# irenemizus/ArtStyleTransfer

Hardware: AMD Instinct MI355X
Metric: style-transfer iters/sec at L=2 (1024-px) (higher is better)
Workload: dtype f32 via f16x2 split (3 f16 MFMAs per product, f32 accumulate; the 14 large-channel conv launches of a closure as Winograd F(2,3) in that arithmetic); 1 GPU; pyramid style transfer, levels_num=3 (1536x1024+768x512+384x256), lbfgs as the reference constructs it (max_eval 1 under torch 2.10), content+noise init, seeded synthetic VGG19 weights, per-step image yield on; parallelism=1 GPU

## Files before the change

### artstyletransfer_amd/_lib.py

```python
from __future__ import annotations

import ctypes as C
import os
import subprocess
import threading

_HERE = os.path.dirname(os.path.abspath(__file__))
LIB_PATH = os.environ.get("NST_LIB") or os.path.join(_HERE, "libnst_hip.so")
CSRC = os.path.join(_HERE, "csrc")

NST_OK = 0
NST_E_ARG = -1
NST_E_STATE = -2
NST_E_UNAVAILABLE = -5
NST_VGG19_CONVS = 13
NST_MAX_LEVELS = 8
NST_LOSS_ROW = 4
NST_MAX_STYLES = 8
NST_OPT_ADAM = 0
NST_OPT_LBFGS = 1
NST_COLOR_RGB = 0
NST_COLOR_LUMINANCE = 1
NST_POOL_MAX = 0
NST_POOL_AVG = 1

c_float_p = C.POINTER(C.c_float)
REDUCE_HOOK = C.CFUNCTYPE(None, C.c_void_p)
c_void = C.c_void_p


NST_CONV_F32, NST_CONV_BF16X3, NST_CONV_F16X2 = 0, 1, 2
CONV_MODES = {"f32": NST_CONV_F32, "bf16x3": NST_CONV_BF16X3, "f16x2": NST_CONV_F16X2}
NST_COMM_ID_BYTES = 128


class StepInfo(C.Structure):
    _fields_ = [("closures", C.c_int), ("total_closures", C.c_int), ("accepted", C.c_int),
                ("loss", C.c_float), ("lr", C.c_float), ("t", C.c_float), ("history", C.c_int)]


class Options(C.Structure):
    _fields_ = [("struct_size", C.c_int), ("conv_mode", C.c_int), ("batched", C.c_int), ("single_stream", C.c_int),
                ("use_graph", C.c_int), ("h2_band_rows", C.c_int), ("lbfgs_gram", C.c_int), ("h2_mfma16", C.c_int),
                ("h2_wg256", C.c_int), ("h2_tile_rows", C.c_int), ("gram_overlap", C.c_int), ("h2_persist", C.c_int), ("level_split", C.c_int), ("h2_winograd", C.c_int)]


class LaunchInfo(C.Structure):
    _fields_ = [(n, C.c_int) for n in ("cls", "h", "w", "cin", "cout", "layer", "h2_rows", "h2_bn", "h2_ntw", "h2_chunk",
                                       "h2_mfma16", "h2_persist", "h2_second", "h2_unpool", "h2_bands")]


SYMBOLS = {
    "nst_version": (C.c_int, []),
    "nst_last_error": (C.c_char_p, [c_void]),
    "nst_device_count": (C.c_int, [C.POINTER(C.c_int)]),
    "nst_ctx_create": (C.c_int, [C.c_int, C.POINTER(c_void), C.POINTER(c_void), C.POINTER(c_void)]),
    "nst_options_default": (None, [C.POINTER(Options)]),
    "nst_ctx_create_ex": (C.c_int, [C.c_int, C.POINTER(c_void), C.POINTER(c_void), C.POINTER(Options), C.POINTER(c_void)]),
    "nst_ctx_destroy": (None, [c_void]),
    "nst_job_configure": (C.c_int, [c_void, C.c_int, C.c_int, C.c_int]),
    "nst_job_set_taps": (C.c_int, [c_void, C.c_int, C.c_uint, C.c_int]),
    "nst_job_set_color": (C.c_int, [c_void, C.c_int]),
    "nst_job_color": (C.c_int, [c_void]),
    "nst_job_set_pooling": (C.c_int, [c_void, C.c_int]),
    "nst_job_pooling": (C.c_int, [c_void]),
    "nst_job_set_style_weights": (C.c_int, [c_void, c_float_p]),
    "nst_job_style_weights": (C.c_int, [c_void, c_float_p]),
    "nst_color_stats": (C.c_int, [c_void, c_void, C.c_int, C.c_int, C.POINTER(C.c_double), C.POINTER(C.c_double), c_void]),
    "nst_color_transfer_matrix": (C.c_int, [C.POINTER(C.c_double)] * 6),
    "nst_color_affine": (C.c_int, [c_void, c_void, C.c_int, C.c_int, C.POINTER(C.c_double), C.POINTER(C.c_double), c_void, c_void]),
    "nst_luminance": (C.c_int, [c_void, c_void, C.c_int, C.c_int, C.c_double, C.c_double, c_void, c_void]),
    "nst_luminance_recombine": (C.c_int, [c_void, c_void, c_void, C.c_int, C.c_int, c_void, c_void]),
    "nst_level_set_targets": (C.c_int, [c_void, C.c_int, c_void, c_void, C.c_int, C.c_int, c_void]),
    "nst_level_set_targets_blend": (C.c_int, [c_void, C.c_int, c_void, C.c_int, C.POINTER(c_void), C.POINTER(C.c_int),
                                              C.POINTER(C.c_int), c_float_p, c_void]),
    "nst_level_set_guidance": (C.c_int, [c_void, C.c_int, C.c_int, c_void, c_float_p, c_void]),
    "nst_level_set_targets_guided": (C.c_int, [c_void, C.c_int, c_void, c_void, C.c_int, C.c_int, c_void, c_void]),
    "nst_level_guidance": (C.c_int, [c_void, C.c_int, C.POINTER(C.c_int), c_float_p, C.POINTER(C.c_double)]),
    "nst_level_guidance_planes": (C.c_int, [c_void, C.c_int, C.c_int, c_void, c_void]),
    "nst_closure": (C.c_int, [c_void, c_void, C.c_float, C.c_float, C.c_float, c_void, c_void, c_void]),
    "nst_closure_levels": (C.c_int, [c_void, c_void, C.c_float, C.c_float, C.c_float, C.c_uint, c_void, c_void, c_void]),
    "nst_closure_forward": (C.c_int, [c_void, c_void, C.c_float, C.c_float, C.c_float, C.c_uint, c_void, c_void]),
    "nst_closure_backward": (C.c_int, [c_void, c_void, C.c_float, C.c_float, C.c_float, C.c_uint, c_void, c_void]),
    "nst_opt_shard_levels": (C.c_int, [c_void, C.c_uint, c_void, c_void, c_void, c_void]),
    "nst_opt_shard_levels_comm": (C.c_int, [c_void, C.c_uint, c_void]),
    "nst_opt_history": (C.c_int, [c_void, C.POINTER(C.c_int), C.POINTER(C.c_int)]),
    "nst_opt_set_closure_reuse": (C.c_int, [c_void, C.c_int]),
    "nst_opt_closure_stats": (C.c_int, [c_void, C.POINTER(C.c_long), C.POINTER(C.c_long)]),
    "nst_opt_set_lazy_backward": (C.c_int, [c_void, C.c_int]),
    "nst_opt_backward_stats": (C.c_int, [c_void, C.POINTER(C.c_long), C.POINTER(C.c_long)]),
    "nst_comm_unique_id": (C.c_int, [c_void]),
    "nst_comm_create": (C.c_int, [C.c_int, C.c_int, C.c_int, c_void, C.POINTER(c_void)]),
    "nst_comm_destroy": (None, [c_void]),
    "nst_comm_info": (C.c_int, [c_void, C.POINTER(C.c_int), C.POINTER(C.c_int), C.POINTER(C.c_long), C.POINTER(C.c_double)]),
    "nst_comm_allreduce_sum": (C.c_int, [c_void, c_void, C.c_size_t, c_void]),
    "nst_adam_step": (C.c_int, [c_void, c_void, c_void, c_void, c_void, C.c_size_t, C.c_int, C.c_double, c_void]),
    "nst_lbfgs_direction": (C.c_int, [c_void, c_void, C.POINTER(c_void), C.POINTER(c_void), C.POINTER(C.c_float), C.c_int,
                                      C.c_float, C.c_size_t, C.c_int, c_void, c_void]),
    "nst_opt_create": (C.c_int, [c_void, C.c_int, C.c_float, C.c_int, C.POINTER(c_void)]),
    "nst_opt_destroy": (None, [c_void]),
    "nst_opt_step": (C.c_int, [c_void, c_void, C.c_float, C.c_float, C.c_float, c_void, C.c_int,
                               C.POINTER(StepInfo), c_void]),
    "nst_vgg_features": (C.c_int, [c_void, c_void, C.c_int, C.c_int, C.POINTER(c_void), c_void]),
    "nst_vgg_features_backward": (C.c_int, [c_void, c_void, C.c_int, C.c_int, C.POINTER(c_void), c_void, c_void]),
    "nst_vgg_activations": (C.c_int, [c_void, c_void, C.c_int, C.c_int, C.POINTER(c_void), c_void]),
    "nst_level_activation": (C.c_int, [c_void, C.c_int, C.c_int, c_void, c_void]),
    "nst_level_image": (C.c_int, [c_void, C.c_int, c_void, c_void]),
    "nst_gram": (C.c_int, [c_void, c_void, C.c_int, C.c_int, C.c_int, C.c_int, c_void, c_void]),
    "nst_guided_gram_backward": (C.c_int, [c_void, c_void, C.c_size_t, C.c_int, C.c_int, c_void, c_void, c_void, c_void, c_void,
                                            c_void, c_void]),
    "nst_total_variation": (C.c_int, [c_void, c_void, C.c_int, C.c_int, C.c_int, c_void, c_void, c_void]),
    "nst_bicubic_half": (C.c_int, [c_void, c_void, C.c_int, C.c_int, C.c_int, c_void, c_void]),
    "nst_bicubic_half_backward": (C.c_int, [c_void, c_void, C.c_int, C.c_int, C.c_int, c_void, c_void]),
    "nst_prepare_img": (C.c_int, [c_void, c_void, C.c_int, C.c_int, c_void, c_void]),
    "nst_unprepare_img": (C.c_int, [c_void, c_void, C.c_int, C.c_int, c_void, c_void]),
    "nst_resize_bicubic": (C.c_int, [c_void, c_void, C.c_int, C.c_int, C.c_int, c_void, C.c_int, C.c_int, c_void]),
    "nst_gather_rows": (C.c_int, [c_void, c_void, c_void, C.c_size_t, C.c_int, c_void, c_void]),
    "nst_gaussian_mask_accumulate": (C.c_int, [c_void, c_void, c_void, C.c_int, C.c_int, C.c_int, C.c_double, C.c_double,
                                               C.c_double, c_void]),
    "nst_noise_blend": (C.c_int, [c_void, c_void, c_void, C.c_int, C.c_int, C.c_int, C.c_double, c_void, c_void]),
    "nst_scale": (C.c_int, [c_void, c_void, C.c_float, C.c_size_t, c_void, c_void]),
    "nst_window_sums_count": (C.c_int, [C.POINTER(C.c_size_t)]),
    "nst_window_begin": (C.c_int, [c_void, c_void, C.c_int, C.c_int, C.c_int, c_void, c_void]),
    "nst_window_end": (C.c_int, [c_void, c_void, C.c_int, C.c_int, C.c_int, C.c_float, C.c_float, C.c_float, c_void, c_void,
                                 c_void, c_void]),
    "nst_conv_mode": (C.c_int, [c_void]),
    "nst_ctx_bytes": (C.c_int, [c_void, C.POINTER(C.c_size_t)]),
    "nst_set_timing": (C.c_int, [c_void, C.c_int]),
    "nst_last_closure_ms": (C.c_int, [c_void, C.POINTER(C.c_float)]),
    "nst_last_closure_class": (C.c_int, [c_void, C.c_int, C.POINTER(C.c_float), C.POINTER(C.c_int),
                                         C.POINTER(C.c_double)]),
    "nst_last_closure_launches": (C.c_int, [c_void, C.POINTER(LaunchInfo), C.c_int, C.POINTER(C.c_int)]),
    "nst_dump_last_closure": (C.c_int, [c_void]),
    "nst_timing_totals": (C.c_int, [c_void, C.c_int, C.POINTER(C.c_double), C.POINTER(C.c_long),
                                    C.POINTER(C.c_double), C.c_int]),
    "nst_timing_mfma_flops": (C.c_int, [c_void, C.c_int, C.POINTER(C.c_double)]),
}

_lib = None
_lock = threading.Lock()


class NstError(RuntimeError):
    pass


def build(force: bool = False) -> str:
    if force:
        subprocess.run(["make", "-C", CSRC, "clean"], check=True, stdout=subprocess.DEVNULL)
    subprocess.run(["make", "-C", CSRC, "-j8"], check=True)
    return LIB_PATH


def load():
    global _lib
    with _lock:
        if _lib is not None:
            return _lib
        if not os.path.exists(LIB_PATH):
            raise NstError(
                f"{LIB_PATH} is missing: the HIP extension is the only implementation of the style-transfer "
                f"hot path (no CPU fallback). Build it with `python -c 'import __graft_entry__ as g; g.build()'` "
                f"or `make -C {CSRC}`.")
        try:
            lib = C.CDLL(LIB_PATH)
        except OSError as e:
            raise NstError(f"cannot load {LIB_PATH}: {e}") from e
        for name, (res, args) in SYMBOLS.items():
            try:
                fn = getattr(lib, name)
            except AttributeError as e:
                raise NstError(f"{LIB_PATH} does not export {name}; rebuild it") from e
            fn.restype = res
            fn.argtypes = args
        _lib = lib
        return lib


def check(ctx, code: int, what: str) -> None:
    if code != NST_OK:
        msg = load().nst_last_error(ctx)
        raise NstError(f"{what} failed ({code}): {msg.decode() if msg else '?'}")
```

### artstyletransfer_amd/csrc/conv_h2.hip

```cpp
#include <hip/hip_runtime.h>

#include <cstdlib>
#include <type_traits>

#include "nst_kernels.h"

namespace nst {

typedef float f32x4 __attribute__((ext_vector_type(4)));
typedef float f32x2 __attribute__((ext_vector_type(2)));
typedef float f32x16 __attribute__((ext_vector_type(16)));
typedef unsigned int u32x2 __attribute__((ext_vector_type(2)));
typedef unsigned int u32x4 __attribute__((ext_vector_type(4)));
typedef _Float16 f16x2 __attribute__((ext_vector_type(2)));
typedef _Float16 f16x8 __attribute__((ext_vector_type(8)));

namespace {

#ifndef NST_H2_DEEP_WEIGHT_PREFETCH
#define NST_H2_DEEP_WEIGHT_PREFETCH 1
#endif
#ifndef NST_H2_WEIGHT_SETS4
#define NST_H2_WEIGHT_SETS4 1
#endif
// ... 574 lines not shown
    ConvParams p;
    {
        int sp_again, ct_again;
        if (Tiles::REFETCH) (void)tiles.get(opaque_s(tile_k), p, sp_again, ct_again);
        else p = p_loop;
    }
    const int words = p.Cout >> 5;
    const bool avg = p.pool_avg != 0;
    float amax = 0.f;
    auto record_amax = [&]() {
        if (p.amax_out) {
#pragma unroll
            for (int off = 32; off > 0; off >>= 1) amax = fmaxf(amax, __shfl_xor(amax, off));
            if (lane == 0) atomicMax(p.amax_out + ((slot_seed * (C::NT / 64) + wave) & (NST_AMAX_SLOTS - 1)), __float_as_uint(amax));
        }
    };

    if constexpr (M16) {
        const int cg0 = n0 + wn * 32 * NTW;
        const float lo_clamp = p.relu ? 0.f : -__builtin_inff();
        auto word_of = [&](const unsigned long long b_even, const unsigned long long b_odd) -> unsigned {
            return (unsigned)((b_even >> (16 * kg)) & 0xFFFFull) | ((unsigned)((b_odd >> (16 * kg)) & 0xFFFFull) << 16);
        };
        const bool interior = (y0 + TH <= p.H) && (x0 + C::TW <= p.W);
        const bool fwd_like = !p.bits_in && !p.addend;
        const bool bwd_like = p.bits_in && !p.bits_out && !p.pool_out && !p.pcode_out;
        if (interior && !p.mask && (fwd_like || bwd_like) && (size_t)p.H * p.W * p.Cout * 4 < 0xFFFFFF00ull) {
            const unsigned out_bytes = (unsigned)((size_t)p.H * p.W * p.Cout * 4);
            const unsigned bit_bytes = (unsigned)((size_t)p.H * p.W * words * 4);
            const int colB = p.Cout * 4, rowB = p.W * colB;
            const int wcolB = words * 4, wrowB = p.W * wcolB;
            const int pix0 = (y0 + wm * 4) * p.W + x0 + 4 * kg;
            const unsigned vbase = (unsigned)pix0 * (unsigned)colB + (unsigned)(cg0 + l15) * 4u;
            const unsigned wbase = (unsigned)pix0 * (unsigned)wcolB + (unsigned)(cg0 >> 5) * 4u;
            const __amdgpu_buffer_rsrc_t rs_out = __builtin_amdgcn_make_buffer_rsrc(p.out, 0, out_bytes * ABL_ST, 0x00020000);
            if (bwd_like) {
                const __amdgpu_buffer_rsrc_t rs_bits = __builtin_amdgcn_make_buffer_rsrc(const_cast<unsigned*>(p.bits_in), 0, bit_bytes * ABL_EL, 0x00020000);
                const __amdgpu_buffer_rsrc_t rs_add = __builtin_amdgcn_make_buffer_rsrc(const_cast<float*>(p.addend), 0, p.addend ? out_bytes * ABL_EL : 0u, 0x00020000);
                unsigned wv[4][4][NTW];
#pragma unroll
                for (int mt = 0; mt < 4; ++mt)
#pragma unroll
                    for (int i = 0; i < 4; ++i) {
                        if (NTW == 2) {
                            const u32x2 w2 = __builtin_bit_cast(u32x2, __builtin_amdgcn_raw_buffer_load_b64(rs_bits, wbase, mt * wrowB + i * wcolB, 0));
                            wv[mt][i][0] = w2[0];
                            wv[mt][i][NTW - 1] = w2[1];
                        } else {
                            wv[mt][i][0] = __builtin_amdgcn_raw_buffer_load_b32(rs_bits, wbase, mt * wrowB + i * wcolB, 0);
                        }
                    }
#pragma unroll
                for (int nt = 0; nt < NT16; ++nt) {
                    const float bv = p.bias ? p.bias[cg0 + nt * 16 + l15] : 0.f;
#pragma unroll
                    for (int mt = 0; mt < 4; ++mt) {
                        float ad[4] = {0.f, 0.f, 0.f, 0.f};
                        if (p.addend) {
#pragma unroll
                            for (int i = 0; i < 4; ++i)
                                ad[i] = __builtin_bit_cast(float, __builtin_amdgcn_raw_buffer_load_b32(rs_add, vbase, mt * rowB + i * colB + nt * 64, 0));
                        }
#pragma unroll
                        for (int i = 0; i < 4; ++i) {
                            float v = fmaf(ax16[mt][nt][i], LO_DOWN, am16[mt][nt][i]) * inv + bv;
                            v = fmaxf(v + ad[i], lo_clamp);
                            v = ((wv[mt][i][nt >> 1] >> ((nt & 1) * 16 + l15)) & 1u) ? v : 0.f;
                            __builtin_amdgcn_raw_buffer_store_b32(__builtin_bit_cast(unsigned, v), rs_out, vbase, mt * rowB + i * colB + nt * 64, 0);
                            amax = fmaxf(amax, fabsf(v));
                        }
                    }
                }
            } else {
                const int PW2 = p.W >> 1;
                const unsigned pool_bytes = (unsigned)((size_t)(p.H >> 1) * PW2 * p.Cout * 4);
                const __amdgpu_buffer_rsrc_t rs_bits = __builtin_amdgcn_make_buffer_rsrc(p.bits_out, 0, p.bits_out ? bit_bytes * ABL_ST : 0u, 0x00020000);
                const __amdgpu_buffer_rsrc_t rs_pool = __builtin_amdgcn_make_buffer_rsrc(p.pool_out, 0, p.pool_out ? pool_bytes * ABL_ST : 0u, 0x00020000);
                const __amdgpu_buffer_rsrc_t rs_code = __builtin_amdgcn_make_buffer_rsrc(
                    p.pcode_out, 0, p.pcode_out ? (unsigned)((size_t)(p.H >> 1) * PW2 * words * 16) * ABL_ST : 0u, 0x00020000);
                const unsigned wlane = (l15 == 0) ? wbase : 0xFFFFFF00u;
                const int ppix0 = ((y0 + wm * 4) >> 1) * PW2 + ((x0 + 4 * kg) >> 1);
                const unsigned pbase = (unsigned)ppix0 * (unsigned)colB + (unsigned)(cg0 + l15) * 4u;
                const unsigned cbase = (l15 == 0) ? ((unsigned)ppix0 * (unsigned)words + (unsigned)(cg0 >> 5)) * 16u : 0xFFFFFF00u;
#pragma unroll
                for (int nt = 0; nt < NT16; ++nt) {
                    const float bv = p.bias ? p.bias[cg0 + nt * 16 + l15] : 0.f;
#pragma unroll
                    for (int mt = 0; mt < 4; ++mt)
#pragma unroll
                        for (int i = 0; i < 4; ++i) {
                            float v = fmaf(ax16[mt][nt][i], LO_DOWN, am16[mt][nt][i]) * inv + bv;
                            v = fmaxf(v, lo_clamp);
                            am16[mt][nt][i] = v;
                            __builtin_amdgcn_raw_buffer_store_b32(__builtin_bit_cast(unsigned, v), rs_out, vbase, mt * rowB + i * colB + nt * 64, 0);
                            amax = fmaxf(amax, fabsf(v));
                        }
                }
                if (p.bits_out) {
#pragma unroll
                    for (int mt = 0; mt < 4; ++mt)
#pragma unroll
                        for (int i = 0; i < 4; ++i)
#pragma unroll
                            for (int w = 0; w < NTW; ++w) {
                                const unsigned long long b0 = __ballot(am16[mt][2 * w][i] > 0.f), b1 = __ballot(am16[mt][2 * w + 1][i] > 0.f);
                                __builtin_amdgcn_raw_buffer_store_b32(word_of(b0, b1), rs_bits, wlane, mt * wrowB + i * wcolB + w * 4, 0);
                            }
                }
                if (p.pool_out) {
#pragma unroll
                    for (int mt = 0; mt < 4; mt += 2)
#pragma unroll
                        for (int i = 0; i < 4; i += 2) {
                            const int poff = (mt >> 1) * PW2 + (i >> 1);
                            unsigned long long code[NTW][4][2];
#pragma unroll
                            for (int nt = 0; nt < NT16; ++nt) {
                                const float e0 = am16[mt][nt][i], e1 = am16[mt][nt][i + 1], e2 = am16[mt + 1][nt][i], e3 = am16[mt + 1][nt][i + 1];
                                const float mx = avg ? (((e0 + e1) + e2) + e3) * 0.25f : fmaxf(fmaxf(e0, e1), fmaxf(e2, e3));
                                __builtin_amdgcn_raw_buffer_store_b32(__builtin_bit_cast(unsigned, mx), rs_pool, pbase, poff * colB + nt * 64, 0);
                                if (p.pcode_out) {
                                    if (avg) {
                                        code[nt >> 1][0][nt & 1] = __ballot(e0 > 0.f);
                                        code[nt >> 1][1][nt & 1] = __ballot(e1 > 0.f);
                                        code[nt >> 1][2][nt & 1] = __ballot(e2 > 0.f);
                                        code[nt >> 1][3][nt & 1] = __ballot(e3 > 0.f);
                                    } else {
                                        int pos = 0;
                                        float best = e0;
                                        if (e1 > best) { best = e1; pos = 1; }
                                        if (e2 > best) { best = e2; pos = 2; }
                                        if (e3 > best) { best = e3; pos = 3; }
                                        const bool live = best > 0.f;
#pragma unroll
                                        for (int q = 0; q < 4; ++q) code[nt >> 1][q][nt & 1] = __ballot(live && pos == q);
                                    }
                                }
                            }
                            if (p.pcode_out) {
#pragma unroll
                                for (int w = 0; w < NTW; ++w)
#pragma unroll
                                    for (int q = 0; q < 4; ++q)
                                        __builtin_amdgcn_raw_buffer_store_b32(word_of(code[w][q][0], code[w][q][1]), rs_code, cbase,
                                                                              (poff * words + w) * 16 + q * 4, 0);
                            }
                        }
                }
            }
            record_amax();
            return;
        }
#pragma unroll
        for (int mt = 0; mt < 4; ++mt) {
            const int y = y0 + wm * 4 + mt;
#pragma unroll
            for (int i = 0; i < 4; ++i) {
                const int x = x0 + 4 * kg + i;
                const bool inb = (y < p.H && x < p.W);
                const size_t pix = (size_t)y * p.W + x;
#pragma unroll
                for (int nt = 0; nt < NT16; ++nt) {
                    const int co = cg0 + nt * 16 + l15;
                    const size_t idx = pix * p.Cout + co;
                    float v = fmaf(ax16[mt][nt][i], LO_DOWN, am16[mt][nt][i]) * inv + (p.bias ? p.bias[co] : 0.f);
                    if (p.addend && inb) v += p.addend[idx];
                    if (p.relu) v = fmaxf(v, 0.f);
                    if (p.bits_in) {
                        const unsigned wv = inb ? p.bits_in[pix * words + (co >> 5)] : 0u;
                        v = ((wv >> (co & 31)) & 1u) ? v : 0.f;
                    } else if (p.mask) {
                        v = (inb && p.mask[idx] > 0.f) ? v : 0.f;
                    }
                    am16[mt][nt][i] = v;
                    if (inb) {
                        p.out[idx] = v;
                        amax = fmaxf(amax, fabsf(v));
                    }
                }
                if (p.bits_out) {
#pragma unroll
                    for (int w = 0; w < NTW; ++w) {
                        const unsigned long long b0 = __ballot(am16[mt][2 * w][i] > 0.f), b1 = __ballot(am16[mt][2 * w + 1][i] > 0.f);
                        if (l15 == 0 && inb) p.bits_out[pix * words + (cg0 >> 5) + w] = word_of(b0, b1);
                    }
                }
            }
        }
        if (p.pool_out) {
            const int PH2 = p.H >> 1, PW2 = p.W >> 1;
#pragma unroll
            for (int mt = 0; mt < 4; mt += 2)
#pragma unroll
                for (int i = 0; i < 4; i += 2) {
                    const int py = (y0 + wm * 4 + mt) >> 1, px = (x0 + 4 * kg + i) >> 1;
                    const bool inw = (py < PH2 && px < PW2);
                    unsigned long long code[NTW][4][2];
#pragma unroll
                    for (int nt = 0; nt < NT16; ++nt) {
                        const float e0 = am16[mt][nt][i], e1 = am16[mt][nt][i + 1], e2 = am16[mt + 1][nt][i], e3 = am16[mt + 1][nt][i + 1];
                        const float mx = avg ? (((e0 + e1) + e2) + e3) * 0.25f : fmaxf(fmaxf(e0, e1), fmaxf(e2, e3));
                        if (inw) p.pool_out[((size_t)py * PW2 + px) * p.Cout + cg0 + nt * 16 + l15] = mx;
                        if (avg) {
                            code[nt >> 1][0][nt & 1] = __ballot(e0 > 0.f);
                            code[nt >> 1][1][nt & 1] = __ballot(e1 > 0.f);
                            code[nt >> 1][2][nt & 1] = __ballot(e2 > 0.f);
                            code[nt >> 1][3][nt & 1] = __ballot(e3 > 0.f);
                        } else {
                            int pos = 0;
                            float best = e0;
                            if (e1 > best) { best = e1; pos = 1; }
                            if (e2 > best) { best = e2; pos = 2; }
                            if (e3 > best) { best = e3; pos = 3; }
                            const bool live = best > 0.f;
#pragma unroll
                            for (int q = 0; q < 4; ++q) code[nt >> 1][q][nt & 1] = __ballot(live && pos == q);
                        }
                    }
                    if (p.pcode_out) {
#pragma unroll
                        for (int w = 0; w < NTW; ++w)
#pragma unroll
                            for (int q = 0; q < 4; ++q)
                                if (l15 == 0 && inw)
                                    p.pcode_out[(((size_t)py * PW2 + px) * words + (cg0 >> 5) + w) * 4 + q] = word_of(code[w][q][0], code[w][q][1]);
                    }
                }
        }
        record_amax();
        return;
    }

    const bool interior = (y0 + TH <= p.H) && (x0 + C::TW <= p.W);
    const bool fwd_like = !p.bits_in && !p.addend;
    const bool bwd_like = p.bits_in && !p.bits_out && !p.pool_out && !p.pcode_out;
    if (interior && !p.mask && (fwd_like || bwd_like) && (size_t)p.H * p.W * p.Cout * 4 < 0xFFFFFF00ull) {
        const unsigned out_bytes = (unsigned)((size_t)p.H * p.W * p.Cout * 4);
        const unsigned bit_bytes = (unsigned)((size_t)p.H * p.W * words * 4);
        const int colB = p.Cout * 4, rowB = p.W * colB;
        const int wcolB = words * 4, wrowB = p.W * wcolB;
        const int pix0 = (y0 + wm * 4) * p.W + x0 + 4 * half;
        const int cg0 = n0 + wn * 32 * NTW;
        const unsigned vbase = (unsigned)pix0 * (unsigned)colB + (unsigned)(cg0 + l31) * 4u;
        const unsigned wbase = (unsigned)pix0 * (unsigned)wcolB + (unsigned)(cg0 >> 5) * 4u;
        const __amdgpu_buffer_rsrc_t rs_out = __builtin_amdgcn_make_buffer_rsrc(p.out, 0, out_bytes * ABL_ST, 0x00020000);
        auto soff = [&](int mt, int r, int rb, int cb) { return ((r >> 3) + 2 * mt) * rb + ((r & 3) + 8 * ((r >> 2) & 1)) * cb; };
        if (bwd_like) {
            const __amdgpu_buffer_rsrc_t rs_bits = __builtin_amdgcn_make_buffer_rsrc(const_cast<unsigned*>(p.bits_in), 0, bit_bytes * ABL_EL, 0x00020000);
            const __amdgpu_buffer_rsrc_t rs_add = __builtin_amdgcn_make_buffer_rsrc(const_cast<float*>(p.addend), 0, p.addend ? out_bytes * ABL_EL : 0u, 0x00020000);
            const float lo_clamp = p.relu ? 0.f : -__builtin_inff();
            if (!p.addend) {
                unsigned wv[2][16][NTW];
#pragma unroll
                for (int mt = 0; mt < 2; ++mt)
#pragma unroll
                    for (int r = 0; r < 16; ++r) {
                        if (NTW == 4) {
                            const u32x4 w4 = __builtin_amdgcn_raw_buffer_load_b128(rs_bits, wbase, soff(mt, r, wrowB, wcolB), 0);
#pragma unroll
                            for (int k = 0; k < NTW; ++k) wv[mt][r][k] = w4[k & 3];
                        } else if (NTW == 2) {
                            const u32x2 w2 = __builtin_bit_cast(u32x2, __builtin_amdgcn_raw_buffer_load_b64(rs_bits, wbase, soff(mt, r, wrowB, wcolB), 0));
                            wv[mt][r][0] = w2[0];
                            wv[mt][r][NTW - 1] = w2[1];
                        } else {
                            wv[mt][r][0] = __builtin_amdgcn_raw_buffer_load_b32(rs_bits, wbase, soff(mt, r, wrowB, wcolB), 0);
                        }
                    }
#pragma unroll
                for (int nt = 0; nt < NTW; ++nt) {
                    const float bv = p.bias ? p.bias[cg0 + nt * 32 + l31] : 0.f;
#pragma unroll
                    for (int mt = 0; mt < 2; ++mt)
#pragma unroll
                        for (int r = 0; r < 16; ++r) {
                            float v = fmaf(accx[mt][nt][r], LO_DOWN, accm[mt][nt][r]) * inv + bv;
                            v = fmaxf(v + 0.f, lo_clamp);
                            v = ((wv[mt][r][nt] >> l31) & 1u) ? v : 0.f;
                            __builtin_amdgcn_raw_buffer_store_b32(__builtin_bit_cast(unsigned, v), rs_out, vbase, soff(mt, r, rowB, colB) + nt * 128, 0);
                            amax = fmaxf(amax, fabsf(v));
                        }
                }
                record_amax();
                return;
            }
#pragma unroll
            for (int nt = 0; nt < NTW; ++nt) {
                const float bv = p.bias ? p.bias[cg0 + nt * 32 + l31] : 0.f;
#pragma unroll
                for (int mt = 0; mt < 2; ++mt) {
#pragma unroll
                    for (int r0 = 0; r0 < 16; r0 += 8) {
                        unsigned wv[8];
                        float ad[8];
#pragma unroll
                        for (int k = 0; k < 8; ++k) {
                            const int r = r0 + k;
                            wv[k] = __builtin_amdgcn_raw_buffer_load_b32(rs_bits, wbase, soff(mt, r, wrowB, wcolB) + nt * 4, 0);
                            ad[k] = __builtin_bit_cast(float, __builtin_amdgcn_raw_buffer_load_b32(rs_add, vbase, soff(mt, r, rowB, colB) + nt * 128, 0));
                        }
#pragma unroll
                        for (int k = 0; k < 8; ++k) {
                            const int r = r0 + k;
                            float v = fmaf(accx[mt][nt][r], LO_DOWN, accm[mt][nt][r]) * inv + bv;
                            v = fmaxf(v + ad[k], lo_clamp);
                            v = ((wv[k] >> l31) & 1u) ? v : 0.f;
                            __builtin_amdgcn_raw_buffer_store_b32(__builtin_bit_cast(unsigned, v), rs_out, vbase, soff(mt, r, rowB, colB) + nt * 128, 0);
                            amax = fmaxf(amax, fabsf(v));
                        }
                    }
                }
            }
        } else {
            const int PW2 = p.W >> 1;
            const unsigned pool_bytes = (unsigned)((size_t)(p.H >> 1) * PW2 * p.Cout * 4);
            const __amdgpu_buffer_rsrc_t rs_bits = __builtin_amdgcn_make_buffer_rsrc(p.bits_out, 0, p.bits_out ? bit_bytes * ABL_ST : 0u, 0x00020000);
            const __amdgpu_buffer_rsrc_t rs_pool = __builtin_amdgcn_make_buffer_rsrc(p.pool_out, 0, p.pool_out ? pool_bytes * ABL_ST : 0u, 0x00020000);
            const __amdgpu_buffer_rsrc_t rs_code = __builtin_amdgcn_make_buffer_rsrc(
                p.pcode_out, 0, p.pcode_out ? (unsigned)((size_t)(p.H >> 1) * PW2 * words * 16) * ABL_ST : 0u, 0x00020000);
            const unsigned wlane = (l31 == 0) ? wbase : 0xFFFFFF00u;
            const int ppix0 = ((y0 + wm * 4) >> 1) * PW2 + ((x0 + 4 * half) >> 1);
            const unsigned pbase = (unsigned)ppix0 * (unsigned)colB + (unsigned)(cg0 + l31) * 4u;
            const unsigned cbase = (l31 == 0) ? ((unsigned)ppix0 * (unsigned)words + (unsigned)(cg0 >> 5)) * 16u : 0xFFFFFF00u;
            const float lo_clamp = p.relu ? 0.f : -__builtin_inff();
#pragma unroll
            for (int nt = 0; nt < NTW; ++nt) {
                const float bv = p.bias ? p.bias[cg0 + nt * 32 + l31] : 0.f;
#pragma unroll
                for (int mt = 0; mt < 2; ++mt) {
#pragma unroll
                    for (int r = 0; r < 16; ++r) {
                        float v = fmaf(accx[mt][nt][r], LO_DOWN, accm[mt][nt][r]) * inv + bv;
                        v = fmaxf(v, lo_clamp);
                        accm[mt][nt][r] = v;
                        __builtin_amdgcn_raw_buffer_store_b32(__builtin_bit_cast(unsigned, v), rs_out, vbase, soff(mt, r, rowB, colB) + nt * 128, 0);
                        amax = fmaxf(amax, fabsf(v));
                        if (p.bits_out) {
                            const unsigned long long bal = __ballot(v > 0.f);
                            __builtin_amdgcn_raw_buffer_store_b32(half ? (unsigned)(bal >> 32) : (unsigned)bal, rs_bits, wlane,
                                                                  soff(mt, r, wrowB, wcolB) + nt * 4, 0);
                        }
                    }
                    if (p.pool_out) {
#pragma unroll
                        for (int j = 0; j < 4; ++j) {
                            const int r = 2 * j;
                            const int pcol = (j & 1) + 4 * (j >> 1);
                            const float mx = avg ? (((accm[mt][nt][r] + accm[mt][nt][r + 1]) + accm[mt][nt][r + 8]) + accm[mt][nt][r + 9]) * 0.25f
                                                 : fmaxf(fmaxf(accm[mt][nt][r], accm[mt][nt][r + 1]),
                                                         fmaxf(accm[mt][nt][r + 8], accm[mt][nt][r + 9]));
                            __builtin_amdgcn_raw_buffer_store_b32(__builtin_bit_cast(unsigned, mx), rs_pool, pbase,
                                                                  (mt * PW2 + pcol) * colB + nt * 128, 0);
                            if (p.pcode_out) {
                                int pos = 0;
                                float best = accm[mt][nt][r];
                                if (accm[mt][nt][r + 1] > best) { best = accm[mt][nt][r + 1]; pos = 1; }
                                if (accm[mt][nt][r + 8] > best) { best = accm[mt][nt][r + 8]; pos = 2; }
                                if (accm[mt][nt][r + 9] > best) { best = accm[mt][nt][r + 9]; pos = 3; }
                                const bool live = best > 0.f;
                                constexpr int roff[4] = {0, 1, 8, 9};
#pragma unroll
                                for (int q = 0; q < 4; ++q) {
                                    const unsigned long long bal = __ballot(avg ? accm[mt][nt][r + roff[q]] > 0.f : (live && pos == q));
                                    __builtin_amdgcn_raw_buffer_store_b32(half ? (unsigned)(bal >> 32) : (unsigned)bal, rs_code, cbase,
                                                                          ((mt * PW2 + pcol) * words + nt) * 16 + q * 4, 0);
                                }
                            }
                        }
                    }
                }
            }
        }
        record_amax();
        return;
    }

#pragma unroll
    for (int nt = 0; nt < NTW; ++nt) {
        const int co = n0 + wn * 32 * NTW + nt * 32 + l31;
        const int cw = (n0 + wn * 32 * NTW + nt * 32) >> 5;
        const float bv = p.bias ? p.bias[co] : 0.f;
#pragma unroll
        for (int mt = 0; mt < 2; ++mt) {
#pragma unroll
            for (int r = 0; r < 16; ++r) {
                const int m = (r & 3) + 8 * (r >> 2) + 4 * half;
                const int y = y0 + wm * 4 + mt * 2 + (m >> 4);
                const int x = x0 + (m & 15);
                const bool inb = (y < p.H && x < p.W);
                const size_t pix = (size_t)y * p.W + x;
                const size_t idx = pix * p.Cout + co;
                float v = fmaf(accx[mt][nt][r], LO_DOWN, accm[mt][nt][r]) * inv + bv;
                if (p.addend && inb) v += p.addend[idx];
                if (p.relu) v = fmaxf(v, 0.f);
                if (p.bits_in) {
                    const unsigned wv = inb ? p.bits_in[pix * words + cw] : 0u;
                    v = ((wv >> l31) & 1u) ? v : 0.f;
                } else if (p.mask) {
                    v = (inb && p.mask[idx] > 0.f) ? v : 0.f;
                }
                if (p.bits_out) {
                    const unsigned long long bal = __ballot(v > 0.f);
                    if (l31 == 0 && inb) p.bits_out[pix * words + cw] = half ? (unsigned)(bal >> 32) : (unsigned)bal;
                }
                accm[mt][nt][r] = v;
                if (inb) {
                    p.out[idx] = v;
                    amax = fmaxf(amax, fabsf(v));
                }
            }
            if (p.pool_out) {
                const int py = (y0 + wm * 4 + mt * 2) >> 1;
                const int PH2 = p.H >> 1, PW2 = p.W >> 1;
#pragma unroll
                for (int j = 0; j < 4; ++j) {
                    const int r = 2 * j;
                    const float mx = avg ? (((accm[mt][nt][r] + accm[mt][nt][r + 1]) + accm[mt][nt][r + 8]) + accm[mt][nt][r + 9]) * 0.25f
                                         : fmaxf(fmaxf(accm[mt][nt][r], accm[mt][nt][r + 1]),
                                                 fmaxf(accm[mt][nt][r + 8], accm[mt][nt][r + 9]));
                    const int mcol = (r & 3) + 8 * (r >> 2) + 4 * half;
                    const int px = (x0 + mcol) >> 1;
                    const bool inw = (py < PH2 && px < PW2);
                    if (inw) p.pool_out[((size_t)py * PW2 + px) * p.Cout + co] = mx;
                    if (p.pcode_out) {
                        int pos = 0;
                        float best = accm[mt][nt][r];
                        if (accm[mt][nt][r + 1] > best) { best = accm[mt][nt][r + 1]; pos = 1; }
                        if (accm[mt][nt][r + 8] > best) { best = accm[mt][nt][r + 8]; pos = 2; }
                        if (accm[mt][nt][r + 9] > best) { best = accm[mt][nt][r + 9]; pos = 3; }
                        const bool live = best > 0.f;
                        constexpr int roff[4] = {0, 1, 8, 9};
#pragma unroll
                        for (int q = 0; q < 4; ++q) {
                            const unsigned long long bal = __ballot(avg ? accm[mt][nt][r + roff[q]] > 0.f : (live && pos == q));
                            if (l31 == 0 && inw)
                                p.pcode_out[(((size_t)py * PW2 + px) * words + cw) * 4 + q] = half ? (unsigned)(bal >> 32) : (unsigned)bal;
                        }
                    }
                }
            }
        }
    }
    record_amax();
    };
    epilogue();
    if (!tiles.get(tile_k + 1, p, sp, ct)) break;
    primed = chain;
  }
}

__device__ __forceinline__ int xcd_contiguous(const int b, const int grid) {
#ifdef NST_NO_XCD_MAP
    return b;
#else
    const int x = b & 7, k = b >> 3;
    const int q = grid >> 3, r = grid & 7;
    return x * q + (x < r ? x : r) + k;
#endif
}

struct H2OneTile {
    static constexpr bool REFETCH = false;
    const ConvParams& p;
    int n_ct;
    __device__ __forceinline__ bool get(const int k, ConvParams& q, int& sp, int& ct) const {
        if (k > 0) return false;
        const int t = xcd_contiguous((int)blockIdx.x, (int)gridDim.x);
        q = p;
        sp = t / n_ct;
        ct = t % n_ct;
        return true;
    }
};
template <bool PERSIST>
struct H2BatchTiles {
    static constexpr bool REFETCH = PERSIST;
    const ConvBatch& b;
    int n_ct;
    __device__ __forceinline__ bool get(const int k, ConvParams& p, int& sp, int& ct) const {
        int t;
        if (!PERSIST) {
            if (k > 0) return false;
            t = xcd_contiguous((int)blockIdx.x, (int)gridDim.x);
        } else {
            const int x = (int)blockIdx.x & 7, j = ((int)blockIdx.x >> 3) + k * ((int)gridDim.x >> 3);
            const int q = b.total_tiles >> 3, r = b.total_tiles & 7;
            if (j >= q + (x < r ? 1 : 0)) return false;
            t = x * q + (x < r ? x : r) + j;
        }
        const int sp_all = t / n_ct;
// ... 93 lines not shown
    sh.rows = shortk ? 8 : h2_tile_rows(Cout, blocks16, tile_rows);
    sh.bn = wide ? 128 : 64;
    sh.chunk = (!wide || shortk) ? 16 : 32;
    sh.ntw = (sh.chunk == 16) ? 2 : (sh.rows < 16 ? 1 : (wg256 ? 4 : 2));
    sh.m16 = (sh.chunk == 32 && sh.ntw <= 2 && h2_use_m16(mfma16, sh.rows, sh.ntw, unpool)) ? 1 : 0;
    sh.second = second ? 1 : 0;
    sh.unpool = unpool ? 1 : 0;
    sh.bands = 1;
    int tiles = 0;
    for (int i = 0; i < n; ++i) tiles += ((W[i] + 15) / 16) * ((H[i] + sh.rows - 1) / sh.rows);
    *blocks = tiles * (Cout / sh.bn);
    const bool pshape = sh.chunk == 16 || (sh.rows == 16 && sh.ntw == 2);
    sh.persist = (persist_opt && !second && Cin > 0 && *blocks > h2_resident(sh) && pshape && !sh.m16) ? 1 : 0;
    return sh;
}

template <int TH, int BN, int NTW, int KC>
static void launch_batch_cfg(const ConvBatch& b, const H2Shape& sh, int blocks, hipStream_t stream) {
    constexpr int lds = H2Cfg<TH, BN, NTW, KC>::LDS_BYTES;
    constexpr int nt = H2Cfg<TH, BN, NTW, KC>::NT;
    if constexpr (h2_m16_built<NTW, KC>) {
        if (sh.m16) {
            if (b.unpool) hipLaunchKernelGGL((conv_h2_batch_kernel<TH, BN, NTW, KC, true, true, false>), dim3(blocks), dim3(nt), lds, stream, b);
            else hipLaunchKernelGGL((conv_h2_batch_kernel<TH, BN, NTW, KC, false, true, false>), dim3(blocks), dim3(nt), lds, stream, b);
            return;
        }
    }
    if constexpr (h2_persist_shape<TH, BN, NTW, KC>) {
        if (sh.persist) {
            if (b.unpool) hipLaunchKernelGGL((conv_h2_batch_kernel<TH, BN, NTW, KC, true, false, true>), dim3(blocks), dim3(nt), lds, stream, b);
            else hipLaunchKernelGGL((conv_h2_batch_kernel<TH, BN, NTW, KC, false, false, true>), dim3(blocks), dim3(nt), lds, stream, b);
            return;
        }
    }
    if (b.unpool) hipLaunchKernelGGL((conv_h2_batch_kernel<TH, BN, NTW, KC, true, false, false>), dim3(blocks), dim3(nt), lds, stream, b);
    else hipLaunchKernelGGL((conv_h2_batch_kernel<TH, BN, NTW, KC, false, false, false>), dim3(blocks), dim3(nt), lds, stream, b);
}
template <int TH, int BN, int NTW, int KC>
static void launch_single_cfg(const ConvParams& p, const H2Shape& sh, int blocks, hipStream_t stream) {
    constexpr int lds = H2Cfg<TH, BN, NTW, KC>::LDS_BYTES;
    constexpr int nt = H2Cfg<TH, BN, NTW, KC>::NT;
    if constexpr (h2_m16_built<NTW, KC>) {
        if (sh.m16) {
            if (p.pcode_in) hipLaunchKernelGGL((conv_h2_kernel<TH, BN, NTW, KC, true, true>), dim3(blocks), dim3(nt), lds, stream, p);
            else hipLaunchKernelGGL((conv_h2_kernel<TH, BN, NTW, KC, false, true>), dim3(blocks), dim3(nt), lds, stream, p);
            return;
        }
    }
    if (p.pcode_in) hipLaunchKernelGGL((conv_h2_kernel<TH, BN, NTW, KC, true, false>), dim3(blocks), dim3(nt), lds, stream, p);
    else hipLaunchKernelGGL((conv_h2_kernel<TH, BN, NTW, KC, false, false>), dim3(blocks), dim3(nt), lds, stream, p);
}

static bool h2_operands_ok(const void* wt, const unsigned* amax_in, int Cin, int Cout, const float* in2, const float* wt2,
                           const unsigned* a2, const unsigned* w2, int Cin2) {
    if (Cin % 32 != 0 || Cout % 64 != 0) return false;
    if (Cin > 0 ? (!wt || !amax_in) : !in2) return false;
    if (in2 && (!wt2 || !a2 || !w2 || Cin2 % 32 != 0 || Cin2 != Cout)) return false;
    return true;
}

template <int TH, int BN, int NTW, int KC>
struct H2Tag { static constexpr int th = TH, bn = BN, ntw = NTW, kc = KC; };
template <typename Launch>
static void h2_dispatch(const H2Shape& sh, Launch&& go) {
    if (sh.bn == 64) go(H2Tag<16, 64, 2, 16>{});
    else if (sh.chunk == 16) go(H2Tag<8, 128, 2, 16>{});
    else if (sh.rows == 4) go(H2Tag<4, 128, 1, 32>{});
    else if (sh.rows == 8) go(H2Tag<8, 128, 1, 32>{});
    else if (sh.ntw == 4) go(H2Tag<16, 128, 4, 32>{});
    else go(H2Tag<16, 128, 2, 32>{});
}

hipError_t launch_conv_h2_batch(const ConvBatch& b0, hipStream_t stream, H2Shape* shape) {
    if (b0.n < 1 || b0.n > 8) return hipErrorInvalidValue;
    ConvBatch b = b0;
    int H[8], W[8];
    bool second = false;
    for (int i = 0; i < b.n; ++i) {
        const ConvImage& im = b.img[i];
        if (!h2_operands_ok(b.wt_h2, im.amax_in, b.Cin, b.Cout, im.in2, im.wt2_f32, im.amax_in2, im.amax_w2, b.Cin2))
            return hipErrorInvalidValue;
        if ((size_t)im.H * im.W * (b.Cin > b.Cin2 ? b.Cin : b.Cin2) * 4 >= 0xFFFFFF00ull) return hipErrorInvalidValue;
        if ((b.unpool != 0) != (im.pcode_in != nullptr)) return hipErrorInvalidValue;
        H[i] = im.H; W[i] = im.W;
        second = second || (im.in2 != nullptr);
    }
    int blocks = 0;
    const H2Shape sh = h2_launch_shape(H, W, b.n, b.Cin, b.Cout, b.unpool != 0, second, b.tile_rows, b.mfma16, b.wg256, b.persist, &blocks);
    int tiles = 0;
    for (int i = 0; i < b.n; ++i) {
        b.img[i].tiles_x = (b.img[i].W + 15) / 16;
        tiles += b.img[i].tiles_x * ((b.img[i].H + sh.rows - 1) / sh.rows);
        b.img[i].tile_end = tiles;
    }
    b.total_tiles = blocks;
    b.persist = sh.persist;
    if (sh.persist) blocks = h2_resident(sh);
    if (shape) *shape = sh;
    h2_dispatch(sh, [&](auto cfg) { launch_batch_cfg<decltype(cfg)::th, decltype(cfg)::bn, decltype(cfg)::ntw, decltype(cfg)::kc>(b, sh, blocks, stream); });
    return hipGetLastError();
}

hipError_t launch_conv_h2(const ConvParams& p0, hipStream_t stream, H2Shape* shape) {
    if (!h2_operands_ok(p0.wt_h2, p0.amax_in, p0.Cin, p0.Cout, p0.in2, p0.wt2_f32, p0.amax_in2, p0.amax_w2, p0.Cin2))
        return hipErrorInvalidValue;
    ConvParams p = p0;
    p.ksplit = 1;
    int all_blocks = 0;
    H2Shape sh = h2_launch_shape(&p.H, &p.W, 1, p.Cin, p.Cout, p.pcode_in != nullptr, p.in2 != nullptr, p.tile_rows, p.mfma16, p.wg256, 0, &all_blocks);
    const int th = sh.rows;
    p.tiles_x = (p.W + 15) / 16;
    const int cmax = p.Cin > p.Cout ? (p.Cin > p.Cin2 ? p.Cin : p.Cin2) : (p.Cout > p.Cin2 ? p.Cout : p.Cin2);
    const size_t row_bytes = (size_t)p.W * cmax * 4;
    int band_rows = p.H;
    if ((size_t)p.H * row_bytes >= 0xFFFFFF00ull) {
        const long fit = (long)(0xFFFFFF00ull / row_bytes) - 32;
        band_rows = (int)(fit / 16) * 16;
        if (band_rows < 16) return hipErrorInvalidValue;
    }
    const int forced_band = p.band_rows;
    if (forced_band >= 16 && forced_band / 16 * 16 < band_rows) band_rows = forced_band / 16 * 16;
    const int PW2 = p.W >> 1, wi = p.Cin >> 5, wo = p.Cout >> 5;
    int bands = 0;
    for (int r0 = 0; r0 < p.H; r0 += band_rows) {
        const int r1 = (r0 + band_rows < p.H) ? r0 + band_rows : p.H;
        const int b0 = (r0 >= 16) ? r0 - 16 : 0, b1 = (r1 + 16 < p.H) ? r1 + 16 : p.H;
        ConvParams q = p;
        const size_t px0 = (size_t)b0 * p.W, pp0 = (size_t)(b0 >> 1) * PW2;
        if (q.pcode_in) { q.in += pp0 * p.Cin; q.pcode_in += pp0 * wi * 4; }
        else if (q.in) q.in += px0 * p.Cin;
        if (q.in2) { q.in2 += px0 * p.Cin2; if (q.in2_rows > 0) q.in2_row0 -= b0; }
        q.out += px0 * p.Cout;
        if (q.addend) q.addend += px0 * p.Cout;
        if (q.mask) q.mask += px0 * p.Cout;
        if (q.bits_in) q.bits_in += px0 * wo;
        if (q.bits_out) q.bits_out += px0 * wo;
        if (q.pool_out) q.pool_out += pp0 * p.Cout;
        if (q.pcode_out) q.pcode_out += pp0 * wo * 4;
        q.H = b1 - b0;
        q.ty0 = (r0 - b0) / th;
        q.tiles_y = (r1 - r0 + th - 1) / th;
        const int blocks = q.tiles_x * q.tiles_y * (p.Cout / sh.bn);
        h2_dispatch(sh, [&](auto cfg) { launch_single_cfg<decltype(cfg)::th, decltype(cfg)::bn, decltype(cfg)::ntw, decltype(cfg)::kc>(q, sh, blocks, stream); });
        const hipError_t e = hipGetLastError();
        if (e != hipSuccess) return e;
        ++bands;
    }
    sh.bands = bands;
    if (shape) *shape = sh;
    return hipSuccess;
}

__global__ __launch_bounds__(256) void absmax_slots_kernel(const float* __restrict__ x, size_t n, unsigned* __restrict__ slots) {
    float m = 0.f;
    const size_t n4 = n / 4;
    for (size_t i = (size_t)blockIdx.x * blockDim.x + threadIdx.x; i < n4; i += (size_t)gridDim.x * blockDim.x) {
        const f32x4 v = reinterpret_cast<const f32x4*>(x)[i];
        m = fmaxf(fmaxf(m, fmaxf(fabsf(v[0]), fabsf(v[1]))), fmaxf(fabsf(v[2]), fabsf(v[3])));
    }
    if (blockIdx.x == 0 && threadIdx.x < (n & 3)) m = fmaxf(m, fabsf(x[n4 * 4 + threadIdx.x]));
#pragma unroll
    for (int off = 32; off > 0; off >>= 1) m = fmaxf(m, __shfl_xor(m, off));
    if ((threadIdx.x & 63) == 0)
        atomicMax(slots + ((blockIdx.x * 4 + (threadIdx.x >> 6)) & (NST_AMAX_SLOTS - 1)), __float_as_uint(m));
}
hipError_t launch_absmax_slots(const float* x, size_t n, unsigned* slots, hipStream_t stream) {
    size_t blocks = (n / 4 + 255) / 256;
    if (blocks > 1024) blocks = 1024;
    if (blocks < 1) blocks = 1;
    hipLaunchKernelGGL(absmax_slots_kernel, dim3((unsigned)blocks), dim3(256), 0, stream, x, n, slots);
    return hipGetLastError();
}

}
```

### artstyletransfer_amd/csrc/conv_wino.hip

```cpp
#include <hip/hip_runtime.h>

#include "nst_kernels.h"

namespace nst {

typedef float f32x4 __attribute__((ext_vector_type(4)));
typedef float f32x2 __attribute__((ext_vector_type(2)));
typedef float f32x16 __attribute__((ext_vector_type(16)));
typedef unsigned int u32x2 __attribute__((ext_vector_type(2)));
typedef unsigned int u32x4 __attribute__((ext_vector_type(4)));
typedef _Float16 f16x2 __attribute__((ext_vector_type(2)));
typedef _Float16 f16x8 __attribute__((ext_vector_type(8)));

#ifdef NST_WINO_STAMPS
__device__ unsigned long long g_wino_stamps[(1 << 14) * 8];
#define WSTAMP(k)                                                                                      \
    do {                                                                                               \
        if (tid == 0 && blockIdx.x < (1 << 14)) g_wino_stamps[blockIdx.x * 8 + (k)] = __builtin_amdgcn_s_memtime(); \
    } while (0)
#define WSTAMP_REAL(k)                                                                                 \
    do {                                                                                               \
        if (tid == 0 && blockIdx.x < (1 << 14)) g_wino_stamps[blockIdx.x * 8 + (k)] = __builtin_amdgcn_s_memrealtime(); \
    } while (0)
#else
// ... 212 lines not shown
            *reinterpret_cast<_Float16*>(base + x * W_PAIRS * W_ROWB + 64) = lo;
        }
    };

    const int a_base = ((l31 >> 3)) * W_PROWB + (xi * W_PAIRS + (l31 & 7)) * W_ROWB + half * 16;
    struct AF { f16x8 v[2][2]; };
    auto read_a = [&](AF& f, const unsigned char* buf, int ky, int ks) {
#pragma unroll
        for (int mt = 0; mt < 2; ++mt)
#pragma unroll
            for (int s = 0; s < 2; ++s)
                f.v[mt][s] = *reinterpret_cast<const f16x8*>(buf + a_base + (mt * 4 + ky) * W_PROWB + s * 64 + ks * 32);
    };
    struct BF { f16x8 v[2][2]; };
    auto load_b = [&](BF& f, int chunk, int ky, int ks) {
        const int soff = (((((ct * nch + chunk) * 3 + ky) * 8 + wave) * 2 + ks) * 4 * 64) * 16;
#pragma unroll
        for (int nt = 0; nt < 2; ++nt)
#pragma unroll
            for (int s = 0; s < 2; ++s)
                f.v[nt][s] = __builtin_bit_cast(f16x8, __builtin_amdgcn_raw_buffer_load_b128(rs_w, lane * 16 + (nt * 2 + s) * 64 * 16, soff, 0));
    };
    auto multiply = [&](const AF& a, const BF& w) {
#pragma unroll
        for (int mt = 0; mt < 2; ++mt)
#pragma unroll
            for (int nt = 0; nt < 2; ++nt) {
                accx[mt][nt] = __builtin_amdgcn_mfma_f32_32x32x16_f16(a.v[mt][1], w.v[nt][0], accx[mt][nt], 0, 0, 0);
                accm[mt][nt] = __builtin_amdgcn_mfma_f32_32x32x16_f16(a.v[mt][0], w.v[nt][0], accm[mt][nt], 0, 0, 0);
                accx[mt][nt] = __builtin_amdgcn_mfma_f32_32x32x16_f16(a.v[mt][0], w.v[nt][1], accx[mt][nt], 0, 0, 0);
            }
    };

    Stage d;
    Stage1 d1;
    BF B[3];
    AF A[2];
    {
        task_load(d, tid, 0);
        load_b(B[0], 0, 0, 0);
        load_b(B[1], 0, 0, 1);
        task_store(d, tid, smem);
        row_load(d1, tid, 0);
        row_store(d1, tid, smem);
    }
    __syncthreads();
    WSTAMP(1);
    read_a(A[0], smem, 0, 0);
    if (wave >= 4) __builtin_amdgcn_s_setprio(1);

    for (int c = 0; c < nch; ++c) {
        const unsigned char* cur = smem + (c & 1) * W_A_BYTES;
        unsigned char* nxt = smem + ((c + 1) & 1) * W_A_BYTES;
        const int cn = (c + 1 < nch) ? c + 1 : c;
        int to = tid;
        asm volatile("" : "+v"(to));
#pragma unroll
        for (int q = 0; q < 6; ++q) {
            {
                const int q2 = q + 2;
                if (q2 < 6) load_b(B[q2 % 3], c, q2 >> 1, q2 & 1);
                else load_b(B[q2 % 3], cn, (q2 - 6) >> 1, (q2 - 6) & 1);
            }
            if (q == 0) task_load(d, to, cn);
            if (q == 1) row_load(d1, to, cn);
            if (q + 1 < 6) read_a(A[(q + 1) & 1], cur, (q + 1) >> 1, (q + 1) & 1);
            multiply(A[q & 1], B[q % 3]);
            if (q == 4) task_store(d, to, nxt);
            if (q == 5) row_store(d1, to, nxt);
        }
        __syncthreads();
        if (c + 1 < nch) read_a(A[0], nxt, 0, 0);
    }

    WSTAMP(2);
    constexpr bool M_FWD = MODE != 2, M_BWD = MODE != 1;
    const float* const e_bias = M_FWD ? b.bias : nullptr;
    const bool e_relu = MODE == 0 ? (b.relu != 0) : (MODE == 1);
    unsigned* const e_bits_out = M_FWD ? im.bits_out : nullptr;
    float* const e_pool_out = M_FWD ? im.pool_out : nullptr;
    unsigned* const e_pcode_out = M_FWD ? im.pcode_out : nullptr;
    const float* const e_addend = M_BWD ? im.addend : nullptr;
    const unsigned* const e_bits_in = M_BWD ? im.bits_in : nullptr;
    float* E = reinterpret_cast<float*>(smem);
    unsigned* WB = reinterpret_cast<unsigned*>(smem + W_BITS_OFF);
    unsigned* PC = reinterpret_cast<unsigned*>(smem + W_CODE_OFF);
    const int words = Cout >> 5;
    float amax = 0.f;
    const int yp = tid >> 7, p = (tid >> 4) & 7, cq = tid & 15;
    f32x4 bvp[2];
    unsigned mw[2][2][2];
#pragma unroll
    for (int pass = 0; pass < 2; ++pass) {
        const int co = n0 + pass * 64 + cq * 4;
        bvp[pass] = e_bias ? *reinterpret_cast<const f32x4*>(e_bias + co) : f32x4{0.f, 0.f, 0.f, 0.f};
#pragma unroll
        for (int k = 0; k < 2; ++k) {
            const int gy = y0 + 2 * yp + k, gx = x0 + 2 * p;
            const size_t pa = (size_t)gy * W + gx;
            mw[pass][k][0] = (e_bits_in && gy < H && gx < W) ? e_bits_in[pa * (Cout >> 5) + (co >> 5)] : 0u;
            mw[pass][k][1] = (e_bits_in && gy < H && gx + 1 < W) ? e_bits_in[(pa + 1) * (Cout >> 5) + (co >> 5)] : 0u;
        }
    }
#pragma unroll
    for (int mt = 0; mt < 2; ++mt)
#pragma unroll
        for (int nt = 0; nt < 2; ++nt)
#pragma unroll
            for (int r = 0; r < 16; ++r) {
                const int m = (r & 3) + 8 * (r >> 2) + 4 * half;
                E[(xi * 64 + mt * 32 + m) * 128 + wn * 64 + nt * 32 + l31] = fmaf(accx[mt][nt][r], LO_DOWN, accm[mt][nt][r]) * inv;
            }
    __syncthreads();
    WSTAMP(3);
    for (int pass = 0; pass < 2; ++pass) {
        const int co = n0 + pass * 64 + cq * 4;
        const f32x4 bv = bvp[pass];
        const int w = pass * 2 + (cq >> 3), sh = (cq & 7) * 4;
        f32x4 win[2][2];
#pragma unroll
        for (int k = 0; k < 2; ++k) {
            const int yy = 2 * yp + k, pr = yy * 8 + p;
            const f32x4 m0 = *reinterpret_cast<const f32x4*>(E + (0 * 64 + pr) * 128 + pass * 64 + cq * 4);
            const f32x4 m1 = *reinterpret_cast<const f32x4*>(E + (1 * 64 + pr) * 128 + pass * 64 + cq * 4);
            const f32x4 m2 = *reinterpret_cast<const f32x4*>(E + (2 * 64 + pr) * 128 + pass * 64 + cq * 4);
            const f32x4 m3 = *reinterpret_cast<const f32x4*>(E + (3 * 64 + pr) * 128 + pass * 64 + cq * 4);
            f32x4 ya = m0 + m1 + m2 + bv, yb = m1 - m2 - m3 + bv;
            const int gy = y0 + yy, gx = x0 + 2 * p;
            const bool ina = gy < H && gx < W, inb = gy < H && gx + 1 < W;
            const size_t pa = (size_t)gy * W + gx;
            if (e_addend) {
                if (ina) ya += *reinterpret_cast<const f32x4*>(e_addend + pa * Cout + co);
                if (inb) yb += *reinterpret_cast<const f32x4*>(e_addend + (pa + 1) * Cout + co);
            }
            unsigned ka = 0xFu, kb = 0xFu;
            if (e_bits_in) {
                ka = (mw[pass][k][0] >> (co & 31)) & 0xFu;
                kb = (mw[pass][k][1] >> (co & 31)) & 0xFu;
            }
            unsigned na = 0u, nb = 0u;
#pragma unroll
            for (int e = 0; e < 4; ++e) {
                if (e_relu) { ya[e] = fmaxf(ya[e], 0.f); yb[e] = fmaxf(yb[e], 0.f); }
                ya[e] = ((ka >> e) & 1u) ? ya[e] : 0.f;
                yb[e] = ((kb >> e) & 1u) ? yb[e] : 0.f;
                na |= (ya[e] > 0.f ? 1u : 0u) << e;
                nb |= (yb[e] > 0.f ? 1u : 0u) << e;
                if (ina) amax = fmaxf(amax, fabsf(ya[e]));
                if (inb) amax = fmaxf(amax, fabsf(yb[e]));
            }
            if (ina) *reinterpret_cast<f32x4*>(im.out + pa * Cout + co) = ya;
            if (inb) *reinterpret_cast<f32x4*>(im.out + (pa + 1) * Cout + co) = yb;
            if (e_bits_out) {
                const int pix = yy * 16 + 2 * p;
                const unsigned wa = or8(na << sh), wb = or8(nb << sh);
                if ((cq & 7) == 0) { WB[pix * 4 + w] = wa; WB[(pix + 1) * 4 + w] = wb; }
            }
            win[k][0] = ya; win[k][1] = yb;
        }
        const int py = (y0 + 2 * yp) >> 1, px = (x0 + 2 * p) >> 1;
        const bool inw = py < PH2 && px < PW2;
        if (e_pool_out) {
            f32x4 mx;
            unsigned cn[4] = {0u, 0u, 0u, 0u};
#pragma unroll
            for (int e = 0; e < 4; ++e) {
                const float e0 = win[0][0][e], e1 = win[0][1][e], e2 = win[1][0][e], e3 = win[1][1][e];
                if (b.pool_avg) {
                    mx[e] = (((e0 + e1) + e2) + e3) * 0.25f;
                    cn[0] |= (e0 > 0.f ? 1u : 0u) << e;
                    cn[1] |= (e1 > 0.f ? 1u : 0u) << e;
                    cn[2] |= (e2 > 0.f ? 1u : 0u) << e;
                    cn[3] |= (e3 > 0.f ? 1u : 0u) << e;
                    continue;
                }
                mx[e] = fmaxf(fmaxf(e0, e1), fmaxf(e2, e3));
                int pos = 0;
                float best = e0;
                if (e1 > best) { best = e1; pos = 1; }
                if (e2 > best) { best = e2; pos = 2; }
                if (e3 > best) { best = e3; pos = 3; }
                const bool live = best > 0.f;
#pragma unroll
                for (int q = 0; q < 4; ++q) cn[q] |= ((live && pos == q) ? 1u : 0u) << e;
            }
            if (inw) *reinterpret_cast<f32x4*>(e_pool_out + ((size_t)py * PW2 + px) * Cout + co) = mx;
            if (e_pcode_out) {
#pragma unroll
                for (int q = 0; q < 4; ++q) {
                    const unsigned wq = or8(cn[q] << sh);
                    if ((cq & 7) == 0) PC[((yp * 8 + p) * 4 + w) * 4 + q] = wq;
                }
            }
        }
    }
    if (e_bits_out || e_pcode_out) {
        __syncthreads();
        if (e_bits_out) {
            const int pix = tid >> 2, w2 = tid & 3;
            const int gy = y0 + (pix >> 4), gx = x0 + (pix & 15);
            if (gy < H && gx < W) e_bits_out[((size_t)gy * W + gx) * words + (n0 >> 5) + w2] = WB[tid];
        }
        if (e_pcode_out) {
            const int pp = tid >> 4, w2 = (tid >> 2) & 3, q = tid & 3;
            const int qy = (y0 >> 1) + (pp >> 3), qx = (x0 >> 1) + (pp & 7);
            if (qy < PH2 && qx < PW2) e_pcode_out[(((size_t)qy * PW2 + qx) * words + (n0 >> 5) + w2) * 4 + q] = PC[tid];
        }
    }
    if (im.amax_out) {
#pragma unroll
        for (int off = 32; off > 0; off >>= 1) amax = fmaxf(amax, __shfl_xor(amax, off));
        if (lane == 0) atomicMax(im.amax_out + ((blockIdx.x * 8 + wave) & (NST_AMAX_SLOTS - 1)), __float_as_uint(amax));
    }
    WSTAMP(4);
#ifdef NST_WINO_STAMPS
    asm volatile("s_waitcnt vmcnt(0)" ::: "memory");
#endif
    WSTAMP(5);
    WSTAMP_REAL(7);
}

namespace {
template <bool UNPOOL, int MODE>
hipError_t wino_attr() {
    return hipFuncSetAttribute(reinterpret_cast<const void*>(&conv_wino_batch_kernel<UNPOOL, MODE>), hipFuncAttributeMaxDynamicSharedMemorySize, W_LDS);
}
}

hipError_t conv_wino_init_device() {
    hipError_t e = wino_attr<false, 0>();
    if (e == hipSuccess) e = wino_attr<false, 1>();
    if (e == hipSuccess) e = wino_attr<false, 2>();
    if (e == hipSuccess) e = wino_attr<true, 0>();
    if (e == hipSuccess) e = wino_attr<true, 2>();
    return e;
}

bool conv_wino_eligible(const ConvBatch& b) {
    if (!b.wt_wino || b.Cin < 128 || b.Cin % 64 != 0 || b.Cout % 128 != 0 || b.Cin2 != 0) return false;
    for (int i = 0; i < b.n; ++i) {
        const ConvImage& im = b.img[i];
        if (im.in2 || im.mask || !im.amax_in || (b.unpool != 0) != (im.pcode_in != nullptr)) return false;
        if (im.pcode_out && !im.pool_out) return false;
        if ((size_t)im.H * im.W * (b.Cin > b.Cout ? b.Cin : b.Cout) * 4 >= 0xFFFFFF00ull) return false;
    }
    return true;
}

hipError_t launch_conv_wino_batch(const ConvBatch& b0, hipStream_t stream) {
    if (b0.n < 1 || b0.n > 8 || !conv_wino_eligible(b0)) return hipErrorInvalidValue;
    ConvBatch b = b0;
    int tiles = 0;
    for (int i = 0; i < b.n; ++i) {
        b.img[i].tiles_x = (b.img[i].W + W_TW - 1) / W_TW;
        tiles += b.img[i].tiles_x * ((b.img[i].H + W_TH - 1) / W_TH);
        b.img[i].tile_end = tiles;
    }
    bool fwd = b.relu && b.bias, bwd = !b.relu && !b.bias;
    for (int i = 0; i < b.n; ++i) {
        const ConvImage& im = b.img[i];
        fwd = fwd && !im.addend && !im.bits_in;
        bwd = bwd && !im.bits_out && !im.pool_out && !im.pcode_out;
    }
    const dim3 grid(tiles * (b.Cout / 128)), block(512);
    if (b.unpool) {
        if (bwd) hipLaunchKernelGGL((conv_wino_batch_kernel<true, 2>), grid, block, W_LDS, stream, b);
        else hipLaunchKernelGGL((conv_wino_batch_kernel<true, 0>), grid, block, W_LDS, stream, b);
    } else {
        if (fwd) hipLaunchKernelGGL((conv_wino_batch_kernel<false, 1>), grid, block, W_LDS, stream, b);
        else if (bwd) hipLaunchKernelGGL((conv_wino_batch_kernel<false, 2>), grid, block, W_LDS, stream, b);
        else hipLaunchKernelGGL((conv_wino_batch_kernel<false, 0>), grid, block, W_LDS, stream, b);
    }
    return hipGetLastError();
}

}
```

### artstyletransfer_amd/csrc/nst_api.cpp

```cpp
#include <algorithm>
#include <cmath>
#include <cstring>

#include "nst_ctx.h"

using namespace nst;

static int vgg_outputs(nst_ctx* ctx, const float* x, int h, int w, float* const* outs, int n, const int* layer_of, void* stream) {
    NSTCHK(bind(ctx));
    if (!x || !outs) return fail(ctx, NST_E_ARG, "null argument");
    hipStream_t s = static_cast<hipStream_t>(stream);
    Scratch sc(ctx, s);
    ActSet& a = sc.acts;
    NSTCHK(alloc_acts(ctx, a, h, w));
    NSTCHK(forward(ctx, a, x, h, w, s));
    for (int i = 0; i < n; ++i) {
        if (!outs[i]) continue;
        const int l = layer_of ? layer_of[i] : i;
        if (launch_hwc_to_chw(a.act[l], kCout[l], a.h[l], a.w[l], outs[i], s) != hipSuccess) return fail(ctx, NST_E_HIP, "hwc_to_chw launch failed");
    }
    return sc.finish();
}

extern "C" {

int nst_vgg_features(nst_ctx* ctx, const float* x, int h, int w, float* const* outs, void* stream) {
    return vgg_outputs(ctx, x, h, w, outs, 6, kTapLayer, stream);
}
int nst_vgg_activations(nst_ctx* ctx, const float* x, int h, int w, float* const* outs, void* stream) {
    return vgg_outputs(ctx, x, h, w, outs, NL, nullptr, stream);
}

int nst_vgg_features_backward(nst_ctx* ctx, const float* x, int h, int w, const float* const* gouts, float* gx,
                              void* stream) {
    NSTCHK(bind(ctx));
    if (!x || !gouts || !gx) return fail(ctx, NST_E_ARG, "null argument");
    hipStream_t s = static_cast<hipStream_t>(stream);
    Scratch sc(ctx, s);
    ActSet& a = sc.acts;
    float* g0 = nullptr; float* g1 = nullptr;
    NSTCHK(alloc_acts(ctx, a, h, w));
    NSTCHK(sc.alloc(&g0, (size_t)h * w * 64));
    NSTCHK(sc.alloc(&g1, (size_t)h * w * 64));
    NSTCHK(forward(ctx, a, x, h, w, s));
    Inject inj[NL];
    for (int i = 0; i < 6; ++i) {
        if (!gouts[i]) continue;
        const int l = kTapLayer[i];
        float* g = nullptr;
        NSTCHK(sc.alloc(&g, (size_t)a.h[l] * a.w[l] * kCout[l]));
        if (launch_chw_to_hwc(gouts[i], kCout[l], a.h[l], a.w[l], g, s) != hipSuccess) return fail(ctx, NST_E_HIP, "chw_to_hwc launch failed");
        inj[l].direct = g;
    }
    NSTCHK(backward(ctx, a, inj, nullptr, g0, g1, gx, h, w, s, NL - 1, ctx->taps.use_relu != 0));
    return sc.finish();
}

int nst_gram(nst_ctx* ctx, const float* f, int C, int h, int w, int normalize, float* gram, void* stream) {
    NSTCHK(bind(ctx));
    if (!f || !gram || C < 1 || h < 1 || w < 1) return fail(ctx, NST_E_ARG, "bad argument");
    hipStream_t s = static_cast<hipStream_t>(stream);
    const size_t N = (size_t)h * w;
    Scratch sc(ctx, s);
    float* nhwc = nullptr; float* part = nullptr; unsigned* amax = nullptr;
    NSTCHK(sc.alloc(&nhwc, N * C));
    NSTCHK(sc.alloc(&part, (size_t)gram_nsplit(C, N) * C * C));
    if (ctx->conv_mode == 2) NSTCHK(sc.alloc(&amax, (size_t)NST_AMAX_SLOTS));
    if (launch_chw_to_hwc(f, C, h, w, nhwc, s) != hipSuccess) return fail(ctx, NST_E_HIP, "chw_to_hwc launch failed");
    if (amax && (launch_zero(amax, NST_AMAX_SLOTS, s) != hipSuccess || launch_absmax_slots(nhwc, N * C, amax, s) != hipSuccess))
        return fail(ctx, NST_E_HIP, "absmax launch failed");
    NSTCHK(gram_of(ctx, nhwc, N, C, amax, normalize ? (float)((double)C * h * w) : 1.f, part, nullptr, 0.f, gram, nullptr, nullptr, nullptr, nullptr, s));
    return sc.finish();
}

int nst_guided_gram_backward(nst_ctx* ctx, const float* f, size_t N, int C, int R, const float* planes, const float* S,
                             const float* addend, const unsigned* relu_bits, float* out, unsigned* amax_slots, void* stream) {
    NSTCHK(bind(ctx));
    if (!f || !planes || !S || !out || N < 1 || C < 64 || C % 64 != 0 || R < 1 || R > NST_MAX_REGIONS)
        return fail(ctx, NST_E_ARG, "bad argument");
    hipStream_t s = static_cast<hipStream_t>(stream);
    GuidedBwd gb{};
    gb.F = f; gb.N = N; gb.C = C; gb.R = R;
    for (int r = 0; r < R; ++r) { gb.t[r] = planes + (size_t)r * N; gb.S[r] = S + (size_t)r * C * C; }
    gb.addend = addend; gb.out = out; gb.bits = relu_bits; gb.amax_out = amax_slots;
    if (amax_slots) HIPCHK(ctx, launch_zero(amax_slots, NST_AMAX_SLOTS, s));
    HIPCHK(ctx, launch_guided_bwd(gb, s));
    return NST_OK;
}

int nst_level_activation(nst_ctx* ctx, int level, int layer, float* out, void* stream) {
    NSTCHK(bind(ctx));
    ++ctx->ws_seq;
    if (level < 0 || level >= ctx->levels) return fail(ctx, NST_E_STATE, "level not configured");
    if (layer < 0 || layer >= NL || !out) return fail(ctx, NST_E_ARG, "bad argument");
    const ActSet& a = ctx->lv[level].acts;
    hipStream_t s = enter(ctx, stream);
    HIPCHK(ctx, launch_hwc_to_chw(a.act[layer], kCout[layer], a.h[layer], a.w[layer], out, s));
    mark(ctx, s);
    return NST_OK;
}

int nst_level_image(nst_ctx* ctx, int level, float* out, void* stream) {
    NSTCHK(bind(ctx));
    if (level < 1 || level >= ctx->levels) return fail(ctx, NST_E_ARG, "level must be 1 .. levels_num - 1 (level 0 is the caller's x)");
    if (!out) return fail(ctx, NST_E_ARG, "null argument");
    const LevelWs& L = ctx->lv[level];
    hipStream_t s = enter(ctx, stream);
    HIPCHK(ctx, hipMemcpyAsync(out, L.xl, (size_t)ctx->channels * L.h * L.w * sizeof(float), hipMemcpyDeviceToDevice, s));
    mark(ctx, s);
    return NST_OK;
}

int nst_total_variation(nst_ctx* ctx, const float* y, int C, int h, int w, float* value, float* grad, void* stream) {
    NSTCHK(bind(ctx));
    if (!y || !value) return fail(ctx, NST_E_ARG, "null argument");
    hipStream_t s = static_cast<hipStream_t>(stream);
    double* partial = nullptr; float* means = nullptr;
    int r = dev_alloc_t(ctx, &partial, 2 * TV_BLOCKS);
    if (r == NST_OK) r = dev_alloc_t(ctx, &means, 2);
    hipError_t e = hipSuccess;
    if (r == NST_OK) {
        e = launch_tv_partial(y, C, h, w, partial, s);
        if (e == hipSuccess) e = launch_tv_finish(y, C, h, w, partial, 1.f, grad, 0, means, s);
        float m[2] = {0, 0};
        if (e == hipSuccess) e = hipMemcpyAsync(m, means, 8, hipMemcpyDeviceToHost, s);
        if (e == hipSuccess) e = hipStreamSynchronize(s);
        const float tv = m[0] * m[0] + m[1] * m[1];
        if (e == hipSuccess) e = hipMemcpy(value, &tv, 4, hipMemcpyHostToDevice);
    }
    dev_free(partial); dev_free(means);
    if (r != NST_OK) return r;
    HIPCHK(ctx, e);
    return NST_OK;
}

int nst_bicubic_half(nst_ctx* ctx, const float* x, int C, int h, int w, float* y, void* stream) {
    NSTCHK(bind(ctx));
    if (!x || !y || h < 2 || w < 2) return fail(ctx, NST_E_ARG, "bad argument");
    HIPCHK(ctx, launch_bicubic_down(x, C, h, w, h / 2, w / 2, y, static_cast<hipStream_t>(stream)));
    return NST_OK;
}
int nst_bicubic_half_backward(nst_ctx* ctx, const float* gy, int C, int h, int w, float* gx, void* stream) {
    NSTCHK(bind(ctx));
    if (!gy || !gx || h < 2 || w < 2) return fail(ctx, NST_E_ARG, "bad argument");
    HIPCHK(ctx, launch_bicubic_down_bwd(gy, C, h, w, h / 2, w / 2, gx, 0, static_cast<hipStream_t>(stream)));
    return NST_OK;
}
int nst_prepare_img(nst_ctx* ctx, const float* hwc, int h, int w, float* chw, void* stream) {
    NSTCHK(bind(ctx));
    if (!hwc || !chw) return fail(ctx, NST_E_ARG, "null argument");
    HIPCHK(ctx, launch_prepare_img(hwc, h, w, chw, static_cast<hipStream_t>(stream)));
    return NST_OK;
}
int nst_unprepare_img(nst_ctx* ctx, const float* chw, int h, int w, float* hwc, void* stream) {
    NSTCHK(bind(ctx));
    if (!hwc || !chw) return fail(ctx, NST_E_ARG, "null argument");
    HIPCHK(ctx, launch_unprepare_img(chw, h, w, hwc, static_cast<hipStream_t>(stream)));
    return NST_OK;
}

int nst_resize_bicubic(nst_ctx* ctx, const float* src, int h, int w, int channels, float* dst, int nh, int nw, void* stream) {
    NSTCHK(bind(ctx));
    if (!src || !dst || h < 1 || w < 1 || nh < 1 || nw < 1 || channels < 1) return fail(ctx, NST_E_ARG, "bad argument");
    HIPCHK(ctx, launch_resize_hwc(src, h, w, channels, dst, nh, nw, static_cast<hipStream_t>(stream)));
    return NST_OK;
}
int nst_gather_rows(nst_ctx* ctx, const float* src, const long long* perm, size_t rows, int channels, float* dst, void* stream) {
    NSTCHK(bind(ctx));
    if (!src || !perm || !dst || channels < 1) return fail(ctx, NST_E_ARG, "bad argument");
    HIPCHK(ctx, launch_gather_rows(src, perm, rows, channels, dst, static_cast<hipStream_t>(stream)));
    return NST_OK;
}
int nst_gaussian_mask_accumulate(nst_ctx* ctx, float* acc, const float* src, int h, int w, int channels, double central,
                                 double peripheral, double dispersion, void* stream) {
    NSTCHK(bind(ctx));
    if (!acc || h < 1 || w < 1 || channels < 1) return fail(ctx, NST_E_ARG, "bad argument");
    HIPCHK(ctx, launch_gauss_mask_acc(acc, src, h, w, channels, central, peripheral, dispersion, static_cast<hipStream_t>(stream)));
    return NST_OK;
}
int nst_noise_blend(nst_ctx* ctx, const float* content, const float* noise, int h, int w, int channels, double noise_factor,
                    float* out, void* stream) {
    NSTCHK(bind(ctx));
// ... 145 lines not shown
```

### artstyletransfer_amd/csrc/nst_closure.cpp

```cpp
#include <algorithm>
#include <cmath>
#include <cstring>

#include "nst_ctx.h"

using namespace nst;

namespace {

double conv_flops(int h, int w, int cin, int cout, int taps) { return 2.0 * h * w * (double)cin * cout * taps; }

bool uses_pieces(const nst_ctx* ctx, const ConvParams& p) {
    if (ctx->conv_mode == 2) return true;
    return ctx->conv_mode != 0 && (size_t)p.H * p.W * p.Cin * 4 < 0xFFFFFF00ull;
}
hipError_t launch_conv3(nst_ctx* ctx, const ConvParams& p, Timer& t) {
    hipStream_t s = t.s;
    if (uses_pieces(ctx, p)) {
        if (ctx->conv_mode != 2) return launch_conv_bf3(p, s);
        H2Shape sh{};
        const hipError_t e = launch_conv_h2(p, s, &sh);
        t.shape(sh);
        return e;
    }
    hipError_t e = launch_conv_mfma(p, 9, s);
    if (e == hipSuccess && ctx->conv_mode == 2 && p.amax_out)
        e = launch_absmax_slots(p.out, (size_t)p.H * p.W * p.Cout, p.amax_out, s);
    return e;
}
bool bf3_unsplit(const nst_ctx* ctx, const ConvParams& p) {
    if (!uses_pieces(ctx, p)) return false;
    if (ctx->conv_mode == 2) return true;
    const int S = conv_bf3_ksplit(p.H, p.W, p.Cin, p.Cout);
    return !(p.partial && S > 1 && (size_t)S * p.H * p.W * p.Cout <= p.partial_floats);
}

void conv_setup(const nst_ctx* ctx, ConvParams& p, const ActSet& a, int l, bool dgrad) {
    p.wt = dgrad ? ctx->wd[l] : ctx->wf[l]; p.wt_bf = dgrad ? ctx->wd_bf[l] : ctx->wf_bf[l];
    p.partial = a.splitk; p.partial_floats = a.splitk_floats;
    if (ctx->conv_mode != 2) return;
    p.wt_h2 = dgrad ? ctx->wd_h2[l] : ctx->wf_h2[l]; p.wt_h2_inv = dgrad ? ctx->wd_h2_inv[l] : ctx->wf_h2_inv[l];
    p.band_rows = ctx->band_rows; p.mfma16 = ctx->mfma16; p.wg256 = ctx->wg256; p.tile_rows = ctx->tile_rows;
}
void conv_setup(const nst_ctx* ctx, ConvBatch& b, int l, bool dgrad) {
    b.mfma16 = ctx->mfma16; b.wg256 = ctx->wg256; b.tile_rows = ctx->tile_rows; b.persist = ctx->persist;
    if (l < 1) { b.wt_h2_inv = 1.f; return; }
    b.wt_bf = dgrad ? ctx->wd_bf[l] : ctx->wf_bf[l];
    b.wt_h2 = dgrad ? ctx->wd_h2[l] : ctx->wf_h2[l]; b.wt_h2_inv = dgrad ? ctx->wd_h2_inv[l] : ctx->wf_h2_inv[l];
    b.wt_wino = dgrad ? ctx->wd_wino[l] : ctx->wf_wino[l]; b.wt_wino_inv = dgrad ? ctx->wd_wino_inv[l] : ctx->wf_wino_inv[l];
}
int launch_conv_batch(nst_ctx* ctx, const ConvBatch& b, Timer& t, bool allow_wino) {
    const bool h2 = ctx->conv_mode == 2;
    if (h2 && allow_wino && b.wt_wino && conv_wino_eligible(b)) { t.mfma_factor(2.0); HIPCHK(ctx, launch_conv_wino_batch(b, t.s)); }
    else if (h2) {
        H2Shape sh{};
        const hipError_t e = launch_conv_h2_batch(b, t.s, &sh);
        t.shape(sh);
        HIPCHK(ctx, e);
    } else HIPCHK(ctx, launch_conv_bf3_batch(b, t.s));
    return NST_OK;
}

hipError_t launch_pool_fwd(const nst_ctx* ctx, const float* in, int H, int W, int C, float* out, hipStream_t s) {
    return (ctx->pool_avg ? launch_avgpool_fwd : launch_maxpool_fwd)(in, H, W, C, out, s);
}
hipError_t launch_pool_bwd_relu(const nst_ctx* ctx, const float* a, const float* gpool, int H, int W, int C, float* gin, hipStream_t s) {
    return (ctx->pool_avg ? launch_avgpool_bwd_relu : launch_maxpool_bwd_relu)(a, gpool, H, W, C, gin, s);
}

struct StyleTerm { int C; size_t N; double divisor; float coef; };
StyleTerm style_term(const Taps& tp, int q, const ActSet& a, float sw, float w, int norm_rows = 0) {
    const int l = tp.style[q], C = kCout[l];
    const size_t N = (size_t)(norm_rows > 0 ? norm_rows >> kScale[l] : a.h[l]) * a.w[l];
    const double chw = (double)C * (double)N;
    return {C, N, chw, (float)((double)sw * (double)w * 4.0 / ((double)tp.nstyle * (double)C * C * chw))};
}
float content_coef(float cw, double n) { return (float)((double)cw * 2.0 / n); }

size_t gram_part_offset(const Taps& tp, int h, int w, int k) {
    size_t off = 0;
    for (int q = 0; q < k; ++q) {
        const int l = tp.style[q];
        const size_t N = (size_t)(h >> kScale[l]) * (w >> kScale[l]);
        off += (size_t)gram_nsplit(kCout[l], N) * kCout[l] * kCout[l];
    }
    return off;
}

StyleTerm guided_term(const Taps& tp, int q, const ActSet& a, float sw, float w, const Guidance& g, int r) {
    const int l = tp.style[q], C = kCout[l];
    const size_t N = (size_t)a.h[l] * a.w[l];
    const double cn = (double)C * g.mass[kScale[l]][r];
    return {C, N, cn, (float)((double)sw * (double)w * (double)g.lambda[r] * 4.0 / ((double)tp.nstyle * (double)C * C * cn))};
}
bool guided_levels(const nst_ctx* ctx, const int* lv, int n) { return n > 0 && ctx->lv[lv[0]].guide.R > 0; }
GuidedBwd guided_bwd_of(const nst_ctx* ctx, const LevelWs& L, int q) {
    const int l = ctx->taps.style[q], C = kCout[l];
    GuidedBwd gb{};
    gb.R = L.guide.R; gb.C = C; gb.N = (size_t)L.acts.h[l] * L.acts.w[l]; gb.F = L.acts.act[l];
    for (int r = 0; r < gb.R; ++r) {
        gb.t[r] = L.guide.plane(kScale[l], r, L.h, L.w);
        gb.S[r] = L.guide.S[q] + (size_t)r * C * C;
    }
    return gb;
}
int launch_guided_backward(nst_ctx* ctx, const GuidedBwd& gb, hipStream_t s) {
    Timer t(ctx, s, K_GRAM, 2.0 * (double)gb.N * gb.C * gb.C * gb.R);
    HIPCHK(ctx, launch_guided_bwd(gb, s));
    return NST_OK;
}
int guided_fold(nst_ctx* ctx, LevelWs& L, int q, hipStream_t s) {
    Timer t(ctx, s, K_OTHER, 0);
    HIPCHK(ctx, launch_guided_fold(L.guide.partial[q], L.guide.R, gram_finish_blocks(kCout[ctx->taps.style[q]]), L.guide.lambda,
                                   L.style_partial[q], s));
    return NST_OK;
}

}

namespace nst {

int forward(nst_ctx* ctx, ActSet& a, const float* x, int h, int w, hipStream_t s, int last_layer, int channels) {
    a.begin_pass();
    const bool h2 = ctx->conv_mode == 2;
    if (h2) HIPCHK(ctx, launch_zero(a.amax, (size_t)(NL + kMaxStyle) * NST_AMAX_SLOTS, s));
    {
        Timer t(ctx, s, K_CONV1, conv_flops(h, w, 3, 64, 9));
        unsigned* bits = ctx->conv_mode ? a.bits[0] : nullptr;
        HIPCHK(ctx, launch_conv1_1_fwd(x, h, w, ctx->w11k, ctx->bias[0], a.act[0], bits, h2 ? amax_act(a, 0) : nullptr, s, channels));
        a.bits_valid[0] = bits != nullptr;
    }
    for (int l = 1; l <= last_layer; ++l) {
        const int pk = pool_index_after(l - 1);
        const float* in = (pk >= 0) ? a.pool[pk] : a.act[l - 1];
        ConvParams p{};
        p.in = in; p.bias = ctx->bias[l]; p.addend = nullptr; p.mask = nullptr; p.out = a.act[l];
        p.H = a.h[l]; p.W = a.w[l]; p.Cin = kCin[l]; p.Cout = kCout[l];
        p.relu = ctx->taps.relu_of(l);
        p.pool_avg = ctx->pool_avg;
        conv_setup(ctx, p, a, l, false);
        if (h2) {
            p.amax_in = amax_act(a, l - 1);
            p.amax_out = amax_act(a, l);
        }
        const int pa = pool_index_after(l);
        const bool fuse = bf3_unsplit(ctx, p);
        if (fuse) {
            p.bits_out = a.bits[l];
            if (pa >= 0 && l < last_layer) p.pool_out = a.pool[pa];
        }
        {
            Timer t(ctx, s, K_CONV3, conv_flops(p.H, p.W, p.Cin, p.Cout, 9), p.H, p.W, p.Cin, p.Cout, 9, l);
            HIPCHK(ctx, launch_conv3(ctx, p, t));
        }
        a.bits_valid[l] = fuse && a.bits[l] != nullptr;
        if (pa >= 0 && l < last_layer) {
            if (p.pool_out) {
                a.pooled[pa] = true;
            } else {
                Timer t(ctx, s, K_OTHER, 0);
                HIPCHK(ctx, launch_pool_fwd(ctx, a.act[l], a.h[l], a.w[l], kCout[l], a.pool[pa], s));
            }
        }
    }
    return NST_OK;
}

int backward(nst_ctx* ctx, ActSet& a, const Inject* inj, const ContentJob* cj, float* gbuf0, float* gbuf1, float* gx,
             int h, int w, hipStream_t s, int top, bool top_mask, int channels) {
    float* cur = gbuf0;
    float* oth = gbuf1;
    const bool h2 = ctx->conv_mode == 2;
    if (h2) HIPCHK(ctx, launch_zero(amax_grad(a, 0), (size_t)NL * NST_AMAX_SLOTS, s));
    {
        const int l = top;
        const size_t n = (size_t)a.h[l] * a.w[l] * kCout[l];
        const bool content = inj[l].content && cj;
        if (content) {
            Timer t(ctx, s, K_OTHER, 0);
            HIPCHK(ctx, launch_mse_grad(a.act[l], cj->target, cj->n, cj->coef, oth, cj->partial, s));
        }
        if (inj[l].guided) {
            GuidedBwd gb = *inj[l].guided;
            gb.addend = content ? oth : nullptr; gb.out = cur; gb.mask = top_mask ? a.act[l] : nullptr;
            NSTCHK(launch_guided_backward(ctx, gb, s));
        } else if (inj[l].S) {
            ConvParams p{};
            p.in = a.act[l]; p.wt = inj[l].S; p.out = cur; p.mask = top_mask ? a.act[l] : nullptr;
            p.addend = content ? oth : nullptr;
            p.H = a.h[l]; p.W = a.w[l]; p.Cin = kCout[l]; p.Cout = kCout[l];
            Timer t(ctx, s, K_GRAM, conv_flops(p.H, p.W, p.Cin, p.Cout, 1));
            HIPCHK(ctx, launch_conv_mfma(p, 1, s));
        } else if (content || inj[l].direct) {
            const float* g = content ? oth : inj[l].direct;
            Timer t(ctx, s, K_OTHER, 0);
            if (top_mask) HIPCHK(ctx, launch_relu_mask(a.act[l], g, n, cur, s));
            else HIPCHK(ctx, launch_copy(g, cur, n, s));
        } else {
            HIPCHK(ctx, launch_zero(cur, n, s));
        }
        if (h2) HIPCHK(ctx, launch_absmax_slots(cur, n, amax_grad(a, l), s));
    }
    for (int l = top; l >= 1; --l) {
        const int pk = pool_index_after(l - 1);
        ConvParams p{};
        p.in = cur; p.out = oth;
        p.H = a.h[l]; p.W = a.w[l]; p.Cin = kCout[l]; p.Cout = kCin[l];
        conv_setup(ctx, p, a, l, true);
        if (h2) {
            p.amax_in = amax_grad(a, l);
            p.amax_out = amax_grad(a, l - 1);
        }
        if (pk >= 0) {
            const bool avg = ctx->pool_avg != 0;
// ... 2 lines not shown
                Timer t(ctx, s, K_CONV3, conv_flops(p.H, p.W, p.Cin, p.Cout, 9), p.H, p.W, p.Cin, p.Cout, 9, -l);
                HIPCHK(ctx, launch_conv3(ctx, p, t));
            }
            Timer t(ctx, s, K_OTHER, 0);
            HIPCHK(ctx, launch_pool_bwd_relu(ctx, a.act[l - 1], oth, a.h[l - 1], a.w[l - 1], kCout[l - 1], cur, s));
            if (avg && h2)
                HIPCHK(ctx, launch_absmax_slots(cur, (size_t)a.h[l - 1] * a.w[l - 1] * kCout[l - 1], amax_grad(a, l - 1), s));
        } else {
            const int m = l - 1;
            const Inject& in = inj[m];
            const bool fuse = bf3_unsplit(ctx, p);
            double extra_flops = 0;
            if (in.content && cj) {
                Timer t(ctx, s, K_OTHER, 0);
                HIPCHK(ctx, launch_mse_grad(a.act[m], cj->target, cj->n, cj->coef, oth, cj->partial, s));
                p.addend = oth;
            } else if (in.direct) {
                p.addend = in.direct;
            }
            if (in.guided) {
                GuidedBwd gb = *in.guided;
                gb.addend = p.addend; gb.out = oth;
                NSTCHK(launch_guided_backward(ctx, gb, s));
                p.addend = oth;
            } else if (in.S && fuse && (h2 ? in.S_amax != nullptr : in.S_bf != nullptr)) {
                p.in2 = a.act[m]; p.Cin2 = kCout[m]; p.wt2_bf = in.S_bf;
                p.wt2_f32 = in.S; p.amax_in2 = amax_act(a, m); p.amax_w2 = in.S_amax;
                extra_flops = conv_flops(a.h[m], a.w[m], kCout[m], kCout[m], 1);
            } else if (in.S) {
                ConvParams q{};
                q.in = a.act[m]; q.wt = in.S; q.out = oth; q.addend = p.addend;
                q.H = a.h[m]; q.W = a.w[m]; q.Cin = kCout[m]; q.Cout = kCout[m];
                Timer t(ctx, s, K_GRAM, conv_flops(q.H, q.W, q.Cin, q.Cout, 1));
                HIPCHK(ctx, launch_conv_mfma(q, 1, s));
                p.addend = oth;
            }
            if (fuse && a.bits_valid[m]) p.bits_in = a.bits[m];
            else p.mask = a.act[m];
            {
                Timer t(ctx, s, K_CONV3, conv_flops(p.H, p.W, p.Cin, p.Cout, 9) + extra_flops, p.H, p.W, p.Cin, p.Cout, 9, -l);
                HIPCHK(ctx, launch_conv3(ctx, p, t));
            }
            float* tmp = cur; cur = oth; oth = tmp;
        }
    }
    {
        Timer t(ctx, s, K_CONV1, conv_flops(h, w, 64, 3, 9));
        HIPCHK(ctx, launch_conv1_1_dgrad(cur, h, w, ctx->w11d, h2 ? amax_grad(a, 0) : nullptr, gx, s, channels));
    }
    return NST_OK;
}

int gram_of(nst_ctx* ctx, const float* f_nhwc, size_t N, int C, const unsigned* f_amax, float divisor, float* part, const float* target,
            float coef, float* gram_out, float* S, unsigned short* S_bf, unsigned* S_amax, double* mse_partial,
            hipStream_t s) {
    const int ns = gram_nsplit(C, N);
    {
        Timer t(ctx, s, K_GRAM, 2.0 * (double)N * C * C);
        HIPCHK(ctx, launch_gram_partial(f_nhwc, N, C, ns, f_amax, part, s));
    }
    Timer t(ctx, s, K_OTHER, 0);
    HIPCHK(ctx, launch_gram_finish(part, gram_nslabs(C, ns), C, divisor, target, coef, gram_out, S, S_bf, S_amax,
                                   mse_partial, s));
    return NST_OK;
}

size_t gram_part_floats_for(const Taps& tp, int h, int w) { return gram_part_offset(tp, h, w, tp.nstyle); }

}

namespace {

struct Window {
    int row0, rows, H0;
    float* sums;
};
inline int win_r0(const Window& w, int sc) { return w.row0 >> sc; }
inline int win_nr(const Window& w, int sc) { return ((w.row0 + w.rows) >> sc) - (w.row0 >> sc); }
constexpr size_t kWinGramOff[5] = {0, 64 * 64, 64 * 64 + 128 * 128, 64 * 64 + 128 * 128 + 256 * 256,
                                   64 * 64 + 128 * 128 + 256 * 256 + 512 * 512};
constexpr size_t kWinScalarOff = 64 * 64 + 128 * 128 + 256 * 256 + 2 * 512 * 512;
constexpr size_t kWinSums = kWinScalarOff + 4;

int batched_gram(nst_ctx* ctx, const int* lv, int n, float sw, hipStream_t s, unsigned qmask);
int batched_forward(nst_ctx* ctx, const float* const* xi, const int* lv, int n, hipStream_t s, const Window* win, float fork_sw = -1.f) {
    const bool h2 = ctx->conv_mode == 2;
    const int top = ctx->taps.top;
    for (int k = 0; k < n; ++k) {
        LevelWs& L = ctx->lv[lv[k]];
        ActSet& a = L.acts;
        a.begin_pass();
        if (h2) HIPCHK(ctx, launch_zero(a.amax, (size_t)AMAX_IDS * NST_AMAX_SLOTS, s));
        {
            Timer t(ctx, s, K_OTHER, 0);
            HIPCHK(ctx, launch_tv_partial(xi[lv[k]], ctx->channels, L.h, L.w, L.tv_partial, s, win ? win->row0 : 0, win ? win->rows : 0));
        }
        Timer t(ctx, s, K_CONV1, conv_flops(L.h, L.w, 3, 64, 9));
        HIPCHK(ctx, launch_conv1_1_fwd(xi[lv[k]], L.h, L.w, ctx->w11k, ctx->bias[0], a.act[0], a.bits[0],
                                       h2 ? amax_act(a, 0) : nullptr, s, ctx->channels));
        a.bits_valid[0] = true;
    }
    for (int l = 1; l <= top; ++l) {
        const int pk = pool_index_after(l - 1), pa = pool_index_after(l);
        ConvBatch b{};
        b.n = n; b.bias = ctx->bias[l]; b.Cin = kCin[l]; b.Cout = kCout[l];
        b.relu = ctx->taps.relu_of(l);
        conv_setup(ctx, b, l, false);
        b.pool_avg = ctx->pool_avg;
        double flops = 0;
        for (int k = 0; k < n; ++k) {
            ActSet& a = ctx->lv[lv[k]].acts;
            ConvImage& im = b.img[k];
            im.in = (pk >= 0) ? a.pool[pk] : a.act[l - 1];
            im.out = a.act[l]; im.H = a.h[l]; im.W = a.w[l];
            im.bits_out = a.bits[l];
            im.pool_out = (pa >= 0) ? a.pool[pa] : nullptr;
            im.pcode_out = (pa >= 0 && h2) ? a.pcode[pa] : nullptr;
            a.bits_valid[l] = a.bits[l] != nullptr;
            if (pa >= 0) a.pooled[pa] = true;
            im.amax_in = amax_act(a, l - 1); im.amax_out = amax_act(a, l);
            flops += conv_flops(im.H, im.W, b.Cin, b.Cout, 9);
        }
        {
            Timer t(ctx, s, K_CONV3, flops, b.img[0].H, b.img[0].W, b.Cin, b.Cout, 9, l);
            NSTCHK(launch_conv_batch(ctx, b, t, true));
        }
        if (l == 4 && fork_sw >= 0.f && ctx->side) {
            HIPCHK(ctx, hipEventRecord(ctx->side_fork, s));
            HIPCHK(ctx, hipStreamWaitEvent(ctx->side, ctx->side_fork, 0));
            NSTCHK(batched_gram(ctx, lv, n, fork_sw, ctx->side, 0x07u));
            HIPCHK(ctx, hipEventRecord(ctx->side_join, ctx->side));
        }
    }
    return NST_OK;
}

int batched_gram_guided(nst_ctx* ctx, const int* lv, int n, float sw, hipStream_t s) {
    GramBatch gb{};
    double flops = 0;
    auto flush = [&]() -> int {
        if (gb.n == 0) return NST_OK;
        Timer t(ctx, s, K_GRAM, flops);
        HIPCHK(ctx, launch_gram_batch(gb, s));
        gb = GramBatch{};
        flops = 0;
        return NST_OK;
    };
    for (int k = 0; k < n; ++k) {
        LevelWs& L = ctx->lv[lv[k]];
        const Guidance& g = L.guide;
        for (int q = 0; q < ctx->taps.nstyle; ++q) {
            const int l = ctx->taps.style[q];
            for (int r = 0; r < g.R; ++r) {
                if (gb.n == NST_GRAM_BATCH_MAX) NSTCHK(flush());
                const StyleTerm st = guided_term(ctx->taps, q, L.acts, sw, ctx->style_weight(q), g, r);
                GramItem& it = gb.it[gb.n++];
                it.f = L.acts.act[l]; it.N = st.N; it.C = st.C; it.amax = amax_act(L.acts, l);
                it.guide = g.plane(kScale[l], r, L.h, L.w);
                it.part = g.part + (size_t)r * g.part_floats_r + gram_part_offset(ctx->taps, L.h, L.w, q);
                it.divisor = (float)st.divisor; it.target = g.gram_t[q] + (size_t)r * st.C * st.C;
                it.coef = st.coef;
                it.gram_out = nullptr; it.S = g.S[q] + (size_t)r * st.C * st.C; it.S_bf = nullptr; it.S_amax = nullptr;
                it.mse_partial = g.partial[q] + (size_t)r * gram_finish_blocks(st.C);
                flops += 2.0 * (double)st.N * st.C * st.C;
            }
        }
    }
    NSTCHK(flush());
    for (int k = 0; k < n; ++k)
        for (int q = 0; q < ctx->taps.nstyle; ++q) NSTCHK(guided_fold(ctx, ctx->lv[lv[k]], q, s));
    return NST_OK;
}

int batched_gram(nst_ctx* ctx, const int* lv, int n, float sw, hipStream_t s, unsigned qmask) {
    const bool h2 = ctx->conv_mode == 2;
    if (guided_levels(ctx, lv, n)) return qmask ? batched_gram_guided(ctx, lv, n, sw, s) : NST_OK;
    if (h2) {
        const int per = std::max(1, NST_GRAM_BATCH_MAX / ctx->taps.nstyle);
        for (int k0 = 0; k0 < n; k0 += per) {
            GramBatch gb{};
            double flops = 0;
            for (int k = k0; k < n && k < k0 + per; ++k) {
                LevelWs& L = ctx->lv[lv[k]];
                for (int q = 0; q < ctx->taps.nstyle; ++q) {
                    if (!((qmask >> q) & 1u)) continue;
                    const int l = ctx->taps.style[q];
                    const StyleTerm st = style_term(ctx->taps, q, L.acts, sw, ctx->style_weight(q));
                    GramItem& it = gb.it[gb.n++];
                    it.f = L.acts.act[l]; it.N = st.N; it.C = st.C; it.amax = amax_act(L.acts, l);
                    it.part = L.gram_part + gram_part_offset(ctx->taps, L.h, L.w, q);
                    it.divisor = (float)st.divisor; it.target = L.gram_t[q];
                    it.coef = st.coef;
                    it.gram_out = nullptr; it.S = L.S[q]; it.S_bf = L.S_bf[q]; it.S_amax = amax_S(L.acts, q);
                    it.mse_partial = L.style_partial[q];
                    flops += 2.0 * (double)st.N * st.C * st.C;
                }
            }
            if (gb.n == 0) continue;
            Timer t(ctx, s, K_GRAM, flops);
            HIPCHK(ctx, launch_gram_batch(gb, s));
        }
    }
    for (int k = 0; k < n && !h2; ++k) {
        LevelWs& L = ctx->lv[lv[k]];
        for (int q = 0; q < ctx->taps.nstyle; ++q) {
// ... 329 lines not shown
        const LevelWs& L = ctx->lv[i];
        if (L.guide.R > 0) {
            ++guided;
            if (!L.guide.targets || L.guide.targets_R != L.guide.R)
                return fail(ctx, NST_E_STATE, "guided targets of level " + std::to_string(i) + " not set (nst_level_set_targets_guided)");
        } else {
            ++plain;
            if (!L.targets) return fail(ctx, NST_E_STATE, "targets of level " + std::to_string(i) + " not set");
        }
    }
    if (guided && plain) return fail(ctx, NST_E_STATE, "the levels of one closure are all guided or all unguided (nst_level_set_guidance)");
    return NST_OK;
}

int set_content_target(nst_ctx* ctx, int level, const float* content, hipStream_t s) {
    LevelWs& L = ctx->lv[level];
    const Taps& tp = ctx->taps;
    if (batch_eligible(ctx)) {
        const float* xi[NST_MAX_LEVELS] = {};
        xi[level] = content;
        const int lv1 = level;
        NSTCHK(batched_forward(ctx, xi, &lv1, 1, s, nullptr));
    } else {
        NSTCHK(forward(ctx, L.acts, content, L.h, L.w, s, tp.content, ctx->channels));
    }
    HIPCHK(ctx, hipMemcpyAsync(L.content_t, L.acts.act[tp.content], L.content_n * 4, hipMemcpyDeviceToDevice, s));
    return NST_OK;
}

void guidance_offsets(int R, int h, int w, size_t off[6]) {
    off[0] = 0;
    for (int sc = 0; sc < 5; ++sc) off[sc + 1] = off[sc] + (size_t)R * (h >> sc) * (w >> sc);
}
int build_guidance(nst_ctx* ctx, float* dst, const size_t* off, int R, int h, int w, double* dscratch, double mass[5][NST_MAX_REGIONS],
                   double* bad, hipStream_t s) {
    double* out = dscratch + (size_t)R * GUIDE_MASS_BLOCKS * 2;
    for (int sc = 0; sc < 5; ++sc) {
        if (sc > 0) HIPCHK(ctx, launch_guide_pool(dst + off[sc - 1], R, h >> (sc - 1), w >> (sc - 1), dst + off[sc], s));
        HIPCHK(ctx, launch_guide_mass(dst + off[sc], R, (size_t)(h >> sc) * (w >> sc), dscratch, out + (size_t)sc * R * 2, s));
    }
    double host[5 * NST_MAX_REGIONS * 2];
    HIPCHK(ctx, hipMemcpyAsync(host, out, (size_t)5 * R * 2 * sizeof(double), hipMemcpyDeviceToHost, s));
    HIPCHK(ctx, hipStreamSynchronize(s));
    *bad = 0.0;
    for (int sc = 0; sc < 5; ++sc)
        for (int r = 0; r < R; ++r) {
            mass[sc][r] = host[((size_t)sc * R + r) * 2];
            if (sc == 0) *bad += host[((size_t)sc * R + r) * 2 + 1];
        }
    return NST_OK;
}
bool guidance_mass_ok(const Taps& tp, const double mass[5][NST_MAX_REGIONS], int R) {
    for (int q = 0; q < tp.nstyle; ++q)
        for (int r = 0; r < R; ++r)
            if (!(mass[kScale[tp.style[q]]][r] >= 1.0)) return false;
    return true;
}

int window_check(nst_ctx* ctx, const float* xs, int row0, int rows, int H0) {
    if (ctx->levels != 1) return fail(ctx, NST_E_STATE, "a stripe context is configured with levels_num = 1");
    if (ctx->conv_mode != 2) return fail(ctx, NST_E_STATE, "the stripe closure runs on the f16x2 convolutions (NST_CONV unset)");
    if (!ctx->taps.is_default)
        return fail(ctx, NST_E_STATE, "the stripe closure implements the default feature maps only (nst_job_set_taps(ctx, 4, 0x2F, 1))");
    if (ctx->channels != 3)
        return fail(ctx, NST_E_STATE, "the stripe closure implements RGB only (nst_job_set_color(ctx, NST_COLOR_RGB))");
    if (ctx->pool_avg)
        return fail(ctx, NST_E_STATE, "the stripe closure implements max pooling only (nst_job_set_pooling(ctx, NST_POOL_MAX))");
    if (!ctx->unit_style_weights())
        return fail(ctx, NST_E_STATE, "the stripe closure implements unit style layer weights only (nst_job_set_style_weights)");
    LevelWs& L = ctx->lv[0];
    if (L.guide.R > 0)
        return fail(ctx, NST_E_STATE, "the stripe closure implements no spatial control (nst_level_set_guidance(ctx, 0, 0, ...) clears it)");
    if (!L.targets) return fail(ctx, NST_E_STATE, "targets of the stripe not set");
    if (!xs) return fail(ctx, NST_E_ARG, "null buffer");
    const bool to_bottom = (row0 + rows == L.h);
    if (row0 < 0 || rows < 16 || row0 % 16 || (!to_bottom && rows % 16) || row0 + rows > L.h || H0 < L.h)
        return fail(ctx, NST_E_ARG, "stripe rows: start and interior boundaries on multiples of 16 rows, inside the stripe image");
    if ((size_t)L.h * L.w * 64 * 4 >= 0xFFFFFF00ull) return fail(ctx, NST_E_ARG, "stripe image too large for the f16x2 kernels");
    return NST_OK;
}

}

extern "C" {

int nst_level_set_targets_blend(nst_ctx* ctx, int level, const float* content, int K, const float* const* styles, const int* hs,
                                const int* ws, const float* blend, void* stream) {
    if (ctx) { ++ctx->closure_epoch; ++ctx->ws_seq; }
    NSTCHK(bind(ctx));
    if (level < 0 || level >= ctx->levels) return fail(ctx, NST_E_STATE, "level not configured");
    if (K < 1 || K > NST_MAX_STYLES) return fail(ctx, NST_E_ARG, "the number of style images must be 1 .. NST_MAX_STYLES");
    if (!content || !styles || !hs || !ws || !blend) return fail(ctx, NST_E_ARG, "null argument");
    for (int k = 0; k < K; ++k) {
        if (!styles[k]) return fail(ctx, NST_E_ARG, "null image");
        if (hs[k] < 16 || ws[k] < 16) return fail(ctx, NST_E_ARG, "style image must be at least 16x16");
    }
    for (int i = 0; i < K * 6; ++i)
        if (!(blend[i] >= 0.f) || std::isinf(blend[i])) return fail(ctx, NST_E_ARG, "blend weights must be finite and >= 0");
    const Taps& tp = ctx->taps;
    float bhat[NST_MAX_STYLES][kMaxStyle] = {};
    for (int q = 0; q < tp.nstyle; ++q) {
        const int i = tap_index_of(tp.style[q]);
        double sum = 0.0;
        for (int k = 0; k < K; ++k) sum += (double)blend[k * 6 + i];
        if (!(sum > 0.0)) return fail(ctx, NST_E_ARG, "every map of the style set needs a positive blend weight of some style image");
        for (int k = 0; k < K; ++k) bhat[k][q] = (float)((double)blend[k * 6 + i] / sum);
    }
    if (K > 1 && ctx->lv[level].guide.R > 0)
        return fail(ctx, NST_E_STATE, "a guided level takes one style image (nst_level_set_targets_guided): no blend of several");
    hipStream_t s = enter(ctx, stream);
    LevelWs& L = ctx->lv[level];
    NSTCHK(set_content_target(ctx, level, content, s));
    bool written[kMaxStyle] = {};
    for (int k = 0; k < K; ++k) {
        int deepest = -1;
        for (int q = 0; q < tp.nstyle; ++q) if (bhat[k][q] > 0.f) deepest = q;
        if (deepest < 0) continue;
        Scratch sc(ctx, s);
        float* part = nullptr;
        NSTCHK(alloc_acts(ctx, sc.acts, hs[k], ws[k]));
        NSTCHK(sc.alloc(&part, gram_part_floats_for(tp, hs[k], ws[k])));
        NSTCHK(forward(ctx, sc.acts, styles[k], hs[k], ws[k], s, tp.style[deepest], ctx->channels));
        for (int q = 0; q <= deepest; ++q) {
            if (!(bhat[k][q] > 0.f)) continue;
            const int l = tp.style[q];
            const StyleTerm st = style_term(tp, q, sc.acts, 0.f, 1.f);
            const int ns = gram_nsplit(st.C, st.N);
            {
                Timer t(ctx, s, K_GRAM, 2.0 * (double)st.N * st.C * st.C);
                HIPCHK(ctx, launch_gram_partial(sc.acts.act[l], st.N, st.C, ns, ctx->conv_mode == 2 ? amax_act(sc.acts, l) : nullptr, part, s));
            }
            Timer t(ctx, s, K_OTHER, 0);
            HIPCHK(ctx, launch_gram_finish_blend(part, gram_nslabs(st.C, ns), st.C, (float)st.divisor, bhat[k][q], written[q] ? 1 : 0,
                                                 L.gram_t[q], s));
            written[q] = true;
        }
        NSTCHK(sc.finish());
    }
    L.targets = true;
    return NST_OK;
}

int nst_level_set_targets(nst_ctx* ctx, int level, const float* content, const float* style, int hs, int ws,
                          void* stream) {
    const float ones[6] = {1.f, 1.f, 1.f, 1.f, 1.f, 1.f};
    return nst_level_set_targets_blend(ctx, level, content, 1, &style, &hs, &ws, ones, stream);
}

int nst_level_set_guidance(nst_ctx* ctx, int level, int R, const float* planes, const float* lambda, void* stream) {
    if (ctx) { ++ctx->closure_epoch; ++ctx->ws_seq; }
    NSTCHK(bind(ctx));
    drop_closure_state(ctx, false);
    if (level < 0 || level >= ctx->levels) return fail(ctx, NST_E_STATE, "level not configured");
    if (R < 0 || R > NST_MAX_REGIONS) return fail(ctx, NST_E_ARG, "the number of regions must be 0 .. NST_MAX_REGIONS");
    LevelWs& L = ctx->lv[level];
    if (R == 0) {
        quiesce(ctx);
        free_guidance(ctx, L);
        return NST_OK;
    }
    if (ctx->conv_mode != 2) return fail(ctx, NST_E_STATE, "spatial control runs in the f16x2 arithmetic only (NST_CONV unset)");
    if (!planes) return fail(ctx, NST_E_ARG, "null argument");
    float lam[NST_MAX_REGIONS] = {1.f, 1.f, 1.f, 1.f};
    bool positive = lambda == nullptr;
    for (int r = 0; r < R && lambda; ++r) {
        if (!(lambda[r] >= 0.f) || std::isinf(lambda[r])) return fail(ctx, NST_E_ARG, "region weights must be finite and >= 0");
        lam[r] = lambda[r];
        positive = positive || lambda[r] > 0.f;
    }
    if (!positive) return fail(ctx, NST_E_ARG, "at least one region weight must be positive");
    hipStream_t s = enter(ctx, stream);
    const Taps& tp = ctx->taps;
    LevelWs tmp;
    Guidance& g = tmp.guide;
    auto refuse = [&](int code, const char* msg) { const int rc = msg ? fail(ctx, code, msg) : code; free_guidance(ctx, tmp); return rc; };
    auto take = [&](auto** p, size_t count) -> int {
        const int rc = dev_alloc_t(ctx, p, count);
        if (rc == NST_OK) g.bytes += std::max<size_t>(count * sizeof(**p), 16);
        return rc;
    };
    size_t off[6];
    guidance_offsets(R, L.h, L.w, off);
    g.R = R; g.plane_floats = off[5];
    for (int sc = 0; sc < 5; ++sc) g.plane_off[sc] = off[sc];
    for (int r = 0; r < NST_MAX_REGIONS; ++r) g.lambda[r] = lam[r];
    int rc = take(&g.planes, g.plane_floats);
    if (rc != NST_OK) return refuse(rc, nullptr);
    double bad = 0.0;
    {
        Scratch sc(ctx, s);
        double* dscratch = nullptr;
        rc = sc.alloc(&dscratch, ((size_t)R * GUIDE_MASS_BLOCKS + 5 * R) * 2);
        if (rc == NST_OK && hipMemcpyAsync(g.planes, planes, (size_t)R * L.h * L.w * 4, hipMemcpyDeviceToDevice, s) != hipSuccess)
            rc = fail(ctx, NST_E_HIP, "hipMemcpyAsync of the guidance planes failed");
        if (rc == NST_OK) rc = build_guidance(ctx, g.planes, off, R, L.h, L.w, dscratch, g.mass, &bad, s);
        if (rc == NST_OK) rc = sc.finish();
        if (rc != NST_OK) return refuse(rc, nullptr);
    }
    if (bad > 0.0) return refuse(NST_E_ARG, "guidance values must be finite and in [0,1]");
    if (!guidance_mass_ok(tp, g.mass, R))
        return refuse(NST_E_ARG, "a region has a mass sum t^2 below 1 on a map in use: less than one pixel's worth of guidance");
    Guidance& old = L.guide;
    if (old.R == R) {
        quiesce(ctx);
        std::swap(old.planes, g.planes);
        for (int sc = 0; sc < 5; ++sc)
            for (int r = 0; r < NST_MAX_REGIONS; ++r) old.mass[sc][r] = g.mass[sc][r];
        for (int r = 0; r < NST_MAX_REGIONS; ++r) old.lambda[r] = g.lambda[r];
        free_guidance(ctx, tmp);
        mark(ctx, s);
        return NST_OK;
    }
    g.part_floats_r = gram_part_floats_for(tp, L.h, L.w);
    rc = take(&g.part, (size_t)R * g.part_floats_r);
    for (int q = 0; q < tp.nstyle && rc == NST_OK; ++q) {
        const size_t C = (size_t)kCout[tp.style[q]];
        rc = take(&g.gram_t[q], (size_t)R * C * C);
        if (rc == NST_OK) rc = take(&g.S[q], (size_t)R * C * C);
        if (rc == NST_OK) rc = take(&g.partial[q], (size_t)R * gram_finish_blocks((int)C));
    }
    if (rc != NST_OK) return refuse(rc, nullptr);
    quiesce(ctx);
    free_guidance(ctx, L);
    L.guide = g;
    tmp.guide = Guidance();
    mark(ctx, s);
    return NST_OK;
}

int nst_level_set_targets_guided(nst_ctx* ctx, int level, const float* content, const float* style, int hs, int ws,
                                 const float* style_planes, void* stream) {
    if (ctx) { ++ctx->closure_epoch; ++ctx->ws_seq; }
    NSTCHK(bind(ctx));
    drop_closure_state(ctx, false);
    if (level < 0 || level >= ctx->levels) return fail(ctx, NST_E_STATE, "level not configured");
    LevelWs& L = ctx->lv[level];
    Guidance& g = L.guide;
    if (g.R < 1) return fail(ctx, NST_E_STATE, "the level has no guidance (nst_level_set_guidance first)");
    if (!content || !style || !style_planes) return fail(ctx, NST_E_ARG, "null argument");
    if (hs < 16 || ws < 16) return fail(ctx, NST_E_ARG, "style image must be at least 16x16");
    const Taps& tp = ctx->taps;
    const int R = g.R;
    hipStream_t s = enter(ctx, stream);
    Scratch sc(ctx, s);
    size_t off[6];
    guidance_offsets(R, hs, ws, off);
    float* sp = nullptr;
    double* dscratch = nullptr;
    double smass[5][NST_MAX_REGIONS] = {};
    double bad = 0.0;
    NSTCHK(sc.alloc(&sp, off[5]));
    NSTCHK(sc.alloc(&dscratch, ((size_t)R * GUIDE_MASS_BLOCKS + 5 * R) * 2));
    HIPCHK(ctx, hipMemcpyAsync(sp, style_planes, (size_t)R * hs * ws * 4, hipMemcpyDeviceToDevice, s));
    NSTCHK(build_guidance(ctx, sp, off, R, hs, ws, dscratch, smass, &bad, s));
    if (bad > 0.0) return fail(ctx, NST_E_ARG, "guidance values must be finite and in [0,1]");
    if (!guidance_mass_ok(tp, smass, R))
        return fail(ctx, NST_E_ARG, "a style region has a mass sum t^2 below 1 on a map in use: less than one pixel's worth of guidance");
    g.targets = false;
    NSTCHK(set_content_target(ctx, level, content, s));
    float* part = nullptr;
    NSTCHK(alloc_acts(ctx, sc.acts, hs, ws));
    NSTCHK(sc.alloc(&part, gram_part_floats_for(tp, hs, ws)));
    NSTCHK(forward(ctx, sc.acts, style, hs, ws, s, tp.style[tp.nstyle - 1], ctx->channels));
    for (int q = 0; q < tp.nstyle; ++q) {
        const int l = tp.style[q], C = kCout[l], scl = kScale[l];
        const size_t N = (size_t)sc.acts.h[l] * sc.acts.w[l];
        const int ns = gram_nsplit(C, N);
        for (int r = 0; r < R; ++r) {
            {
                Timer t(ctx, s, K_GRAM, 2.0 * (double)N * C * C);
                HIPCHK(ctx, launch_gram_partial(sc.acts.act[l], N, C, ns, amax_act(sc.acts, l), part, s, sp + off[scl] + (size_t)r * N));
            }
            Timer t(ctx, s, K_OTHER, 0);
            HIPCHK(ctx, launch_gram_finish_blend(part, gram_nslabs(C, ns), C, (float)((double)C * smass[scl][r]), 1.f, 0,
                                                 g.gram_t[q] + (size_t)r * C * C, s));
        }
    }
    NSTCHK(sc.finish());
    g.targets = true; g.targets_R = R;
    mark(ctx, s);
    return NST_OK;
}

int nst_level_guidance(const nst_ctx* ctx, int level, int* R, float* lambda, double* mass) {
    if (!ctx) return fail(nullptr, NST_E_ARG, "null context");
    if (level < 0 || level >= ctx->levels) return NST_E_STATE;
    const Guidance& g = ctx->lv[level].guide;
    if (R) *R = g.R;
    for (int r = 0; r < NST_MAX_REGIONS && lambda; ++r) lambda[r] = g.lambda[r];
    for (int sc = 0; sc < 5 && mass; ++sc)
        for (int r = 0; r < NST_MAX_REGIONS; ++r) mass[sc * NST_MAX_REGIONS + r] = r < g.R ? g.mass[sc][r] : 0.0;
    return NST_OK;
}

int nst_level_guidance_planes(nst_ctx* ctx, int level, int scale, float* out, void* stream) {
    NSTCHK(bind(ctx));
    if (level < 0 || level >= ctx->levels) return fail(ctx, NST_E_STATE, "level not configured");
    const LevelWs& L = ctx->lv[level];
    if (L.guide.R < 1) return fail(ctx, NST_E_STATE, "the level has no guidance");
    if (scale < 0 || scale > 4 || !out) return fail(ctx, NST_E_ARG, "scale must be 0 .. 4 and out not null");
    hipStream_t s = enter(ctx, stream);
    HIPCHK(ctx, hipMemcpyAsync(out, L.guide.planes + L.guide.plane_off[scale],
                               (size_t)L.guide.R * (L.h >> scale) * (L.w >> scale) * 4, hipMemcpyDeviceToDevice, s));
    mark(ctx, s);
    return NST_OK;
}

int nst_closure(nst_ctx* ctx, const float* x, float cw, float sw, float tvw, float* grad, float* losses, void* stream) {
    return nst_closure_levels(ctx, x, cw, sw, tvw, 0xFFFFFFFFu, grad, losses, stream);
}

int nst_closure_levels(nst_ctx* ctx, const float* x, float cw, float sw, float tvw, unsigned level_mask, float* grad,
                       float* losses, void* stream) {
    NSTCHK(bind(ctx));
    ++ctx->ws_seq;
    if (ctx->levels < 1) return fail(ctx, NST_E_STATE, "nst_job_configure has not been called");
    if (!x || !grad || !losses) return fail(ctx, NST_E_ARG, "null buffer");
    NSTCHK(closure_targets_check(ctx, level_mask));
    hipStream_t main = enter(ctx, stream);
    if (ctx->timing >= 2) NSTCHK(fold_timed(ctx));
    ctx->timed.clear();
    ctx->ev_used = 0;
    ctx->timed_valid = false;
    ctx->timed_backward = false;
    ctx->sample_now = (ctx->timing != 4) || ((ctx->closure_seq++ & 3) == 0);
    if (ctx->timing) HIPCHK(ctx, hipEventRecord(ctx->t0, main));

    const nst_ctx::GraphKey key{x, grad, losses, cw, sw, tvw, level_mask};
    const bool same_as_last = std::memcmp(&key, &ctx->glast, sizeof(key)) == 0;
    ctx->glast = key;
    bool done = false;
    if (ctx->use_graph && ctx->timing < 2 && batch_eligible(ctx) && same_as_last) {
        if (!ctx->gexec || std::memcmp(&key, &ctx->gkey, sizeof(key)) != 0) {
            if (ctx->gexec) { (void)hipGraphExecDestroy(ctx->gexec); ctx->gexec = nullptr; }
            hipGraph_t graph = nullptr;
            HIPCHK(ctx, hipStreamBeginCapture(ctx->gstream, hipStreamCaptureModeThreadLocal));
            const int rc = closure_record(ctx, x, cw, sw, tvw, level_mask, grad, losses, ctx->gstream);
            const hipError_t ce = hipStreamEndCapture(ctx->gstream, &graph);
            if (rc != NST_OK) { if (graph) (void)hipGraphDestroy(graph); return rc; }
            HIPCHK(ctx, ce);
            const hipError_t ie = hipGraphInstantiate(&ctx->gexec, graph, nullptr, nullptr, 0);
            (void)hipGraphDestroy(graph);
            HIPCHK(ctx, ie);
            ctx->gkey = key;
        }
        HIPCHK(ctx, hipGraphLaunch(ctx->gexec, main));
        done = true;
    }
    if (!done) NSTCHK(closure_record(ctx, x, cw, sw, tvw, level_mask, grad, losses, main));
    if (ctx->timing) { HIPCHK(ctx, hipEventRecord(ctx->t1, main)); ctx->timed_valid = true; }
    mark(ctx, main);
    return NST_OK;
}

int nst_closure_forward(nst_ctx* ctx, const float* x, float cw, float sw, float tvw, unsigned level_mask, float* losses,
                        void* stream) {
    NSTCHK(bind(ctx));
    ++ctx->ws_seq;
    ctx->fwd_token.valid = false;
    if (ctx->levels < 1) return fail(ctx, NST_E_STATE, "nst_job_configure has not been called");
    if (!x || !losses) return fail(ctx, NST_E_ARG, "null buffer");
    NSTCHK(closure_targets_check(ctx, level_mask));
// ... 114 lines not shown
```

### artstyletransfer_amd/csrc/nst_ctx.cpp

```cpp
#include <algorithm>
#include <atomic>
#include <climits>
#include <cmath>
#include <cstdint>
#include <cstdio>
#include <cstdlib>
#include <cstring>

#include "nst_ctx.h"

using namespace nst;

namespace {
thread_local std::string g_err;
}

int nst::fail(nst_ctx* ctx, int code, const std::string& msg) {
    if (ctx) ctx->err = msg; else g_err = msg;
    return code;
}

namespace {
void poison_if_asked(void* p, size_t bytes) {
    static const char* spec = getenv("NST_POISON_ALLOC");
// ... 205 lines not shown
                                const int o = ct * 128 + wn * 64 + nt * 32 + r;
                                const float* src = U.data() + ((size_t)(ky * 4 + x) * rows + o) * K + ch * 32 + ks * 16 + 8 * h;
                                uint16_t* hi_dst = out.data() + (unit0 + lane) * 8;
                                uint16_t* lo_dst = out.data() + (unit0 + 64 + lane) * 8;
                                for (int j = 0; j < 8; ++j) {
                                    const float v = src[j] * s;
                                    hi_dst[j] = f32_to_f16(v);
                                    lo_dst[j] = f32_to_f16((v - f16_to_f32(hi_dst[j])) * 2048.f);
                                }
                            }
                        }
}

void free_tap_buffers(nst_ctx* ctx, LevelWs& L) {
    auto drop = [&](void* p, size_t bytes) { if (p) { dev_free(p); if (ctx->bytes >= bytes) ctx->bytes -= bytes; } };
    drop(L.content_t, L.content_n * 4); L.content_t = nullptr; L.content_n = 0;
    for (int k = 0; k < kMaxStyle; ++k) {
        const size_t C = (size_t)L.tap_c[k];
        drop(L.gram_t[k], C * C * 4); drop(L.S[k], C * C * 4); drop(L.S_bf[k], C * C * 6);
        drop(L.style_partial[k], (size_t)gram_finish_blocks((int)std::max<size_t>(C, 1)) * 8);
        L.gram_t[k] = nullptr; L.S[k] = nullptr; L.S_bf[k] = nullptr; L.style_partial[k] = nullptr; L.tap_c[k] = 0;
    }
    drop(L.gram_part, L.gram_part_floats * 4); L.gram_part = nullptr; L.gram_part_floats = 0;
}
int alloc_tap_buffers(nst_ctx* ctx, LevelWs& L) {
    const Taps& tp = ctx->taps;
    const int m = tp.content;
    L.content_n = (size_t)L.acts.h[m] * L.acts.w[m] * kCout[m];
    NSTCHK(dev_alloc_t(ctx, &L.content_t, L.content_n));
    for (int k = 0; k < tp.nstyle; ++k) {
        const int C = kCout[tp.style[k]];
        L.tap_c[k] = C;
        NSTCHK(dev_alloc_t(ctx, &L.gram_t[k], (size_t)C * C));
        NSTCHK(dev_alloc_t(ctx, &L.S[k], (size_t)C * C));
        NSTCHK(dev_alloc_t(ctx, &L.S_bf[k], (size_t)C * C * 3));
        NSTCHK(dev_alloc_t(ctx, &L.style_partial[k], gram_finish_blocks(C)));
    }
    L.gram_part_floats = gram_part_floats_for(tp, L.h, L.w);
    NSTCHK(dev_alloc_t(ctx, &L.gram_part, L.gram_part_floats));
    return NST_OK;
}

void free_level_image(nst_ctx* ctx, LevelWs& L) {
    for (float** p : {&L.xl, &L.gxl}) {
        if (*p) { dev_free(*p); if (ctx->bytes >= L.xl_floats * 4) ctx->bytes -= L.xl_floats * 4; }
        *p = nullptr;
    }
    L.xl_floats = 0;
}
int alloc_level_image(nst_ctx* ctx, LevelWs& L) {
    L.xl_floats = (size_t)ctx->channels * L.h * L.w;
    NSTCHK(dev_alloc_t(ctx, &L.xl, L.xl_floats));
    NSTCHK(dev_alloc_t(ctx, &L.gxl, L.xl_floats));
    return NST_OK;
}

void free_level(nst_ctx* ctx, LevelWs& L) {
    free_guidance(ctx, L);
    free_acts(ctx, L.acts);
    dev_free(L.gbuf[0]); dev_free(L.gbuf[1]); dev_free(L.xl); dev_free(L.gxl);
    free_tap_buffers(ctx, L);
    dev_free(L.content_partial); dev_free(L.tv_partial); dev_free(L.tv_means);
    if (L.stream) (void)hipStreamDestroy(L.stream);
    if (L.done) (void)hipEventDestroy(L.done);
    L = LevelWs();
}

}

namespace nst {

void free_guidance(nst_ctx* ctx, LevelWs& L) {
    Guidance& g = L.guide;
    dev_free(g.planes); dev_free(g.part);
    for (int k = 0; k < kMaxStyle; ++k) { dev_free(g.gram_t[k]); dev_free(g.S[k]); dev_free(g.partial[k]); }
    if (ctx->bytes >= g.bytes) ctx->bytes -= g.bytes;
    g = Guidance();
}

void drop_closure_state(nst_ctx* ctx, bool drop_targets) {
    if (ctx->gexec) { (void)hipGraphExecDestroy(ctx->gexec); ctx->gexec = nullptr; }
    ctx->gkey = {}; ctx->glast = {};
    for (int i = 0; drop_targets && i < ctx->levels; ++i) { ctx->lv[i].targets = false; ctx->lv[i].guide.targets = false; }
}

int fold_timed(nst_ctx* ctx) {
    if (!ctx->timed_valid) return NST_OK;
    HIPCHK(ctx, hipEventSynchronize(ctx->t1));
    float ms = 0.f;
    HIPCHK(ctx, hipEventElapsedTime(&ms, ctx->t0, ctx->t1));
    ctx->acc_closure_ms += ms;
    if (!ctx->timed_backward) {
        ctx->acc_closures += 1;
        if (!ctx->timed.empty()) ctx->acc_sampled += 1;
    }
    ctx->timed_backward = false;
    for (const TimedLaunch& t : ctx->timed) {
        float d = 0.f;
        HIPCHK(ctx, hipEventSynchronize(t.b));
        HIPCHK(ctx, hipEventElapsedTime(&d, t.a, t.b));
        ctx->acc_ms[t.cls] += d;
        ctx->acc_flops[t.cls] += t.flops;
        {
            const double mode = (t.cls == K_CONV3 || t.cls == K_GRAM) ? (ctx->conv_mode == 2 ? 3.0 : ctx->conv_mode == 1 ? 6.0 : 1.0) : 1.0;
            ctx->acc_mfma[t.cls] += t.flops * (t.mfma_factor >= 0.0 ? t.mfma_factor : mode);
        }
        ctx->acc_launches[t.cls] += 1;
    }
    ctx->timed.clear();
    ctx->ev_used = 0;
    ctx->timed_valid = false;
    return NST_OK;
}

int bind(nst_ctx* ctx) {
    if (!ctx) return fail(nullptr, NST_E_ARG, "null context");
    HIPCHK(ctx, hipSetDevice(ctx->device));
    return NST_OK;
}

void mark(nst_ctx* ctx, hipStream_t s) {
    if (ctx && ctx->tail && hipEventRecord(ctx->tail, s) == hipSuccess) { ctx->tail_stream = s; ctx->tail_set = true; }
}
hipStream_t enter(nst_ctx* ctx, void* stream) {
    hipStream_t s = static_cast<hipStream_t>(stream);
    if (ctx->tail_set && s != ctx->tail_stream) (void)hipStreamWaitEvent(s, ctx->tail, 0);
    return s;
}
void quiesce(nst_ctx* ctx) {
    if (ctx->tail) (void)hipEventSynchronize(ctx->tail);
    for (int i = 0; i < NST_MAX_LEVELS; ++i)
        if (ctx->lv[i].stream) (void)hipStreamSynchronize(ctx->lv[i].stream);
    if (ctx->gstream) (void)hipStreamSynchronize(ctx->gstream);
    if (ctx->side) (void)hipStreamSynchronize(ctx->side);
}

}

namespace {

int env_flag(const char* name, int dflt) {
    const char* e = getenv(name);
    if (!e || !e[0]) return dflt;
    return std::atoi(e);
}

unsigned positive_weight_mask(const float* w) {
    unsigned m = 0;
    for (int i = 0; i < 6; ++i) if (w[i] > 0.f) m |= 1u << i;
    return m;
}
unsigned style_mask_of(const Taps& tp) {
    unsigned m = 0;
    for (int q = 0; q < tp.nstyle; ++q) m |= 1u << tap_index_of(tp.style[q]);
    return m;
}

}

extern "C" {

int nst_version(void) { return 200; }

const char* nst_last_error(const nst_ctx* ctx) { return ctx ? ctx->err.c_str() : g_err.c_str(); }

int nst_device_count(int* count) {
    if (!count) return fail(nullptr, NST_E_ARG, "count is null");
    int n = 0;
    hipError_t e = hipGetDeviceCount(&n);
    if (e != hipSuccess) { *count = 0; return fail(nullptr, NST_E_HIP, hipGetErrorString(e)); }
    *count = n;
    return NST_OK;
}

void nst_options_default(nst_options* o) {
    if (!o) return;
    o->struct_size = (int)sizeof(nst_options);
    o->conv_mode = -1; o->batched = -1; o->single_stream = -1; o->use_graph = -1; o->h2_band_rows = -1; o->lbfgs_gram = -1;
    o->h2_mfma16 = -1; o->h2_wg256 = -1; o->h2_tile_rows = -1; o->gram_overlap = -1; o->h2_persist = -1; o->level_split = -1; o->h2_winograd = -1;
}

int nst_ctx_create(int device, const float* const* weights, const float* const* biases, nst_ctx** out) {
    return nst_ctx_create_ex(device, weights, biases, nullptr, out);
}

int nst_ctx_create_ex(int device, const float* const* weights, const float* const* biases, const nst_options* opts_in,
                      nst_ctx** out) {
    if (!weights || !biases || !out) return fail(nullptr, NST_E_ARG, "null argument");
    nst_options opts;
    nst_options_default(&opts);
    if (opts_in) {
        if (opts_in->struct_size != (int)sizeof(nst_options)) return fail(nullptr, NST_E_ARG, "nst_options.struct_size mismatch (use nst_options_default)");
        opts = *opts_in;
    }
    for (int l = 0; l < NL; ++l)
        if (!weights[l] || !biases[l]) return fail(nullptr, NST_E_ARG, "null weight/bias pointer");
    int ndev = 0;
    if (hipGetDeviceCount(&ndev) != hipSuccess || ndev < 1) return fail(nullptr, NST_E_HIP, "no HIP device visible");
    if (device < 0 || device >= ndev) return fail(nullptr, NST_E_ARG, "device index out of range");
    nst_ctx* ctx = new (std::nothrow) nst_ctx();
    if (!ctx) return fail(nullptr, NST_E_NOMEM, "out of host memory");
    ctx->device = device;
    auto bail = [&](int code) { g_err = ctx->err; nst_ctx_destroy(ctx); return code; };
    if (hipSetDevice(device) != hipSuccess) { ctx->err = "hipSetDevice failed"; return bail(NST_E_HIP); }
    hipError_t e = conv_mfma_init_device();
    if (e == hipSuccess) e = conv_bf3_init_device();
    if (e == hipSuccess) e = conv_h2_init_device();
    if (e == hipSuccess) e = conv_wino_init_device();
    if (e == hipSuccess) e = gram_init_device();
    if (opts.conv_mode >= 0) {
        if (opts.conv_mode > NST_CONV_F16X2) { ctx->err = "nst_options.conv_mode must be NST_CONV_F32, NST_CONV_BF16X3 or NST_CONV_F16X2"; return bail(NST_E_ARG); }
        ctx->conv_mode = opts.conv_mode;
    } else {
        const char* cm = getenv("NST_CONV");
        if (cm && std::strcmp(cm, "f32") == 0) ctx->conv_mode = 0;
        else if (cm && std::strcmp(cm, "bf16x3") == 0) ctx->conv_mode = 1;
        else if (cm && std::strcmp(cm, "f16x2") == 0) ctx->conv_mode = 2;
        else if (cm && cm[0]) { ctx->err = "NST_CONV must be f32, bf16x3 or f16x2"; return bail(NST_E_ARG); }
    }
    ctx->batched = (opts.batched >= 0 ? opts.batched : env_flag("NST_BATCH", 1)) ? 1 : 0;
    ctx->use_graph = (opts.use_graph >= 0 ? opts.use_graph : env_flag("NST_GRAPH", 0)) ? 1 : 0;
    ctx->single_stream = (opts.single_stream >= 0 ? opts.single_stream : env_flag("NST_SINGLE_STREAM", 0)) != 0;
    ctx->band_rows = opts.h2_band_rows >= 0 ? opts.h2_band_rows : env_flag("NST_H2_BAND_ROWS", 0);
    ctx->lbfgs_gram = (opts.lbfgs_gram >= 0 ? opts.lbfgs_gram : env_flag("NST_LBFGS_GRAM", 1)) ? 1 : 0;
    ctx->mfma16 = opts.h2_mfma16 >= 0 ? opts.h2_mfma16 : env_flag("NST_H2_MFMA16", 1);
    ctx->wg256 = (opts.h2_wg256 >= 0 ? opts.h2_wg256 : env_flag("NST_H2_WG256", 0)) ? 1 : 0;
    ctx->tile_rows = opts.h2_tile_rows >= 0 ? opts.h2_tile_rows : env_flag("NST_H2_TILE_ROWS", 0);
    ctx->persist = (opts.h2_persist >= 0 ? opts.h2_persist : env_flag("NST_H2_PERSIST", 0)) ? 1 : 0;
    ctx->winograd = (opts.h2_winograd >= 0 ? opts.h2_winograd : env_flag("NST_H2_WINOGRAD", 1)) ? 1 : 0;
    ctx->level_split = (opts.level_split >= 0 ? opts.level_split : env_flag("NST_LEVEL_SPLIT", 0)) ? 1 : 0;
    ctx->gram_overlap = (opts.gram_overlap >= 0 ? opts.gram_overlap : env_flag("NST_GRAM_OVERLAP", 0)) ? 1 : 0;
    if (ctx->use_graph && hipStreamCreateWithFlags(&ctx->gstream, hipStreamNonBlocking) != hipSuccess) { ctx->err = "stream creation failed"; return bail(NST_E_HIP); }
    if (e != hipSuccess) { ctx->err = std::string("kernel attribute setup: ") + hipGetErrorString(e); return bail(NST_E_HIP); }

    std::vector<float> tmp;
    std::vector<uint16_t> tmp16;
    auto upload = [&](auto& dst, const void* src, size_t bytes, const char* what) -> int {
        if (dev_alloc(ctx, reinterpret_cast<void**>(&dst), bytes) != NST_OK) return NST_E_NOMEM;
        if (hipMemcpy(dst, src, bytes, hipMemcpyHostToDevice) != hipSuccess) { ctx->err = std::string(what) + " upload failed"; return NST_E_HIP; }
        return NST_OK;
    };
    auto pieces = [&](int rows, int K, void*& bf, void*& h2, float& h2_inv, void*& wino, float& wino_inv) -> int {
        if (ctx->conv_mode == 1) {
            make_bf3(tmp.data(), 9, rows, K, tmp16);
            return upload(bf, tmp16.data(), tmp16.size() * 2, "weight");
        }
        if (ctx->conv_mode != 2) return NST_OK;
        make_h2(tmp.data(), 9, rows, K, tmp16, &h2_inv);
        NSTCHK(upload(h2, tmp16.data(), tmp16.size() * 2, "weight"));
        if (ctx->winograd && K >= 256 && K % 64 == 0 && rows % 128 == 0) {
            make_wino(tmp.data(), rows, K, tmp16, &wino_inv);
            NSTCHK(upload(wino, tmp16.data(), tmp16.size() * 2, "weight"));
        }
        return NST_OK;
    };
    for (int l = 0; l < NL; ++l) {
        const int ci = kCin[l], co = kCout[l];
        const float* W = weights[l];
        if (int r = upload(ctx->bias[l], biases[l], co * 4, "bias")) return bail(r);
        if (l == 0) {
            tmp.assign(28 * 64, 0.f);
            for (int o = 0; o < 64; ++o)
                for (int c = 0; c < 3; ++c)
                    for (int t = 0; t < 9; ++t) tmp[(c * 9 + t) * 64 + o] = W[(o * 3 + c) * 9 + t];
            if (int r = upload(ctx->w11k, tmp.data(), tmp.size() * 4, "weight")) return bail(r);
            tmp.assign(9 * 64 * 4, 0.f);
            for (int t = 0; t < 9; ++t) {
                const int ky = 2 - t / 3, kx = 2 - t % 3;
                for (int o = 0; o < 64; ++o)
                    for (int c = 0; c < 3; ++c) tmp[(t * 64 + o) * 4 + c] = W[(o * 3 + c) * 9 + ky * 3 + kx];
            }
            if (int r = upload(ctx->w11d, tmp.data(), tmp.size() * 4, "weight")) return bail(r);
            continue;
        }
        const size_t n = (size_t)9 * ci * co;
        tmp.resize(n);
        for (int t = 0; t < 9; ++t)
            for (int o = 0; o < co; ++o)
                for (int c = 0; c < ci; ++c) tmp[((size_t)t * co + o) * ci + c] = W[((size_t)o * ci + c) * 9 + t];
        if (int r = upload(ctx->wf[l], tmp.data(), n * 4, "weight")) return bail(r);
        if (int r = pieces(co, ci, ctx->wf_bf[l], ctx->wf_h2[l], ctx->wf_h2_inv[l], ctx->wf_wino[l], ctx->wf_wino_inv[l])) return bail(r);
        for (int t = 0; t < 9; ++t) {
            const int ky = 2 - t / 3, kx = 2 - t % 3;
            for (int c = 0; c < ci; ++c)
                for (int o = 0; o < co; ++o) tmp[((size_t)t * ci + c) * co + o] = W[((size_t)o * ci + c) * 9 + ky * 3 + kx];
        }
        if (int r = upload(ctx->wd[l], tmp.data(), n * 4, "weight")) return bail(r);
        if (int r = pieces(ci, co, ctx->wd_bf[l], ctx->wd_h2[l], ctx->wd_h2_inv[l], ctx->wd_wino[l], ctx->wd_wino_inv[l])) return bail(r);
    }
    if (ctx->level_split) ctx->gram_overlap = 0;
    if ((ctx->gram_overlap || ctx->level_split) && ctx->conv_mode == 2 &&
        (hipStreamCreateWithFlags(&ctx->side, hipStreamNonBlocking) != hipSuccess ||
         hipEventCreateWithFlags(&ctx->side_fork, hipEventDisableTiming) != hipSuccess ||
         hipEventCreateWithFlags(&ctx->side_join, hipEventDisableTiming) != hipSuccess)) {
        ctx->err = "side stream creation failed";
        return bail(NST_E_HIP);
    }
    if (hipEventCreateWithFlags(&ctx->fork, hipEventDisableTiming) != hipSuccess ||
        hipEventCreateWithFlags(&ctx->tail, hipEventDisableTiming) != hipSuccess ||
        hipEventCreate(&ctx->t0) != hipSuccess || hipEventCreate(&ctx->t1) != hipSuccess) {
        ctx->err = "event creation failed";
        return bail(NST_E_HIP);
    }
    *out = ctx;
    return NST_OK;
}

void nst_ctx_destroy(nst_ctx* ctx) {
    if (!ctx) return;
    (void)hipSetDevice(ctx->device);
    quiesce(ctx);
    for (int i = 0; i < NST_MAX_LEVELS; ++i) free_level(ctx, ctx->lv[i]);
    if (ctx->tail) (void)hipEventDestroy(ctx->tail);
    for (int l = 0; l < NL; ++l) { dev_free(ctx->wf[l]); dev_free(ctx->wd[l]); dev_free(ctx->bias[l]); dev_free(ctx->wf_bf[l]); dev_free(ctx->wd_bf[l]); dev_free(ctx->wf_h2[l]); dev_free(ctx->wd_h2[l]); dev_free(ctx->wf_wino[l]); dev_free(ctx->wd_wino[l]); }
    dev_free(ctx->w11k); dev_free(ctx->w11d); dev_free(ctx->color_scratch);
    drop_closure_state(ctx, false);
    if (ctx->gstream) (void)hipStreamDestroy(ctx->gstream);
    if (ctx->side) (void)hipStreamDestroy(ctx->side);
    if (ctx->side_fork) (void)hipEventDestroy(ctx->side_fork);
    if (ctx->side_join) (void)hipEventDestroy(ctx->side_join);
    if (ctx->fork) (void)hipEventDestroy(ctx->fork);
    if (ctx->t0) (void)hipEventDestroy(ctx->t0);
    if (ctx->t1) (void)hipEventDestroy(ctx->t1);
    for (hipEvent_t e : ctx->ev_pool) (void)hipEventDestroy(e);
    delete ctx;
}

int nst_conv_mode(const nst_ctx* ctx) { return ctx ? ctx->conv_mode : -1; }

int nst_ctx_bytes(const nst_ctx* ctx, size_t* bytes) {
    if (!ctx || !bytes) return fail(nullptr, NST_E_ARG, "null argument");
    *bytes = ctx->bytes;
    return NST_OK;
}

int nst_job_configure(nst_ctx* ctx, int levels_num, int H0, int W0) {
    if (ctx) { ++ctx->closure_epoch; ++ctx->ws_seq; }
    NSTCHK(bind(ctx));
    if (levels_num < 1 || levels_num > NST_MAX_LEVELS) return fail(ctx, NST_E_ARG, "levels_num out of range");
    if ((H0 >> (levels_num - 1)) < 16 || (W0 >> (levels_num - 1)) < 16)
        return fail(ctx, NST_E_ARG, "coarsest pyramid level must be at least 16x16");
    quiesce(ctx);
    for (int i = 0; i < NST_MAX_LEVELS; ++i) free_level(ctx, ctx->lv[i]);
    drop_closure_state(ctx, false);
    ctx->levels = 0;
    int h = H0, w = W0;
    for (int i = 0; i < levels_num; ++i) {
        LevelWs& L = ctx->lv[i];
        L.h = h; L.w = w;
        NSTCHK(alloc_acts(ctx, L.acts, h, w));
        L.gbuf_floats = (size_t)h * w * 64;
        NSTCHK(dev_alloc_t(ctx, &L.gbuf[0], L.gbuf_floats));
        NSTCHK(dev_alloc_t(ctx, &L.gbuf[1], L.gbuf_floats));
        if (i > 0) NSTCHK(alloc_level_image(ctx, L));
        NSTCHK(alloc_tap_buffers(ctx, L));
        NSTCHK(dev_alloc_t(ctx, &L.content_partial, MSE_BLOCKS));
        NSTCHK(dev_alloc_t(ctx, &L.tv_partial, 2 * TV_BLOCKS));
        NSTCHK(dev_alloc_t(ctx, &L.tv_means, 2));
        h /= 2; w /= 2;
    }
    ctx->levels = levels_num;
    return NST_OK;
}

int nst_job_set_taps(nst_ctx* ctx, int content_index, unsigned style_mask, int use_relu) {
    if (ctx) { ++ctx->closure_epoch; ++ctx->ws_seq; }
    NSTCHK(bind(ctx));
    if (content_index < 0 || content_index > 5) return fail(ctx, NST_E_ARG, "content_index must be 0 .. 5");
    if (style_mask == 0u || (style_mask & ~0x3Fu) != 0u)
        return fail(ctx, NST_E_ARG, "style_mask must be a non-empty set of bits 0 .. 5");
    if (use_relu != 0 && use_relu != 1) return fail(ctx, NST_E_ARG, "use_relu must be 0 or 1");
    Taps tp;
    tp.content = kTapLayer[content_index];
    tp.nstyle = 0;
    for (int i = 0; i < 6; ++i)
        if ((style_mask >> i) & 1u) tp.style[tp.nstyle++] = kTapLayer[i];
    tp.top = std::max(tp.content, tp.style[tp.nstyle - 1]);
    tp.use_relu = use_relu;
    tp.is_default = content_index == 4 && style_mask == 0x2Fu && use_relu == 1;
    if ((style_mask & positive_weight_mask(ctx->style_w)) == 0u)
        return fail(ctx, NST_E_ARG, "no map of style_mask has a positive style layer weight (nst_job_set_style_weights)");
    quiesce(ctx);
    drop_closure_state(ctx, true);
    ctx->taps = tp;
    for (int i = 0; i < ctx->levels; ++i) {
        LevelWs& L = ctx->lv[i];
        free_guidance(ctx, L);
        free_tap_buffers(ctx, L);
        NSTCHK(alloc_tap_buffers(ctx, L));
    }
    return NST_OK;
}

int nst_job_set_color(nst_ctx* ctx, int mode) {
    if (ctx) { ++ctx->closure_epoch; ++ctx->ws_seq; }
    NSTCHK(bind(ctx));
    if (mode != NST_COLOR_RGB && mode != NST_COLOR_LUMINANCE) return fail(ctx, NST_E_ARG, "mode must be NST_COLOR_RGB or NST_COLOR_LUMINANCE");
    const int channels = mode == NST_COLOR_LUMINANCE ? 1 : 3;
    quiesce(ctx);
    float* img[NST_MAX_LEVELS][2] = {};
    int r = NST_OK;
    for (int i = 1; i < ctx->levels && r == NST_OK; ++i) {
        const size_t n = (size_t)channels * ctx->lv[i].h * ctx->lv[i].w;
        r = dev_alloc_t(ctx, &img[i][0], n);
        if (r == NST_OK) r = dev_alloc_t(ctx, &img[i][1], n);
    }
    if (r != NST_OK) {
        for (int i = 1; i < ctx->levels; ++i) {
            const size_t bytes = (size_t)channels * ctx->lv[i].h * ctx->lv[i].w * 4;
            for (float* p : img[i])
                if (p) { dev_free(p); if (ctx->bytes >= bytes) ctx->bytes -= bytes; }
        }
        return r;
    }
    drop_closure_state(ctx, true);
    ctx->channels = channels;
    for (int i = 1; i < ctx->levels; ++i) {
        LevelWs& L = ctx->lv[i];
        free_level_image(ctx, L);
        L.xl = img[i][0]; L.gxl = img[i][1];
        L.xl_floats = (size_t)channels * L.h * L.w;
    }
    return NST_OK;
}

int nst_job_color(const nst_ctx* ctx) { return ctx ? (ctx->channels == 1 ? NST_COLOR_LUMINANCE : NST_COLOR_RGB) : -1; }

int nst_job_set_pooling(nst_ctx* ctx, int mode) {
    if (ctx) { ++ctx->closure_epoch; ++ctx->ws_seq; }
    NSTCHK(bind(ctx));
    if (mode != NST_POOL_MAX && mode != NST_POOL_AVG) return fail(ctx, NST_E_ARG, "mode must be NST_POOL_MAX or NST_POOL_AVG");
    quiesce(ctx);
    drop_closure_state(ctx, true);
    ctx->pool_avg = mode == NST_POOL_AVG ? 1 : 0;
    return NST_OK;
}

int nst_job_pooling(const nst_ctx* ctx) { return ctx ? (ctx->pool_avg ? NST_POOL_AVG : NST_POOL_MAX) : -1; }

int nst_job_set_style_weights(nst_ctx* ctx, const float* w) {
    if (ctx) { ++ctx->closure_epoch; ++ctx->ws_seq; }
    NSTCHK(bind(ctx));
    if (!w) return fail(ctx, NST_E_ARG, "null argument");
    for (int i = 0; i < 6; ++i)
        if (!(w[i] >= 0.f) || std::isinf(w[i])) return fail(ctx, NST_E_ARG, "style layer weights must be finite and >= 0");
    if ((style_mask_of(ctx->taps) & positive_weight_mask(w)) == 0u)
        return fail(ctx, NST_E_ARG, "at least one map of the current style set needs a positive style layer weight");
    quiesce(ctx);
    drop_closure_state(ctx, false);
    for (int i = 0; i < 6; ++i) ctx->style_w[i] = w[i];
    return NST_OK;
}

int nst_job_style_weights(const nst_ctx* ctx, float* w) {
    if (!ctx || !w) return fail(nullptr, NST_E_ARG, "null argument");
    for (int i = 0; i < 6; ++i) w[i] = ctx->style_w[i];
    return NST_OK;
}

int nst_set_timing(nst_ctx* ctx, int enabled) {
    NSTCHK(bind(ctx));
    ctx->timing = enabled;
    if (enabled >= 2 && ctx->ev_pool.empty()) {
        ctx->ev_pool.resize(2048);
        for (auto& e : ctx->ev_pool) HIPCHK(ctx, hipEventCreate(&e));
    }
    return NST_OK;
}

int nst_last_closure_ms(nst_ctx* ctx, float* ms) {
    NSTCHK(bind(ctx));
    if (!ms) return fail(ctx, NST_E_ARG, "null argument");
    *ms = 0.f;
    if (!ctx->timed_valid) return NST_OK;
    HIPCHK(ctx, hipEventSynchronize(ctx->t1));
    HIPCHK(ctx, hipEventElapsedTime(ms, ctx->t0, ctx->t1));
    return NST_OK;
}

int nst_last_closure_class(nst_ctx* ctx, int cls, float* ms, int* launches, double* flops) {
    NSTCHK(bind(ctx));
    if (!ms || !launches || !flops || cls < 0 || cls >= K_NCLASS) return fail(ctx, NST_E_ARG, "bad argument");
    *ms = 0.f; *launches = 0; *flops = 0.0;
    if (!ctx->timed_valid) return NST_OK;
    HIPCHK(ctx, hipEventSynchronize(ctx->t1));
    for (const TimedLaunch& t : ctx->timed) {
        if (t.cls != cls) continue;
        float d = 0.f;
        HIPCHK(ctx, hipEventSynchronize(t.b));
        HIPCHK(ctx, hipEventElapsedTime(&d, t.a, t.b));
        *ms += d; *launches += 1; *flops += t.flops;
    }
    return NST_OK;
}

int nst_last_closure_launches(nst_ctx* ctx, nst_launch_info* out, int capacity, int* count) {
    NSTCHK(bind(ctx));
    if (!count || capacity < 0 || (capacity > 0 && !out)) return fail(ctx, NST_E_ARG, "bad argument");
    *count = ctx->timed_valid ? (int)ctx->timed.size() : 0;
    for (int i = 0; i < *count && i < capacity; ++i) {
        const TimedLaunch& t = ctx->timed[i];
        const H2Shape& sh = t.shape;
        out[i] = nst_launch_info{t.cls, t.tag[0], t.tag[1], t.tag[2], t.tag[3], t.tag[5], sh.rows, sh.bn, sh.ntw, sh.chunk,
                                 sh.m16, sh.persist, sh.second, sh.unpool, sh.bands};
    }
    return NST_OK;
}

int nst_dump_last_closure(nst_ctx* ctx) {
    NSTCHK(bind(ctx));
    if (!ctx->timed_valid) return NST_OK;
    HIPCHK(ctx, hipEventSynchronize(ctx->t1));
    for (const TimedLaunch& t : ctx->timed) {
        float d = 0.f;
        HIPCHK(ctx, hipEventSynchronize(t.b));
        HIPCHK(ctx, hipEventElapsedTime(&d, t.a, t.b));
        char shape[64] = "";
        if (t.shape.rows > 0)
            snprintf(shape, sizeof(shape), "  h2<%d,%d,%d,%d>%s%s x%d", t.shape.rows, t.shape.bn, t.shape.ntw, t.shape.chunk,
                     t.shape.m16 ? " m16" : "", t.shape.persist ? " persist" : "", t.shape.bands);
        fprintf(stderr, "cls %d  %4dx%-4d cin %3d cout %3d taps %d layer %3d  %8.3f ms  %7.2f TFLOP/s%s\n", t.cls, t.tag[0],
                t.tag[1], t.tag[2], t.tag[3], t.tag[4], t.tag[5], d, d > 0 ? t.flops / (d * 1e-3) / 1e12 : 0.0, shape);
    }
    return NST_OK;
}

int nst_timing_totals(nst_ctx* ctx, int cls, double* ms, long* launches, double* flops, int reset) {
    NSTCHK(bind(ctx));
    if (!ms || !launches || !flops || cls < -2 || cls >= K_NCLASS) return fail(ctx, NST_E_ARG, "bad argument");
    NSTCHK(fold_timed(ctx));
    if (cls == -2) { *ms = 0; *launches = ctx->acc_sampled; *flops = 0; }
    else if (cls < 0) { *ms = ctx->acc_closure_ms; *launches = ctx->acc_closures; *flops = 0; }
    else { *ms = ctx->acc_ms[cls]; *launches = ctx->acc_launches[cls]; *flops = ctx->acc_flops[cls]; }
    if (reset) {
        for (int i = 0; i < 4; ++i) { ctx->acc_ms[i] = 0; ctx->acc_flops[i] = 0; ctx->acc_mfma[i] = 0; ctx->acc_launches[i] = 0; }
        ctx->acc_closure_ms = 0; ctx->acc_closures = 0; ctx->acc_sampled = 0;
    }
    return NST_OK;
}

int nst_timing_mfma_flops(nst_ctx* ctx, int cls, double* mfma_flops) {
    NSTCHK(bind(ctx));
    if (!mfma_flops || cls < 0 || cls >= K_NCLASS) return fail(ctx, NST_E_ARG, "bad argument");
    NSTCHK(fold_timed(ctx));
    *mfma_flops = ctx->acc_mfma[cls];
    return NST_OK;
}

int nst_internal_device(const nst_ctx* ctx) { return ctx ? ctx->device : 0; }
int nst_internal_levels(const nst_ctx* ctx) { return ctx ? ctx->levels : 0; }
int nst_internal_channels(const nst_ctx* ctx) { return ctx ? ctx->channels : 3; }
size_t nst_internal_pixels(const nst_ctx* ctx) { return (ctx && ctx->levels > 0) ? (size_t)ctx->lv[0].h * ctx->lv[0].w : 0; }
int nst_internal_fail(nst_ctx* ctx, int code, const char* msg) { return fail(ctx, code, msg ? msg : ""); }
void nst_internal_poison(void* p, size_t bytes) { poison_if_asked(p, bytes); }
int nst_internal_lbfgs_gram(const nst_ctx* ctx) { return ctx ? ctx->lbfgs_gram : 1; }
unsigned long long nst_internal_closure_epoch(const nst_ctx* ctx) { return ctx ? ctx->closure_epoch : 0; }
void nst_internal_mark(nst_ctx* ctx, void* stream) { mark(ctx, static_cast<hipStream_t>(stream)); }

}
```

### artstyletransfer_amd/csrc/nst_ctx.h

```cpp
#pragma once
#include <hip/hip_runtime.h>

#include <string>
#include <vector>

#include "../../include/nst_hip.h"
#include "nst_kernels.h"

#pragma GCC visibility push(hidden)
namespace nst {

constexpr int NL = NST_VGG19_CONVS;
constexpr int kCin[NL] = {3, 64, 64, 128, 128, 256, 256, 256, 256, 512, 512, 512, 512};
constexpr int kCout[NL] = {64, 64, 128, 128, 256, 256, 256, 256, 512, 512, 512, 512, 512};
constexpr int kScale[NL] = {0, 0, 1, 1, 2, 2, 2, 2, 3, 3, 3, 3, 4};
constexpr int kPoolAfter[4] = {1, 3, 7, 11};
constexpr int kTapLayer[6] = {0, 2, 4, 8, 9, 12};
constexpr int kMaxStyle = 6;
inline int tap_index_of(int layer) {
    for (int i = 0; i < 6; ++i) if (kTapLayer[i] == layer) return i;
    return -1;
}
inline int pool_index_after(int l) {
    for (int k = 0; k < 4; ++k) if (kPoolAfter[k] == l) return k;
    return -1;
}

struct ActSet {
    int h[NL], w[NL];
    float* act[NL] = {};
    float* pool[4] = {};
    float* splitk = nullptr;
    size_t splitk_floats = 0;
    unsigned* bits[NL] = {};
    bool bits_valid[NL] = {};
    bool pooled[4] = {};
    unsigned* amax = nullptr;
    unsigned* pcode[4] = {};
    size_t bytes = 0;
    void begin_pass() {
        for (int l = 0; l < NL; ++l) bits_valid[l] = false;
        for (int k = 0; k < 4; ++k) pooled[k] = false;
    }
};
constexpr int AMAX_IDS = 2 * NST_VGG19_CONVS + kMaxStyle;
inline unsigned* amax_act(const ActSet& a, int l) { return a.amax + (size_t)l * NST_AMAX_SLOTS; }
inline unsigned* amax_S(const ActSet& a, int q) { return a.amax + (size_t)(NST_VGG19_CONVS + q) * NST_AMAX_SLOTS; }
inline unsigned* amax_grad(const ActSet& a, int l) { return a.amax + (size_t)(NST_VGG19_CONVS + kMaxStyle + l) * NST_AMAX_SLOTS; }

struct Taps {
    int content = 9;
    int style[kMaxStyle] = {0, 2, 4, 8, 12};
    int nstyle = 5;
    int top = 12;
    int use_relu = 1;
    bool is_default = true;
    int style_slot(int l) const {
        for (int q = 0; q < nstyle; ++q) if (style[q] == l) return q;
        return -1;
    }
    int relu_of(int l) const { return (l == NL - 1 && !use_relu) ? 0 : 1; }
    bool top_mask() const { return use_relu || top != NST_VGG19_CONVS - 1; }
};

enum KClass { K_CONV3 = 0, K_GRAM = 1, K_CONV1 = 2, K_OTHER = 3, K_NCLASS = 4 };

struct TimedLaunch { hipEvent_t a, b; int cls; double flops; int tag[6]; double mfma_factor; H2Shape shape; };

struct Guidance {
    int R = 0;
    float lambda[NST_MAX_REGIONS] = {1.f, 1.f, 1.f, 1.f};
    float* planes = nullptr;
    size_t plane_off[5] = {};
    size_t plane_floats = 0;
    double mass[5][NST_MAX_REGIONS] = {};
    float* gram_t[kMaxStyle] = {};
    float* S[kMaxStyle] = {};
    double* partial[kMaxStyle] = {};
    float* part = nullptr;
    size_t part_floats_r = 0;
    bool targets = false;
    int targets_R = 0;
    size_t bytes = 0;
    const float* plane(int scale, int r, int h, int w) const { return planes + plane_off[scale] + (size_t)r * (h >> scale) * (w >> scale); }
};

struct LevelWs {
    int h = 0, w = 0;
    Guidance guide;
    ActSet acts;
    float* gbuf[2] = {};
    size_t gbuf_floats = 0;
    float* xl = nullptr;
    float* gxl = nullptr;
    size_t xl_floats = 0;
    float* content_t = nullptr;
    size_t content_n = 0;
    float* gram_t[kMaxStyle] = {};
    float* S[kMaxStyle] = {};
    unsigned short* S_bf[kMaxStyle] = {};
    float* gram_part = nullptr;
    size_t gram_part_floats = 0;
    double* style_partial[kMaxStyle] = {};
    int tap_c[kMaxStyle] = {};
    double* content_partial = nullptr;
    double* tv_partial = nullptr;
    float* tv_means = nullptr;
    bool targets = false;
    hipStream_t stream = nullptr;
    hipEvent_t done = nullptr;
};

}

struct nst_ctx {
    int device = 0;
    std::string err;
    float* wf[nst::NL] = {};
    float* wd[nst::NL] = {};
    void* wf_bf[nst::NL] = {};
    void* wd_bf[nst::NL] = {};
    void* wd_wino[nst::NL] = {};
    float wd_wino_inv[nst::NL] = {};
    void* wf_wino[nst::NL] = {};
    float wf_wino_inv[nst::NL] = {};
    int winograd = 0;
    void* wf_h2[nst::NL] = {};
    void* wd_h2[nst::NL] = {};
    float wf_h2_inv[nst::NL] = {};
    float wd_h2_inv[nst::NL] = {};
    int conv_mode = 2;
    int band_rows = 0;
    int lbfgs_gram = 1;
    int mfma16 = 1;
    int wg256 = 0;
    int tile_rows = 0;
    int gram_overlap = 0;
    int persist = 1;
    int level_split = 0;
    hipStream_t side = nullptr;
    hipEvent_t side_fork = nullptr, side_join = nullptr;
    hipStream_t tail_stream = nullptr;
    bool tail_set = false;
    hipEvent_t tail = nullptr;
    int batched = 1;
    int use_graph = 0;
    hipStream_t gstream = nullptr;
    hipGraphExec_t gexec = nullptr;
    struct GraphKey { const float* x; float* grad; float* losses; float cw, sw, tvw; unsigned mask; } gkey{}, glast{};
    float* bias[nst::NL] = {};
    float* w11k = nullptr;
    float* w11d = nullptr;
    int levels = 0;
    nst::Taps taps;
    int channels = 3;
    int pool_avg = 0;
    float style_w[6] = {1.f, 1.f, 1.f, 1.f, 1.f, 1.f};
    float style_weight(int q) const { return style_w[nst::tap_index_of(taps.style[q])]; }
    bool unit_style_weights() const {
        for (float w : style_w) if (w != 1.f) return false;
        return true;
    }
    unsigned long long closure_epoch = 0;
    unsigned long long ws_seq = 0;
    struct ForwardToken {
        bool valid = false;
        const float* x = nullptr;
        float cw = 0.f, sw = 0.f, tvw = 0.f;
        unsigned mask = 0;
        unsigned long long epoch = 0, seq = 0;
    } fwd_token;
    double* color_scratch = nullptr;
    nst::LevelWs lv[NST_MAX_LEVELS];
    hipEvent_t fork = nullptr;
    size_t bytes = 0;
    bool single_stream = false;
    int timing = 0;
    hipEvent_t t0 = nullptr, t1 = nullptr;
    std::vector<hipEvent_t> ev_pool;
    size_t ev_used = 0;
    std::vector<nst::TimedLaunch> timed;
    bool timed_valid = false;
    bool timed_backward = false;
    double acc_ms[4] = {0, 0, 0, 0};
    double acc_flops[4] = {0, 0, 0, 0};
    double acc_mfma[4] = {0, 0, 0, 0};
    long acc_launches[4] = {0, 0, 0, 0};
    double acc_closure_ms = 0;
    long acc_closures = 0;
    long acc_sampled = 0;
    long closure_seq = 0;
    bool sample_now = true;
};

namespace nst {

int fail(nst_ctx* ctx, int code, const std::string& msg);

#define HIPCHK(ctx, expr)                                                                         \
    do {                                                                                          \
        hipError_t _e = (expr);                                                                   \
        if (_e != hipSuccess)                                                                     \
            return fail(ctx, NST_E_HIP, std::string(#expr) + ": " + hipGetErrorString(_e));       \
    } while (0)

#define NSTCHK(expr)                 \
    do {                             \
        int _r = (expr);             \
        if (_r != NST_OK) return _r; \
    } while (0)

struct Timer {
    nst_ctx* ctx; hipStream_t s; bool on; size_t slot;
    Timer(nst_ctx* c, hipStream_t st, int cls, double flops, int t0 = 0, int t1 = 0, int t2 = 0, int t3 = 0, int t4 = 0,
          int t5 = 0)
        : ctx(c), s(st), on(false), slot(0) {
        if (c->timing >= 2 && (c->timing < 3 || cls == K_CONV3) && c->sample_now && c->ev_used + 2 <= c->ev_pool.size()) {
            on = true;
            TimedLaunch t{c->ev_pool[c->ev_used], c->ev_pool[c->ev_used + 1], cls, flops, {t0, t1, t2, t3, t4, t5}, -1.0, H2Shape{}};
            c->ev_used += 2;
            slot = c->timed.size();
            c->timed.push_back(t);
            (void)hipEventRecord(t.a, st);
        }
    }
    ~Timer() { if (on) (void)hipEventRecord(ctx->timed[slot].b, s); }
    void mfma_factor(double f) { if (on) ctx->timed[slot].mfma_factor = f; }
    void shape(const H2Shape& sh) { if (on) ctx->timed[slot].shape = sh; }
};
int fold_timed(nst_ctx* ctx);

int dev_alloc(nst_ctx* ctx, void** p, size_t bytes);
template <typename T>
int dev_alloc_t(nst_ctx* ctx, T** p, size_t count) { return dev_alloc(ctx, reinterpret_cast<void**>(p), count * sizeof(T)); }
inline void dev_free(void* p) { if (p) (void)hipFree(p); }
int alloc_acts(nst_ctx* ctx, ActSet& a, int h, int w);
void free_acts(nst_ctx* ctx, ActSet& a);
int bind(nst_ctx* ctx);
void drop_closure_state(nst_ctx* ctx, bool drop_targets);
void free_guidance(nst_ctx* ctx, LevelWs& L);
hipStream_t enter(nst_ctx* ctx, void* stream);
void mark(nst_ctx* ctx, hipStream_t s);
void quiesce(nst_ctx* ctx);

struct Scratch {
    nst_ctx* ctx; hipStream_t s; ActSet acts; std::vector<void*> bufs; bool open = true;
    Scratch(nst_ctx* c, hipStream_t st) : ctx(c), s(st) {}
    Scratch(const Scratch&) = delete;
    ~Scratch() { (void)release(); }
    template <typename T>
    int alloc(T** p, size_t count) {
        NSTCHK(dev_alloc_t(ctx, p, count));
        bufs.push_back(*p);
        return NST_OK;
    }
    hipError_t release() {
        if (!open) return hipSuccess;
        open = false;
        const hipError_t e = hipStreamSynchronize(s);
        free_acts(ctx, acts);
        for (void* p : bufs) dev_free(p);
        return e;
    }
    int finish() { const hipError_t e = release(); HIPCHK(ctx, e); return NST_OK; }
};

struct Inject {
    const float* S = nullptr;
    const void* S_bf = nullptr;
    const unsigned* S_amax = nullptr;
    const float* direct = nullptr;
    bool content = false;
    const GuidedBwd* guided = nullptr;
};
struct ContentJob { const float* target; size_t n; float coef; double* partial; };
int forward(nst_ctx* ctx, ActSet& a, const float* x, int h, int w, hipStream_t s, int last_layer = NL - 1, int channels = 3);
int backward(nst_ctx* ctx, ActSet& a, const Inject* inj, const ContentJob* cj, float* gbuf0, float* gbuf1, float* gx,
             int h, int w, hipStream_t s, int top = NL - 1, bool top_mask = true, int channels = 3);
int gram_of(nst_ctx* ctx, const float* f_nhwc, size_t N, int C, const unsigned* f_amax, float divisor, float* part, const float* target,
            float coef, float* gram_out, float* S, unsigned short* S_bf, unsigned* S_amax, double* mse_partial,
            hipStream_t s);
size_t gram_part_floats_for(const Taps& tp, int h, int w);

}
#pragma GCC visibility pop
```

### artstyletransfer_amd/engine.py

```python
from __future__ import annotations

import ctypes as C
from typing import List, Optional, Sequence, Tuple

import numpy as np
import torch

from . import _lib
from . import taps as _taps
from .pooling_modes import check_pooling
from . import style_modes as _style
from . import regions as _regions
from ._lib import NST_LOSS_ROW, NstError, StepInfo

TAP_CHANNELS = (64, 128, 256, 512, 512, 512)
TAP_SCALE = (0, 1, 2, 3, 3, 4)
DEFAULT_TAPS = (_taps.DEFAULT_CONTENT_INDEX, _taps.DEFAULT_STYLE_INDICES, True)


def _ptr(t: Optional[torch.Tensor]):
    return C.c_void_p(t.data_ptr()) if t is not None else C.c_void_p(0)


def _stream(device) -> C.c_void_p:
    return C.c_void_p(torch.cuda.current_stream(device).cuda_stream)


def _chk_dev(t: torch.Tensor, device, shape=None):
    if not (t.is_cuda and t.dtype == torch.float32 and t.is_contiguous()):
        raise NstError("expected a contiguous float32 CUDA tensor")
    if t.device != device:
        raise NstError(f"tensor is on {t.device}, context on {device}")
    if shape is not None and tuple(t.shape) != tuple(shape):
        raise NstError(f"expected shape {tuple(shape)}, got {tuple(t.shape)}")


class StyleEngine:

    def __init__(self, weights: Sequence[Tuple[torch.Tensor, torch.Tensor]], device: int | str | torch.device = 0,
                 conv_mode: Optional[str] = None, batched: Optional[bool] = None, single_stream: Optional[bool] = None,
                 use_graph: Optional[bool] = None, h2_band_rows: Optional[int] = None, lbfgs_gram: Optional[bool] = None,
                 h2_mfma16: Optional[bool] = None, h2_wg256: Optional[bool] = None,
                 h2_tile_rows: Optional[int] = None, gram_overlap: Optional[bool] = None,
                 h2_persist: Optional[bool] = None, level_split: Optional[bool] = None,
                 h2_winograd: Optional[bool] = None):
        self.lib = _lib.load()
        if not torch.cuda.is_available():
            raise NstError("no GPU visible: the style-transfer hot path runs only on the HIP device")
        self.device = torch.device(device if not isinstance(device, int) else f"cuda:{device}")
        if self.device.type != "cuda":
            raise NstError("StyleEngine needs a cuda (HIP) device; there is no CPU fallback")
        idx = self.device.index if self.device.index is not None else torch.cuda.current_device()
        self.device = torch.device("cuda", idx)
        if len(weights) != _lib.NST_VGG19_CONVS:
            raise NstError("expected 13 (weight, bias) pairs conv1_1..conv5_1")
        ws = [np.ascontiguousarray(w.detach().cpu().numpy(), dtype=np.float32) for w, _ in weights]
        bs = [np.ascontiguousarray(b.detach().cpu().numpy(), dtype=np.float32) for _, b in weights]
        wp = (C.c_void_p * 13)(*[a.ctypes.data for a in ws])
        bp = (C.c_void_p * 13)(*[a.ctypes.data for a in bs])
        opts = _lib.Options()
        self.lib.nst_options_default(C.byref(opts))
        if conv_mode is not None:
            if conv_mode not in _lib.CONV_MODES:
                raise NstError(f"conv_mode must be one of {sorted(_lib.CONV_MODES)}")
            opts.conv_mode = _lib.CONV_MODES[conv_mode]
        for name, val in (("batched", batched), ("single_stream", single_stream), ("use_graph", use_graph),
                          ("h2_band_rows", h2_band_rows), ("lbfgs_gram", lbfgs_gram), ("h2_mfma16", h2_mfma16),
                          ("h2_wg256", h2_wg256), ("h2_tile_rows", h2_tile_rows),
                          ("gram_overlap", gram_overlap), ("h2_persist", h2_persist), ("level_split", level_split), ("h2_winograd", h2_winograd)):
            if val is not None:
                setattr(opts, name, int(val))
        ctx = C.c_void_p()
        _lib.check(None, self.lib.nst_ctx_create_ex(idx, wp, bp, C.byref(opts), C.byref(ctx)), "nst_ctx_create_ex")
        self.ctx = ctx
        self.weights_id = id(weights)
        self.levels = 0
        self.shape = None
        self.taps = DEFAULT_TAPS
        self.channels = 3
        self.pooling = "max"
        self.layer_weights = _style.UNIT_WEIGHTS

    def close(self):
        if getattr(self, "ctx", None):
            self.lib.nst_ctx_destroy(self.ctx)
            self.ctx = None

    def __del__(self):
        try:
            self.close()
        except Exception:
            pass

    def configure(self, levels_num: int, H0: int, W0: int) -> None:
        _lib.check(self.ctx, self.lib.nst_job_configure(self.ctx, levels_num, H0, W0), "nst_job_configure")
        self.levels = levels_num
        self.shape = (H0, W0)

    def set_taps(self, content_index, style_indices, use_relu: bool = True) -> None:
        content, style = _taps.normalize_taps(content_index, style_indices, use_relu)
        _lib.check(self.ctx, self.lib.nst_job_set_taps(self.ctx, content, _taps.style_mask(style), int(use_relu)),
                   "nst_job_set_taps")
        self.taps = (content, style, bool(use_relu))

    def reset_taps(self) -> None:
        if self.taps != DEFAULT_TAPS:
            self.set_taps(*DEFAULT_TAPS)

    def set_color(self, mode) -> None:
        if mode not in (None, "rgb", "luminance"):
            raise ValueError(f"colour mode must be 'rgb' or 'luminance', not {mode!r}")
        lum = mode == "luminance"
        try:
            _lib.check(self.ctx, self.lib.nst_job_set_color(self.ctx, _lib.NST_COLOR_LUMINANCE if lum else _lib.NST_COLOR_RGB),
                       "nst_job_set_color")
        finally:
            self.channels = 1 if self.lib.nst_job_color(self.ctx) == _lib.NST_COLOR_LUMINANCE else 3

    def reset_color(self) -> None:
        if self.channels != 3:
            self.set_color("rgb")

    def set_pooling(self, mode) -> None:
        check_pooling(mode)
        try:
            _lib.check(self.ctx, self.lib.nst_job_set_pooling(self.ctx, _lib.NST_POOL_AVG if mode == "avg" else _lib.NST_POOL_MAX),
                       "nst_job_set_pooling")
        finally:
            self.pooling = "avg" if self.lib.nst_job_pooling(self.ctx) == _lib.NST_POOL_AVG else "max"

    def reset_pooling(self) -> None:
        if self.pooling != "max":
            self.set_pooling("max")

    def set_style_weights(self, w) -> None:
        w = _style.check_style_layer_weights(w, style_indices=self.taps[1])
        arr = (C.c_float * _style.NUM_MAPS)(*w)
        try:
            _lib.check(self.ctx, self.lib.nst_job_set_style_weights(self.ctx, arr), "nst_job_set_style_weights")
        finally:
            self.layer_weights = self.style_weights()

    def style_weights(self) -> Tuple[float, ...]:
        arr = (C.c_float * _style.NUM_MAPS)()
        _lib.check(self.ctx, self.lib.nst_job_style_weights(self.ctx, arr), "nst_job_style_weights")
        return tuple(float(v) for v in arr)

    def reset_style_weights(self) -> None:
        if self.layer_weights != _style.UNIT_WEIGHTS:
            self.set_style_weights(_style.UNIT_WEIGHTS)

    def release_job(self) -> None:
        self.configure(1, 16, 16)

    def level_shape(self, level: int) -> Tuple[int, int]:
        h, w = self.shape
        return h >> level, w >> level
# ... 193 lines not shown

    def bytes(self) -> int:
        n = C.c_size_t()
        _lib.check(self.ctx, self.lib.nst_ctx_bytes(self.ctx, C.byref(n)), "nst_ctx_bytes")
        return n.value

    def set_timing(self, mode: int) -> None:
        _lib.check(self.ctx, self.lib.nst_set_timing(self.ctx, mode), "nst_set_timing")

    def last_closure_ms(self) -> float:
        ms = C.c_float()
        _lib.check(self.ctx, self.lib.nst_last_closure_ms(self.ctx, C.byref(ms)), "nst_last_closure_ms")
        return ms.value

    def last_closure_class(self, cls: int):
        ms, n, fl = C.c_float(), C.c_int(), C.c_double()
        _lib.check(self.ctx, self.lib.nst_last_closure_class(self.ctx, cls, C.byref(ms), C.byref(n), C.byref(fl)),
                   "nst_last_closure_class")
        return ms.value, n.value, fl.value

    def last_closure_launches(self) -> List[dict]:
        n = C.c_int()
        _lib.check(self.ctx, self.lib.nst_last_closure_launches(self.ctx, None, 0, C.byref(n)), "nst_last_closure_launches")
        buf = (_lib.LaunchInfo * max(n.value, 1))()
        _lib.check(self.ctx, self.lib.nst_last_closure_launches(self.ctx, buf, n.value, C.byref(n)), "nst_last_closure_launches")
        return [{name: getattr(buf[i], name) for name, _ in _lib.LaunchInfo._fields_} for i in range(n.value)]

    def timing_totals(self, cls: int, reset: bool = False):
        ms, n, fl = C.c_double(), C.c_long(), C.c_double()
        _lib.check(self.ctx, self.lib.nst_timing_totals(self.ctx, cls, C.byref(ms), C.byref(n), C.byref(fl),
                                                        int(reset)), "nst_timing_totals")
        return ms.value, n.value, fl.value

    def timing_mfma_flops(self, cls: int) -> float:
        fl = C.c_double()
        _lib.check(self.ctx, self.lib.nst_timing_mfma_flops(self.ctx, cls, C.byref(fl)), "nst_timing_mfma_flops")
        return fl.value

    def vgg_features(self, x: torch.Tensor) -> List[torch.Tensor]:
        x = x.reshape(3, x.shape[-2], x.shape[-1])
        _chk_dev(x, self.device)
        h, w = x.shape[1], x.shape[2]
        outs = [torch.empty((1, c, h >> s, w >> s), dtype=torch.float32, device=self.device)
                for c, s in zip(TAP_CHANNELS, TAP_SCALE)]
        arr = (C.c_void_p * 6)(*[o.data_ptr() for o in outs])
        _lib.check(self.ctx, self.lib.nst_vgg_features(self.ctx, _ptr(x), h, w, arr, _stream(self.device)),
                   "nst_vgg_features")
        return outs

    def vgg_features_backward(self, x: torch.Tensor, gouts: Sequence[Optional[torch.Tensor]]) -> torch.Tensor:
        x = x.reshape(3, x.shape[-2], x.shape[-1])
        _chk_dev(x, self.device)
        h, w = x.shape[1], x.shape[2]
        for g in gouts:
            if g is not None:
                _chk_dev(g, self.device)
        arr = (C.c_void_p * 6)(*[(g.data_ptr() if g is not None else 0) for g in gouts])
        gx = torch.empty((1, 3, h, w), dtype=torch.float32, device=self.device)
        _lib.check(self.ctx, self.lib.nst_vgg_features_backward(self.ctx, _ptr(x), h, w, arr, _ptr(gx),
                                                                _stream(self.device)), "nst_vgg_features_backward")
        return gx

    LAYER_CHANNELS = (64, 64, 128, 128, 256, 256, 256, 256, 512, 512, 512, 512, 512)
    LAYER_SCALE = (0, 0, 1, 1, 2, 2, 2, 2, 3, 3, 3, 3, 4)

    def vgg_activations(self, x: torch.Tensor) -> List[torch.Tensor]:
        x = x.reshape(3, x.shape[-2], x.shape[-1])
        _chk_dev(x, self.device)
        h, w = x.shape[1], x.shape[2]
        outs = [torch.empty((1, c, h >> sc, w >> sc), dtype=torch.float32, device=self.device)
                for c, sc in zip(self.LAYER_CHANNELS, self.LAYER_SCALE)]
        arr = (C.c_void_p * 13)(*[o.data_ptr() for o in outs])
        _lib.check(self.ctx, self.lib.nst_vgg_activations(self.ctx, _ptr(x), h, w, arr, _stream(self.device)),
                   "nst_vgg_activations")
        return outs

    def level_activation(self, level: int, layer: int) -> torch.Tensor:
        h, w = self.level_shape(level)
        c, sc = self.LAYER_CHANNELS[layer], self.LAYER_SCALE[layer]
        t = torch.empty((1, c, h >> sc, w >> sc), dtype=torch.float32, device=self.device)
        _lib.check(self.ctx, self.lib.nst_level_activation(self.ctx, level, layer, _ptr(t), _stream(self.device)),
                   "nst_level_activation")
        return t

    def level_image(self, level: int) -> torch.Tensor:
        h, w = self.level_shape(level)
        t = torch.empty((1, self.channels, h, w), dtype=torch.float32, device=self.device)
        _lib.check(self.ctx, self.lib.nst_level_image(self.ctx, level, _ptr(t), _stream(self.device)), "nst_level_image")
        return t

    def level_activations(self, level: int) -> List[torch.Tensor]:
        h, w = self.level_shape(level)
        outs = []
        for l, (c, sc) in enumerate(zip(self.LAYER_CHANNELS, self.LAYER_SCALE)):
            t = torch.empty((1, c, h >> sc, w >> sc), dtype=torch.float32, device=self.device)
            _lib.check(self.ctx, self.lib.nst_level_activation(self.ctx, level, l, _ptr(t), _stream(self.device)),
                       "nst_level_activation")
            outs.append(t)
        return outs

    def gram(self, f: torch.Tensor, normalize: bool = True) -> torch.Tensor:
        _chk_dev(f, self.device)
        b, c, h, w = f.shape
        assert b == 1
        g = torch.empty((1, c, c), dtype=torch.float32, device=self.device)
        _lib.check(self.ctx, self.lib.nst_gram(self.ctx, _ptr(f), c, h, w, int(normalize), _ptr(g),
                                               _stream(self.device)), "nst_gram")
        return g

    def guided_gram_backward(self, f: torch.Tensor, planes: torch.Tensor, s_mats: torch.Tensor, addend: Optional[torch.Tensor] = None,
                             relu_bits: Optional[torch.Tensor] = None, out: Optional[torch.Tensor] = None, want_absmax: bool = False):
        n, c = f.shape
        r = planes.shape[0]
        if tuple(planes.shape) != (r, n) or tuple(s_mats.shape) != (r, c, c):
            raise NstError("planes must be (R,N) and s_mats (R,C,C)")
        if out is None:
            out = torch.empty((n, c), dtype=torch.float32, device=self.device)
        slots = torch.empty(64, dtype=torch.int32, device=self.device) if want_absmax else None
        for t in (f, planes, s_mats, addend, out):
            if t is not None:
                _chk_dev(t, self.device)
        if relu_bits is not None and not (relu_bits.is_cuda and relu_bits.dtype == torch.int32 and relu_bits.is_contiguous()
                                          and tuple(relu_bits.shape) == (n, c // 32)):
            raise NstError(f"relu_bits must be a contiguous int32 CUDA tensor of shape ({n},{c // 32})")
        if (addend is not None and addend.shape != f.shape) or out.shape != f.shape:
            raise NstError("addend and out must have the shape of f")
        _lib.check(self.ctx, self.lib.nst_guided_gram_backward(self.ctx, _ptr(f), n, c, r, _ptr(planes), _ptr(s_mats), _ptr(addend),
                                                               _ptr(relu_bits), _ptr(out), _ptr(slots), _stream(self.device)),
                   "nst_guided_gram_backward")
        return (out, slots.view(torch.float32).max()) if want_absmax else out

    def total_variation(self, y: torch.Tensor, want_grad: bool = False):
        _chk_dev(y, self.device)
        b, c, h, w = y.shape
        val = torch.empty(1, dtype=torch.float32, device=self.device)
        grad = torch.empty_like(y) if want_grad else None
        _lib.check(self.ctx, self.lib.nst_total_variation(self.ctx, _ptr(y), b * c, h, w, _ptr(val), _ptr(grad),
                                                          _stream(self.device)), "nst_total_variation")
        return (val, grad) if want_grad else val

    def bicubic_half(self, x: torch.Tensor) -> torch.Tensor:
        _chk_dev(x, self.device)
        b, c, h, w = x.shape
        y = torch.empty((b, c, h // 2, w // 2), dtype=torch.float32, device=self.device)
        _lib.check(self.ctx, self.lib.nst_bicubic_half(self.ctx, _ptr(x), b * c, h, w, _ptr(y), _stream(self.device)),
                   "nst_bicubic_half")
        return y

    def bicubic_half_backward(self, gy: torch.Tensor, h: int, w: int) -> torch.Tensor:
        _chk_dev(gy, self.device)
        b, c = gy.shape[0], gy.shape[1]
        gx = torch.empty((b, c, h, w), dtype=torch.float32, device=self.device)
        _lib.check(self.ctx, self.lib.nst_bicubic_half_backward(self.ctx, _ptr(gy), b * c, h, w, _ptr(gx),
                                                                _stream(self.device)), "nst_bicubic_half_backward")
        return gx

    def prepare_img(self, hwc: torch.Tensor) -> torch.Tensor:
        _chk_dev(hwc, self.device)
        h, w, _ = hwc.shape
        out = torch.empty((1, 3, h, w), dtype=torch.float32, device=self.device)
        _lib.check(self.ctx, self.lib.nst_prepare_img(self.ctx, _ptr(hwc), h, w, _ptr(out), _stream(self.device)),
                   "nst_prepare_img")
        return out

    def unprepare_img(self, chw: torch.Tensor) -> torch.Tensor:
        _chk_dev(chw, self.device)
# ... 310 lines not shown
```

### include/nst_hip.h

```cpp
#ifndef NST_HIP_H
#define NST_HIP_H

#include <stddef.h>
#include <stdint.h>

#ifdef __cplusplus
extern "C" {
#endif

#define NST_OK 0
#define NST_E_ARG (-1)
#define NST_E_STATE (-2)
#define NST_E_HIP (-3)
#define NST_E_NOMEM (-4)
#define NST_E_UNAVAILABLE (-5)

#define NST_VGG19_CONVS 13
#define NST_MAX_LEVELS 8
#define NST_LOSS_ROW 4
#define NST_MAX_STYLES 8
#define NST_MAX_REGIONS 4

typedef struct nst_ctx nst_ctx;
typedef struct nst_opt nst_opt;
// ... 39 lines not shown
int nst_job_color(const nst_ctx* ctx);

#define NST_POOL_MAX 0
#define NST_POOL_AVG 1
int nst_job_set_pooling(nst_ctx* ctx, int mode);
int nst_job_pooling(const nst_ctx* ctx);

int nst_job_set_style_weights(nst_ctx* ctx, const float w[6]);
int nst_job_style_weights(const nst_ctx* ctx, float w[6]);

int nst_level_set_targets(nst_ctx* ctx, int level, const float* content, const float* style,
                          int hs, int ws, void* stream);

int nst_level_set_targets_blend(nst_ctx* ctx, int level, const float* content, int K, const float* const* styles,
                                const int* hs, const int* ws, const float* blend , void* stream);

int nst_level_set_guidance(nst_ctx* ctx, int level, int R, const float* planes ,
                           const float* lambda , void* stream);
int nst_level_set_targets_guided(nst_ctx* ctx, int level, const float* content, const float* style, int hs, int ws,
                                 const float* style_planes , void* stream);
int nst_level_guidance(const nst_ctx* ctx, int level, int* R, float lambda[NST_MAX_REGIONS], double mass[5 * NST_MAX_REGIONS]);
int nst_level_guidance_planes(nst_ctx* ctx, int level, int scale, float* out, void* stream);

int nst_closure(nst_ctx* ctx, const float* x, float content_weight, float style_weight,
                float tv_weight, float* grad, float* losses, void* stream);

int nst_closure_levels(nst_ctx* ctx, const float* x, float content_weight, float style_weight,
                       float tv_weight, unsigned level_mask, float* grad, float* losses, void* stream);

int nst_closure_forward(nst_ctx* ctx, const float* x, float content_weight, float style_weight, float tv_weight,
                        unsigned level_mask, float* losses, void* stream);
int nst_closure_backward(nst_ctx* ctx, const float* x, float content_weight, float style_weight, float tv_weight,
                         unsigned level_mask, float* grad, void* stream);

#define NST_OPT_ADAM 0
#define NST_OPT_LBFGS 1
int nst_opt_create(nst_ctx* ctx, int kind, float lr_start, int lbfgs_max_eval, nst_opt** out);
void nst_opt_destroy(nst_opt* opt);

typedef struct nst_step_info {
    int closures;
    int total_closures;
    int accepted;
    float loss;
    float lr;
    float t;
    int history;
} nst_step_info;

int nst_opt_step(nst_opt* opt, float* x, float content_weight, float style_weight, float tv_weight,
                 float* losses_host, int closures_capacity, nst_step_info* info, void* stream);

typedef void (*nst_reduce_hook)(void* user);
int nst_opt_shard_levels(nst_opt* opt, unsigned level_mask, float* grad, float* losses, nst_reduce_hook hook,
                         void* user);

int nst_opt_shard_levels_comm(nst_opt* opt, unsigned level_mask, nst_comm* comm);

int nst_opt_history(const nst_opt* opt, int* pairs, int* n_iter);

int nst_opt_set_closure_reuse(nst_opt* opt, int enabled);
int nst_opt_closure_stats(const nst_opt* opt, long* evaluated, long* served);

int nst_opt_set_lazy_backward(nst_opt* opt, int enabled);
int nst_opt_backward_stats(const nst_opt* opt, long* forward_only, long* skipped);

#define NST_COMM_ID_BYTES 128
int nst_comm_unique_id(void* id);
int nst_comm_create(int device, int rank, int world, const void* id, nst_comm** out);
void nst_comm_destroy(nst_comm* comm);
int nst_comm_info(const nst_comm* comm, int* rank, int* world, long* calls, double* bytes);
int nst_comm_allreduce_sum(nst_comm* comm, float* buf, size_t n, void* stream);

int nst_adam_step(nst_ctx* ctx, float* x, const float* g, float* m, float* v, size_t n, int k, double lr, void* stream);
int nst_lbfgs_direction(nst_ctx* ctx, const float* g, const float* const* y, const float* const* s, const float* ro, int m,
                        float h_diag, size_t n, int form, float* d, void* stream);


int nst_vgg_features(nst_ctx* ctx, const float* x, int h, int w, float* const* outs, void* stream);
int nst_vgg_activations(nst_ctx* ctx, const float* x, int h, int w, float* const* outs, void* stream);
int nst_vgg_features_backward(nst_ctx* ctx, const float* x, int h, int w, const float* const* gouts,
                              float* gx, void* stream);
int nst_level_activation(nst_ctx* ctx, int level, int layer, float* out, void* stream);
int nst_level_image(nst_ctx* ctx, int level, float* out, void* stream);
int nst_gram(nst_ctx* ctx, const float* f, int C, int h, int w, int normalize, float* gram, void* stream);
int nst_guided_gram_backward(nst_ctx* ctx, const float* f, size_t N, int C, int R, const float* planes, const float* S,
                             const float* addend, const unsigned* relu_bits, float* out, unsigned* amax_slots, void* stream);
int nst_total_variation(nst_ctx* ctx, const float* y, int C, int h, int w, float* value, float* grad,
                        void* stream);
int nst_bicubic_half(nst_ctx* ctx, const float* x, int C, int h, int w, float* y, void* stream);
int nst_bicubic_half_backward(nst_ctx* ctx, const float* gy, int C, int h, int w, float* gx, void* stream);
int nst_prepare_img(nst_ctx* ctx, const float* hwc, int h, int w, float* chw, void* stream);
int nst_unprepare_img(nst_ctx* ctx, const float* chw, int h, int w, float* hwc, void* stream);


int nst_resize_bicubic(nst_ctx* ctx, const float* src, int h, int w, int channels, float* dst, int nh, int nw, void* stream);
int nst_gather_rows(nst_ctx* ctx, const float* src, const long long* perm, size_t rows, int channels, float* dst, void* stream);
int nst_gaussian_mask_accumulate(nst_ctx* ctx, float* acc, const float* src, int h, int w, int channels, double central,
                                 double peripheral, double dispersion, void* stream);
int nst_noise_blend(nst_ctx* ctx, const float* content, const float* noise, int h, int w, int channels, double noise_factor,
                    float* out, void* stream);
int nst_scale(nst_ctx* ctx, const float* src, float alpha, size_t n, float* dst, void* stream);

int nst_color_stats(nst_ctx* ctx, const float* hwc, int h, int w, double* mean, double* cov, void* stream);
int nst_color_transfer_matrix(const double* mean_c, const double* cov_c, const double* mean_s, const double* cov_s, double* A,
                              double* b);
int nst_color_affine(nst_ctx* ctx, const float* src, int h, int w, const double* A, const double* b, float* dst, void* stream);
int nst_luminance(nst_ctx* ctx, const float* hwc, int h, int w, double alpha, double beta, float* out, void* stream);
int nst_luminance_recombine(nst_ctx* ctx, const float* u, const float* content, int h, int w, float* out, void* stream);

int nst_window_sums_count(size_t* count);
int nst_window_begin(nst_ctx* ctx, const float* xs, int row0, int rows, int H0, float* sums, void* stream);
int nst_window_end(nst_ctx* ctx, const float* xs, int row0, int rows, int H0, float content_weight, float style_weight,
                   float tv_weight, float* sums, float* gxs, float* losses, void* stream);

int nst_conv_mode(const nst_ctx* ctx);

int nst_ctx_bytes(const nst_ctx* ctx, size_t* bytes);

int nst_set_timing(nst_ctx* ctx, int enabled);
int nst_last_closure_ms(nst_ctx* ctx, float* ms);
int nst_last_closure_class(nst_ctx* ctx, int cls, float* ms, int* launches, double* flops);
int nst_timing_totals(nst_ctx* ctx, int cls, double* ms, long* launches, double* flops, int reset);
int nst_timing_mfma_flops(nst_ctx* ctx, int cls, double* mfma_flops);
typedef struct nst_launch_info {
    int cls;
    int h, w, cin, cout;
    int layer;
    int h2_rows, h2_bn, h2_ntw, h2_chunk;
    int h2_mfma16;
    int h2_persist;
    int h2_second, h2_unpool;
    int h2_bands;
} nst_launch_info;
int nst_last_closure_launches(nst_ctx* ctx, nst_launch_info* out, int capacity, int* count);
int nst_dump_last_closure(nst_ctx* ctx);

#ifdef __cplusplus
}
#endif
#endif
```

Baseline: 448.1 iters/s.

## Skip storing full-resolution conv maps that feed only a pooling layer

In the h2 batched forward, conv layers whose output goes straight into a pool now write only the pooled map, pool codes and ReLU bits, not the full-resolution activation. This removes the large f32 store traffic for those maps. The skipped maps are tracked per pass, and if a caller later asks for one, it is rebuilt by re-running that conv layer. A keep_all_maps option and graph mode keep the old behaviour, at the cost of extra bookkeeping and an invalidation path when targets or levels change.

After: 460.0 iters/s (median of 6 runs). 1.03x the previous value.

```diff
diff --git a/artstyletransfer_amd/_lib.py b/artstyletransfer_amd/_lib.py
--- a/artstyletransfer_amd/_lib.py
+++ b/artstyletransfer_amd/_lib.py
@@ -105,6 +105,9 @@
     "nst_vgg_features_backward": (C.c_int, [c_void, c_void, C.c_int, C.c_int, C.POINTER(c_void), c_void, c_void]),
     "nst_vgg_activations": (C.c_int, [c_void, c_void, C.c_int, C.c_int, C.POINTER(c_void), c_void]),
     "nst_level_activation": (C.c_int, [c_void, C.c_int, C.c_int, c_void, c_void]),
+    "nst_job_map_stats": (C.c_int, [c_void, C.c_int, C.POINTER(C.c_uint)]),
+    "nst_ctx_set_keep_all_maps": (C.c_int, [c_void, C.c_int]),
+    "nst_ctx_keep_all_maps": (C.c_int, [c_void]),
     "nst_level_image": (C.c_int, [c_void, C.c_int, c_void, c_void]),
     "nst_gram": (C.c_int, [c_void, c_void, C.c_int, C.c_int, C.c_int, C.c_int, c_void, c_void]),
     "nst_guided_gram_backward": (C.c_int, [c_void, c_void, C.c_size_t, C.c_int, C.c_int, c_void, c_void, c_void, c_void, c_void,
diff --git a/artstyletransfer_amd/csrc/conv_h2.hip b/artstyletransfer_amd/csrc/conv_h2.hip
--- a/artstyletransfer_amd/csrc/conv_h2.hip
+++ b/artstyletransfer_amd/csrc/conv_h2.hip
@@ -680,6 +680,7 @@
                 const int ppix0 = ((y0 + wm * 4) >> 1) * PW2 + ((x0 + 4 * kg) >> 1);
                 const unsigned pbase = (unsigned)ppix0 * (unsigned)colB + (unsigned)(cg0 + l15) * 4u;
                 const unsigned cbase = (l15 == 0) ? ((unsigned)ppix0 * (unsigned)words + (unsigned)(cg0 >> 5)) * 16u : 0xFFFFFF00u;
+                const bool full = UNPOOL || p.out != nullptr;
 #pragma unroll
                 for (int nt = 0; nt < NT16; ++nt) {
                     const float bv = p.bias ? p.bias[cg0 + nt * 16 + l15] : 0.f;
@@ -690,7 +691,7 @@
                             float v = fmaf(ax16[mt][nt][i], LO_DOWN, am16[mt][nt][i]) * inv + bv;
                             v = fmaxf(v, lo_clamp);
                             am16[mt][nt][i] = v;
-                            __builtin_amdgcn_raw_buffer_store_b32(__builtin_bit_cast(unsigned, v), rs_out, vbase, mt * rowB + i * colB + nt * 64, 0);
+                            if (full) __builtin_amdgcn_raw_buffer_store_b32(__builtin_bit_cast(unsigned, v), rs_out, vbase, mt * rowB + i * colB + nt * 64, 0);
                             amax = fmaxf(amax, fabsf(v));
                         }
                 }
@@ -772,7 +773,7 @@
                     }
                     am16[mt][nt][i] = v;
                     if (inb) {
-                        p.out[idx] = v;
+                        if (UNPOOL || p.out) p.out[idx] = v;
                         amax = fmaxf(amax, fabsf(v));
                     }
                 }
@@ -921,6 +922,7 @@
             const unsigned pbase = (unsigned)ppix0 * (unsigned)colB + (unsigned)(cg0 + l31) * 4u;
             const unsigned cbase = (l31 == 0) ? ((unsigned)ppix0 * (unsigned)words + (unsigned)(cg0 >> 5)) * 16u : 0xFFFFFF00u;
             const float lo_clamp = p.relu ? 0.f : -__builtin_inff();
+            const bool full = UNPOOL || p.out != nullptr;
 #pragma unroll
             for (int nt = 0; nt < NTW; ++nt) {
                 const float bv = p.bias ? p.bias[cg0 + nt * 32 + l31] : 0.f;
@@ -931,7 +933,7 @@
                         float v = fmaf(accx[mt][nt][r], LO_DOWN, accm[mt][nt][r]) * inv + bv;
                         v = fmaxf(v, lo_clamp);
                         accm[mt][nt][r] = v;
-                        __builtin_amdgcn_raw_buffer_store_b32(__builtin_bit_cast(unsigned, v), rs_out, vbase, soff(mt, r, rowB, colB) + nt * 128, 0);
+                        if (full) __builtin_amdgcn_raw_buffer_store_b32(__builtin_bit_cast(unsigned, v), rs_out, vbase, soff(mt, r, rowB, colB) + nt * 128, 0);
                         amax = fmaxf(amax, fabsf(v));
                         if (p.bits_out) {
                             const unsigned long long bal = __ballot(v > 0.f);
@@ -1003,7 +1005,7 @@
                 }
                 accm[mt][nt][r] = v;
                 if (inb) {
-                    p.out[idx] = v;
+                    if (UNPOOL || p.out) p.out[idx] = v;
                     amax = fmaxf(amax, fabsf(v));
                 }
             }
@@ -1263,6 +1265,7 @@
             return hipErrorInvalidValue;
         if ((size_t)im.H * im.W * (b.Cin > b.Cin2 ? b.Cin : b.Cin2) * 4 >= 0xFFFFFF00ull) return hipErrorInvalidValue;
         if ((b.unpool != 0) != (im.pcode_in != nullptr)) return hipErrorInvalidValue;
+        if (!im.out && !im.pool_out) return hipErrorInvalidValue;
         H[i] = im.H; W[i] = im.W;
         second = second || (im.in2 != nullptr);
     }
@@ -1285,6 +1288,7 @@
 hipError_t launch_conv_h2(const ConvParams& p0, hipStream_t stream, H2Shape* shape) {
     if (!h2_operands_ok(p0.wt_h2, p0.amax_in, p0.Cin, p0.Cout, p0.in2, p0.wt2_f32, p0.amax_in2, p0.amax_w2, p0.Cin2))
         return hipErrorInvalidValue;
+    if (!p0.out && !p0.pool_out) return hipErrorInvalidValue;
     ConvParams p = p0;
     p.ksplit = 1;
     int all_blocks = 0;
@@ -1311,7 +1315,7 @@
         if (q.pcode_in) { q.in += pp0 * p.Cin; q.pcode_in += pp0 * wi * 4; }
         else if (q.in) q.in += px0 * p.Cin;
         if (q.in2) { q.in2 += px0 * p.Cin2; if (q.in2_rows > 0) q.in2_row0 -= b0; }
-        q.out += px0 * p.Cout;
+        if (q.out) q.out += px0 * p.Cout;
         if (q.addend) q.addend += px0 * p.Cout;
         if (q.mask) q.mask += px0 * p.Cout;
         if (q.bits_in) q.bits_in += px0 * wo;
diff --git a/artstyletransfer_amd/csrc/conv_wino.hip b/artstyletransfer_amd/csrc/conv_wino.hip
--- a/artstyletransfer_amd/csrc/conv_wino.hip
+++ b/artstyletransfer_amd/csrc/conv_wino.hip
@@ -318,6 +318,7 @@
     unsigned* const e_pcode_out = M_FWD ? im.pcode_out : nullptr;
     const float* const e_addend = M_BWD ? im.addend : nullptr;
     const unsigned* const e_bits_in = M_BWD ? im.bits_in : nullptr;
+    const bool e_full = M_FWD ? im.out != nullptr : true;
     float* E = reinterpret_cast<float*>(smem);
     unsigned* WB = reinterpret_cast<unsigned*>(smem + W_BITS_OFF);
     unsigned* PC = reinterpret_cast<unsigned*>(smem + W_CODE_OFF);
@@ -385,8 +386,10 @@
                 if (ina) amax = fmaxf(amax, fabsf(ya[e]));
                 if (inb) amax = fmaxf(amax, fabsf(yb[e]));
             }
-            if (ina) *reinterpret_cast<f32x4*>(im.out + pa * Cout + co) = ya;
-            if (inb) *reinterpret_cast<f32x4*>(im.out + (pa + 1) * Cout + co) = yb;
+            if (e_full) {
+                if (ina) *reinterpret_cast<f32x4*>(im.out + pa * Cout + co) = ya;
+                if (inb) *reinterpret_cast<f32x4*>(im.out + (pa + 1) * Cout + co) = yb;
+            }
             if (e_bits_out) {
                 const int pix = yy * 16 + 2 * p;
                 const unsigned wa = or8(na << sh), wb = or8(nb << sh);
@@ -478,6 +481,7 @@
         const ConvImage& im = b.img[i];
         if (im.in2 || im.mask || !im.amax_in || (b.unpool != 0) != (im.pcode_in != nullptr)) return false;
         if (im.pcode_out && !im.pool_out) return false;
+        if (!im.out && !im.pool_out) return false;
         if ((size_t)im.H * im.W * (b.Cin > b.Cout ? b.Cin : b.Cout) * 4 >= 0xFFFFFF00ull) return false;
     }
     return true;
diff --git a/artstyletransfer_amd/csrc/nst_api.cpp b/artstyletransfer_amd/csrc/nst_api.cpp
--- a/artstyletransfer_amd/csrc/nst_api.cpp
+++ b/artstyletransfer_amd/csrc/nst_api.cpp
@@ -95,9 +95,13 @@
     if (layer < 0 || layer >= NL || !out) return fail(ctx, NST_E_ARG, "bad argument");
     const ActSet& a = ctx->lv[level].acts;
     hipStream_t s = enter(ctx, stream);
-    HIPCHK(ctx, launch_hwc_to_chw(a.act[layer], kCout[layer], a.h[layer], a.w[layer], out, s));
+    const int rc = restore_map(ctx, level, layer, s);
+    if (rc == NST_OK && launch_hwc_to_chw(a.act[layer], kCout[layer], a.h[layer], a.w[layer], out, s) != hipSuccess) {
+        mark(ctx, s);
+        return fail(ctx, NST_E_HIP, "hwc_to_chw launch failed");
+    }
     mark(ctx, s);
-    return NST_OK;
+    return rc;
 }
 
 int nst_level_image(nst_ctx* ctx, int level, float* out, void* stream) {
diff --git a/artstyletransfer_amd/csrc/nst_closure.cpp b/artstyletransfer_amd/csrc/nst_closure.cpp
--- a/artstyletransfer_amd/csrc/nst_closure.cpp
+++ b/artstyletransfer_amd/csrc/nst_closure.cpp
@@ -49,17 +49,18 @@
     b.wt_h2 = dgrad ? ctx->wd_h2[l] : ctx->wf_h2[l]; b.wt_h2_inv = dgrad ? ctx->wd_h2_inv[l] : ctx->wf_h2_inv[l];
     b.wt_wino = dgrad ? ctx->wd_wino[l] : ctx->wf_wino[l]; b.wt_wino_inv = dgrad ? ctx->wd_wino_inv[l] : ctx->wf_wino_inv[l];
 }
-int launch_conv_batch(nst_ctx* ctx, const ConvBatch& b, Timer& t, bool allow_wino) {
+int launch_conv_batch(nst_ctx* ctx, const ConvBatch& b, hipStream_t s, Timer* t, bool allow_wino) {
     const bool h2 = ctx->conv_mode == 2;
-    if (h2 && allow_wino && b.wt_wino && conv_wino_eligible(b)) { t.mfma_factor(2.0); HIPCHK(ctx, launch_conv_wino_batch(b, t.s)); }
+    if (h2 && allow_wino && b.wt_wino && conv_wino_eligible(b)) { if (t) t->mfma_factor(2.0); HIPCHK(ctx, launch_conv_wino_batch(b, s)); }
     else if (h2) {
         H2Shape sh{};
-        const hipError_t e = launch_conv_h2_batch(b, t.s, &sh);
-        t.shape(sh);
+        const hipError_t e = launch_conv_h2_batch(b, s, &sh);
+        if (t) t->shape(sh);
         HIPCHK(ctx, e);
-    } else HIPCHK(ctx, launch_conv_bf3_batch(b, t.s));
-    return NST_OK;
-}
+    } else HIPCHK(ctx, launch_conv_bf3_batch(b, s));
+    return NST_OK;
+}
+int launch_conv_batch(nst_ctx* ctx, const ConvBatch& b, Timer& t, bool allow_wino) { return launch_conv_batch(ctx, b, t.s, &t, allow_wino); }
 
 hipError_t launch_pool_fwd(const nst_ctx* ctx, const float* in, int H, int W, int C, float* out, hipStream_t s) {
     return (ctx->pool_avg ? launch_avgpool_fwd : launch_maxpool_fwd)(in, H, W, C, out, s);
@@ -76,6 +77,17 @@
     return {C, N, chw, (float)((double)sw * (double)w * 4.0 / ((double)tp.nstyle * (double)C * C * chw))};
 }
 float content_coef(float cw, double n) { return (float)((double)cw * 2.0 / n); }
+
+constexpr bool taps_avoid_pools() {
+    for (int t : kTapLayer)
+        for (int p : kPoolAfter) if (t == p) return false;
+    return true;
+}
+static_assert(taps_avoid_pools(), "a map in front of a pooling layer became a tap: map_stored must keep it where a job reads it");
+bool map_stored(const nst_ctx* ctx, int l) {
+    if (ctx->conv_mode != 2 || ctx->keep_all_maps || ctx->use_graph) return true;
+    return pool_index_after(l) < 0;
+}
 
 size_t gram_part_offset(const Taps& tp, int h, int w, int k) {
     size_t off = 0;
@@ -130,6 +142,8 @@
         HIPCHK(ctx, launch_conv1_1_fwd(x, h, w, ctx->w11k, ctx->bias[0], a.act[0], bits, h2 ? amax_act(a, 0) : nullptr, s, channels));
         a.bits_valid[0] = bits != nullptr;
     }
+    a.pass = 0;
+    for (int l = 0; l <= last_layer; ++l) a.stored[l] = true;
     for (int l = 1; l <= last_layer; ++l) {
         const int pk = pool_index_after(l - 1);
         const float* in = (pk >= 0) ? a.pool[pk] : a.act[l - 1];
@@ -298,6 +312,31 @@
 constexpr size_t kWinScalarOff = 64 * 64 + 128 * 128 + 256 * 256 + 2 * 512 * 512;
 constexpr size_t kWinSums = kWinScalarOff + 4;
 
+ConvBatch forward_batch(nst_ctx* ctx, const int* lv, int n, int l, bool full, double* flops) {
+    const bool h2 = ctx->conv_mode == 2;
+    const int pk = pool_index_after(l - 1), pa = pool_index_after(l);
+    ConvBatch b{};
+    b.n = n; b.bias = ctx->bias[l]; b.Cin = kCin[l]; b.Cout = kCout[l];
+    b.relu = ctx->taps.relu_of(l);
+    conv_setup(ctx, b, l, false);
+    b.pool_avg = ctx->pool_avg;
+    for (int k = 0; k < n; ++k) {
+        ActSet& a = ctx->lv[lv[k]].acts;
+        ConvImage& im = b.img[k];
+        im.in = (pk >= 0) ? a.pool[pk] : a.act[l - 1];
+        im.out = full ? a.act[l] : nullptr; im.H = a.h[l]; im.W = a.w[l];
+        im.bits_out = a.bits[l];
+        im.pool_out = (pa >= 0) ? a.pool[pa] : nullptr;
+        im.pcode_out = (pa >= 0 && h2) ? a.pcode[pa] : nullptr;
+        a.bits_valid[l] = a.bits[l] != nullptr;
+        a.stored[l] = full;
+        if (pa >= 0) a.pooled[pa] = true;
+        im.amax_in = amax_act(a, l - 1); im.amax_out = amax_act(a, l);
+        *flops += conv_flops(im.H, im.W, b.Cin, b.Cout, 9);
+    }
+    return b;
+}
+
 int batched_gram(nst_ctx* ctx, const int* lv, int n, float sw, hipStream_t s, unsigned qmask);
 int batched_forward(nst_ctx* ctx, const float* const* xi, const int* lv, int n, hipStream_t s, const Window* win, float fork_sw = -1.f) {
     const bool h2 = ctx->conv_mode == 2;
@@ -315,28 +354,17 @@
         HIPCHK(ctx, launch_conv1_1_fwd(xi[lv[k]], L.h, L.w, ctx->w11k, ctx->bias[0], a.act[0], a.bits[0],
                                        h2 ? amax_act(a, 0) : nullptr, s, ctx->channels));
         a.bits_valid[0] = true;
+        a.stored[0] = true;
+    }
+    ++ctx->fwd_pass;
+    for (int k = 0; k < n; ++k) {
+        ActSet& a = ctx->lv[lv[k]].acts;
+        a.pass = ctx->fwd_pass; a.pass_n = n;
+        for (int j = 0; j < n; ++j) a.pass_lv[j] = lv[j];
     }
     for (int l = 1; l <= top; ++l) {
-        const int pk = pool_index_after(l - 1), pa = pool_index_after(l);
-        ConvBatch b{};
-        b.n = n; b.bias = ctx->bias[l]; b.Cin = kCin[l]; b.Cout = kCout[l];
-        b.relu = ctx->taps.relu_of(l);
-        conv_setup(ctx, b, l, false);
-        b.pool_avg = ctx->pool_avg;
         double flops = 0;
-        for (int k = 0; k < n; ++k) {
-            ActSet& a = ctx->lv[lv[k]].acts;
-            ConvImage& im = b.img[k];
-            im.in = (pk >= 0) ? a.pool[pk] : a.act[l - 1];
-            im.out = a.act[l]; im.H = a.h[l]; im.W = a.w[l];
-            im.bits_out = a.bits[l];
-            im.pool_out = (pa >= 0) ? a.pool[pa] : nullptr;
-            im.pcode_out = (pa >= 0 && h2) ? a.pcode[pa] : nullptr;
-            a.bits_valid[l] = a.bits[l] != nullptr;
-            if (pa >= 0) a.pooled[pa] = true;
-            im.amax_in = amax_act(a, l - 1); im.amax_out = amax_act(a, l);
-            flops += conv_flops(im.H, im.W, b.Cin, b.Cout, 9);
-        }
+        const ConvBatch b = forward_batch(ctx, lv, n, l, map_stored(ctx, l), &flops);
         {
             Timer t(ctx, s, K_CONV3, flops, b.img[0].H, b.img[0].W, b.Cin, b.Cout, 9, l);
             NSTCHK(launch_conv_batch(ctx, b, t, true));
@@ -832,6 +860,25 @@
 
 }
 
+namespace nst {
+
+int restore_map(nst_ctx* ctx, int level, int layer, hipStream_t s) {
+    ActSet& a = ctx->lv[level].acts;
+    if (a.stored[layer] || a.pass == 0 || layer > ctx->taps.top) return NST_OK;
+    bool whole = a.pass_n >= 1;
+    for (int k = 0; k < a.pass_n; ++k) whole = whole && ctx->lv[a.pass_lv[k]].acts.pass == a.pass;
+    if (!whole)
+        return fail(ctx, NST_E_STATE, "the level's last forward pass left this map out and a later pass has run over some of its levels: "
+                                      "evaluate the level again, or set keep_all_maps");
+    int lv[NST_MAX_LEVELS];
+    for (int k = 0; k < a.pass_n; ++k) lv[k] = a.pass_lv[k];
+    double flops = 0;
+    const ConvBatch b = forward_batch(ctx, lv, a.pass_n, layer, true, &flops);
+    return launch_conv_batch(ctx, b, s, nullptr, true);
+}
+
+}
+
 extern "C" {
 
 int nst_level_set_targets_blend(nst_ctx* ctx, int level, const float* content, int K, const float* const* styles, const int* hs,
@@ -888,6 +935,7 @@
         NSTCHK(sc.finish());
     }
     L.targets = true;
+    forget_forward_pass(ctx);
     return NST_OK;
 }
 
@@ -1028,6 +1076,7 @@
     }
     NSTCHK(sc.finish());
     g.targets = true; g.targets_R = R;
+    forget_forward_pass(ctx);
     mark(ctx, s);
     return NST_OK;
 }
diff --git a/artstyletransfer_amd/csrc/nst_ctx.cpp b/artstyletransfer_amd/csrc/nst_ctx.cpp
--- a/artstyletransfer_amd/csrc/nst_ctx.cpp
+++ b/artstyletransfer_amd/csrc/nst_ctx.cpp
@@ -311,6 +311,13 @@
     if (ctx->gexec) { (void)hipGraphExecDestroy(ctx->gexec); ctx->gexec = nullptr; }
     ctx->gkey = {}; ctx->glast = {};
     for (int i = 0; drop_targets && i < ctx->levels; ++i) { ctx->lv[i].targets = false; ctx->lv[i].guide.targets = false; }
+    if (drop_targets) forget_forward_pass(ctx);
+}
+void forget_forward_pass(nst_ctx* ctx) {
+    for (int i = 0; i < NST_MAX_LEVELS; ++i) {
+        ctx->lv[i].acts.pass = 0; ctx->lv[i].acts.pass_n = 0;
+        for (bool& st : ctx->lv[i].acts.stored) st = false;
+    }
 }
 
 int fold_timed(nst_ctx* ctx) {
@@ -459,6 +466,7 @@
     ctx->winograd = (opts.h2_winograd >= 0 ? opts.h2_winograd : env_flag("NST_H2_WINOGRAD", 1)) ? 1 : 0;
     ctx->level_split = (opts.level_split >= 0 ? opts.level_split : env_flag("NST_LEVEL_SPLIT", 0)) ? 1 : 0;
     ctx->gram_overlap = (opts.gram_overlap >= 0 ? opts.gram_overlap : env_flag("NST_GRAM_OVERLAP", 0)) ? 1 : 0;
+    ctx->keep_all_maps = env_flag("NST_KEEP_ALL_MAPS", 0) ? 1 : 0;
     if (ctx->use_graph && hipStreamCreateWithFlags(&ctx->gstream, hipStreamNonBlocking) != hipSuccess) { ctx->err = "stream creation failed"; return bail(NST_E_HIP); }
     if (e != hipSuccess) { ctx->err = std::string("kernel attribute setup: ") + hipGetErrorString(e); return bail(NST_E_HIP); }
 
@@ -572,6 +580,7 @@
     quiesce(ctx);
     for (int i = 0; i < NST_MAX_LEVELS; ++i) free_level(ctx, ctx->lv[i]);
     drop_closure_state(ctx, false);
+    forget_forward_pass(ctx);
     ctx->levels = 0;
     int h = H0, w = W0;
     for (int i = 0; i < levels_num; ++i) {
@@ -665,6 +674,25 @@
     return NST_OK;
 }
 
+int nst_ctx_set_keep_all_maps(nst_ctx* ctx, int enabled) {
+    NSTCHK(bind(ctx));
+    ++ctx->ws_seq;
+    drop_closure_state(ctx, false);
+    ctx->keep_all_maps = enabled ? 1 : 0;
+    return NST_OK;
+}
+int nst_ctx_keep_all_maps(const nst_ctx* ctx) { return ctx ? ctx->keep_all_maps : -1; }
+
+int nst_job_map_stats(nst_ctx* ctx, int level, unsigned* stored_mask) {
+    NSTCHK(bind(ctx));
+    if (level < 0 || level >= ctx->levels) return fail(ctx, NST_E_STATE, "level not configured");
+    if (!stored_mask) return fail(ctx, NST_E_ARG, "null argument");
+    unsigned m = 0;
+    for (int l = 0; l < NL; ++l) m |= (ctx->lv[level].acts.stored[l] ? 1u : 0u) << l;
+    *stored_mask = m;
+    return NST_OK;
+}
+
 int nst_job_pooling(const nst_ctx* ctx) { return ctx ? (ctx->pool_avg ? NST_POOL_AVG : NST_POOL_MAX) : -1; }
 
 int nst_job_set_style_weights(nst_ctx* ctx, const float* w) {
@@ -782,6 +810,32 @@
 size_t nst_internal_pixels(const nst_ctx* ctx) { return (ctx && ctx->levels > 0) ? (size_t)ctx->lv[0].h * ctx->lv[0].w : 0; }
 int nst_internal_fail(nst_ctx* ctx, int code, const char* msg) { return fail(ctx, code, msg ? msg : ""); }
 void nst_internal_poison(void* p, size_t bytes) { poison_if_asked(p, bytes); }
+int nst_internal_map_fill(nst_ctx* ctx, int level, int layer, int byte) {
+    if (!ctx || level < 0 || level >= ctx->levels || layer < 0 || layer >= NL) return 1;
+    const ActSet& a = ctx->lv[level].acts;
+    const size_t bytes = (size_t)a.h[layer] * a.w[layer] * kCout[layer] * 4;
+    if (hipSetDevice(ctx->device) != hipSuccess) return 1;
+    quiesce(ctx);
+    hipStream_t zs = nullptr;
+    if (hipStreamCreateWithFlags(&zs, hipStreamNonBlocking) != hipSuccess) return 1;
+    hipError_t e = hipMemsetAsync(a.act[layer], byte, bytes, zs);
+    if (e == hipSuccess) e = hipStreamSynchronize(zs);
+    (void)hipStreamDestroy(zs);
+    return e == hipSuccess ? 0 : 1;
+}
+int nst_internal_map_read(nst_ctx* ctx, int level, int layer, void* dst) {
+    if (!ctx || !dst || level < 0 || level >= ctx->levels || layer < 0 || layer >= NL) return 1;
+    const ActSet& a = ctx->lv[level].acts;
+    const size_t bytes = (size_t)a.h[layer] * a.w[layer] * kCout[layer] * 4;
+    if (hipSetDevice(ctx->device) != hipSuccess) return 1;
+    quiesce(ctx);
+    hipStream_t zs = nullptr;
+    if (hipStreamCreateWithFlags(&zs, hipStreamNonBlocking) != hipSuccess) return 1;
+    hipError_t e = hipMemcpyAsync(dst, a.act[layer], bytes, hipMemcpyDeviceToDevice, zs);
+    if (e == hipSuccess) e = hipStreamSynchronize(zs);
+    (void)hipStreamDestroy(zs);
+    return e == hipSuccess ? 0 : 1;
+}
 int nst_internal_lbfgs_gram(const nst_ctx* ctx) { return ctx ? ctx->lbfgs_gram : 1; }
 unsigned long long nst_internal_closure_epoch(const nst_ctx* ctx) { return ctx ? ctx->closure_epoch : 0; }
 void nst_internal_mark(nst_ctx* ctx, void* stream) { mark(ctx, static_cast<hipStream_t>(stream)); }
diff --git a/artstyletransfer_amd/csrc/nst_ctx.h b/artstyletransfer_amd/csrc/nst_ctx.h
--- a/artstyletransfer_amd/csrc/nst_ctx.h
+++ b/artstyletransfer_amd/csrc/nst_ctx.h
@@ -35,12 +35,17 @@
     unsigned* bits[NL] = {};
     bool bits_valid[NL] = {};
     bool pooled[4] = {};
+    bool stored[NL] = {};
+    unsigned long long pass = 0;
+    int pass_lv[NST_MAX_LEVELS] = {};
+    int pass_n = 0;
     unsigned* amax = nullptr;
     unsigned* pcode[4] = {};
     size_t bytes = 0;
     void begin_pass() {
         for (int l = 0; l < NL; ++l) bits_valid[l] = false;
         for (int k = 0; k < 4; ++k) pooled[k] = false;
+        for (int l = 0; l < NL; ++l) stored[l] = false;
     }
 };
 constexpr int AMAX_IDS = 2 * NST_VGG19_CONVS + kMaxStyle;
@@ -138,6 +143,8 @@
     int gram_overlap = 0;
     int persist = 1;
     int level_split = 0;
+    int keep_all_maps = 0;
+    unsigned long long fwd_pass = 0;
     hipStream_t side = nullptr;
     hipEvent_t side_fork = nullptr, side_join = nullptr;
     hipStream_t tail_stream = nullptr;
@@ -280,6 +287,8 @@
 int gram_of(nst_ctx* ctx, const float* f_nhwc, size_t N, int C, const unsigned* f_amax, float divisor, float* part, const float* target,
             float coef, float* gram_out, float* S, unsigned short* S_bf, unsigned* S_amax, double* mse_partial,
             hipStream_t s);
+int restore_map(nst_ctx* ctx, int level, int layer, hipStream_t s);
+void forget_forward_pass(nst_ctx* ctx);
 size_t gram_part_floats_for(const Taps& tp, int h, int w);
 
 }
diff --git a/artstyletransfer_amd/engine.py b/artstyletransfer_amd/engine.py
--- a/artstyletransfer_amd/engine.py
+++ b/artstyletransfer_amd/engine.py
@@ -43,7 +43,7 @@
                  h2_mfma16: Optional[bool] = None, h2_wg256: Optional[bool] = None,
                  h2_tile_rows: Optional[int] = None, gram_overlap: Optional[bool] = None,
                  h2_persist: Optional[bool] = None, level_split: Optional[bool] = None,
-                 h2_winograd: Optional[bool] = None):
+                 h2_winograd: Optional[bool] = None, keep_all_maps: Optional[bool] = None):
         self.lib = _lib.load()
         if not torch.cuda.is_available():
             raise NstError("no GPU visible: the style-transfer hot path runs only on the HIP device")
@@ -73,6 +73,8 @@
         ctx = C.c_void_p()
         _lib.check(None, self.lib.nst_ctx_create_ex(idx, wp, bp, C.byref(opts), C.byref(ctx)), "nst_ctx_create_ex")
         self.ctx = ctx
+        if keep_all_maps is not None:
+            _lib.check(self.ctx, self.lib.nst_ctx_set_keep_all_maps(self.ctx, int(bool(keep_all_maps))), "nst_ctx_set_keep_all_maps")
         self.weights_id = id(weights)
         self.levels = 0
         self.shape = None
@@ -432,6 +434,11 @@
         _lib.check(self.ctx, self.lib.nst_level_activation(self.ctx, level, layer, _ptr(t), _stream(self.device)),
                    "nst_level_activation")
         return t
+
+    def map_stats(self, level: int) -> int:
+        m = C.c_uint(0)
+        _lib.check(self.ctx, self.lib.nst_job_map_stats(self.ctx, level, C.byref(m)), "nst_job_map_stats")
+        return int(m.value)
 
     def level_image(self, level: int) -> torch.Tensor:
         h, w = self.level_shape(level)
diff --git a/include/nst_hip.h b/include/nst_hip.h
--- a/include/nst_hip.h
+++ b/include/nst_hip.h
@@ -145,6 +145,9 @@
 int nst_vgg_features_backward(nst_ctx* ctx, const float* x, int h, int w, const float* const* gouts,
                               float* gx, void* stream);
 int nst_level_activation(nst_ctx* ctx, int level, int layer, float* out, void* stream);
+int nst_job_map_stats(nst_ctx* ctx, int level, unsigned* stored_mask);
+int nst_ctx_set_keep_all_maps(nst_ctx* ctx, int enabled);
+int nst_ctx_keep_all_maps(const nst_ctx* ctx);
 int nst_level_image(nst_ctx* ctx, int level, float* out, void* stream);
 int nst_gram(nst_ctx* ctx, const float* f, int C, int h, int w, int normalize, float* gram, void* stream);
 int nst_guided_gram_backward(nst_ctx* ctx, const float* f, size_t N, int C, int R, const float* planes, const float* S,
```
